# GrandmasterB42/bevyray

Measured on AMD Instinct MI355X. Metric: Mrays/s at 1920x1080, 64 spp, 8 bounces, higher is better.
Workload: dtype f32

## Files before the change

bevyray_amd/_lib.py:

```python
from __future__ import annotations

import ctypes as C
import os
import subprocess
import threading

_HERE = os.path.dirname(os.path.abspath(__file__))
_CSRC = os.path.join(_HERE, "csrc")
LIB_PATH = os.environ.get("BRT_LIB_PATH") or os.path.join(_HERE, "libbevyray_amd.so")

_lock = threading.Lock()
_lib = None


class BrtStats(C.Structure):
    _fields_ = [
        ("rays", C.c_uint64), ("node_pops", C.c_uint64), ("interior_visits", C.c_uint64),
        ("sphere_tests", C.c_uint64), ("hits", C.c_uint64), ("paths", C.c_uint64),
        ("kernel_ms", C.c_double), ("gather_ms", C.c_double), ("total_ms", C.c_double),
        ("lds_bytes", C.c_uint32), ("scene_in_lds", C.c_uint32), ("n_workgroups", C.c_uint32),
        ("threads_per_workgroup", C.c_uint32), ("prepass_ms", C.c_double),
        ("kernel_variant", C.c_uint32), ("measured_tile_costs", C.c_uint32),
        ("tree_rebuilt", C.c_uint32), ("tree_reach", C.c_float), ("forwarded_bytes", C.c_uint64),
        ("hot_records", C.c_uint32), ("reserved", C.c_uint32),
    ]

    def as_dict(self):
        return {name: getattr(self, name) for name, _ in self._fields_}


def _stale() -> bool:
    if not os.path.exists(LIB_PATH):
        return True
    t = os.path.getmtime(LIB_PATH)
    paths = [os.path.join(_CSRC, s) for s in os.listdir(_CSRC) if s.endswith((".cpp", ".hip", ".h")) or s == "Makefile"]
    paths.append(os.path.join(_HERE, "..", "include", "bevyray_amd.h"))
    return any(os.path.exists(p) and os.path.getmtime(p) > t for p in paths)


def build(force: bool = False) -> str:
    if os.environ.get("BRT_LIB_PATH"):
        return LIB_PATH
    with _lock:
        if force or _stale():
            cmd = ["make", "-C", _CSRC, "-j", str(min(6, os.cpu_count() or 1))] + (["-B"] if force else [])
            proc = subprocess.run(cmd, capture_output=True, text=True)
            if proc.returncode != 0:
                raise RuntimeError("building libbevyray_amd.so failed:\n" + proc.stdout + proc.stderr)
    return LIB_PATH


_VP, _U32, _I32, _F = C.c_void_p, C.c_uint32, C.c_int32, C.c_float
_PROTOTYPES = {
    "brt_abi_version": (_U32, []),
    "brt_last_error": (C.c_char_p, [_VP]),
    "brt_create": (_I32, [C.POINTER(_I32), _I32, C.POINTER(_VP)]),
    "brt_destroy": (_I32, [_VP]),
    "brt_set_policy": (_I32, [_VP, _U32]),
    "brt_set_tuning": (_I32, [_VP, C.c_char_p, _U32]),
    "brt_get_tuning": (_I32, [_VP, C.c_char_p, C.POINTER(_U32), C.POINTER(_U32)]),
    "brt_upload_scene": (_I32, [_VP, _VP, _U32, _VP, _U32, _VP, _U32]),
    "brt_render": (_I32, [_VP, _VP, _VP, _U32, _U32, _U32, _VP, _VP, _VP, _U32, C.POINTER(BrtStats)]),
    "brt_host_alloc": (_I32, [_VP, C.c_uint64, C.POINTER(_VP)]),
    "brt_host_free": (_I32, [_VP, _VP]),
    "brt_render_part_device": (_I32, [_VP, _VP, _VP, _U32, _U32, _U32, _U32, _U32, _VP, _VP, _VP, _VP, _U32,
                                      C.POINTER(BrtStats)]),
    "brt_render_device": (_I32, [_VP, _VP, _VP, _U32, _U32, _U32, _VP, _VP, _VP, _VP, _U32, C.POINTER(BrtStats)]),
    "brt_tile_rows": (_U32, [_U32, _U32]),
    "brt_set_strip_table": (_I32, [_VP, _U32, _U32, _VP]),
    "brt_plan_strips": (_I32, [_VP, _VP, _VP, _U32, _U32, _U32, _U32, _U32, _VP]),
    "brt_host_plan_strips": (_I32, [_VP, _U32, _U32, _VP]),
    "brt_deinterleave_device": (_I32, [_VP, _VP, _U32, _U32, _U32, _VP, _VP, _U32]),
    "brt_rccl_unique_id": (_I32, [_VP]),
    "brt_rccl_comm_create": (_I32, [_VP, _VP, _I32, _I32, C.POINTER(_VP)]),
    "brt_rccl_comm_destroy": (_I32, [_VP, _VP]),
    "brt_gather_rccl": (_I32, [_VP, _VP, _I32, _I32, _VP, _VP, _U32, _U32, _VP, _VP, _U32]),
    "brt_import_frame_fd": (_I32, [_VP, _I32, C.c_uint64, _U32, C.POINTER(_VP)]),
    "brt_release_frame": (_I32, [_VP, _VP]),
    "brt_debug_export_frame_fd": (_I32, [_VP, C.c_uint64, C.POINTER(_I32), C.POINTER(_VP)]),
    "brt_debug_copy_to_host": (_I32, [_VP, _VP, _VP, C.c_uint64]),
    "brt_debug_eval": (_I32, [_VP, _U32, _VP, _VP, _U32]),
    "brt_set_denoise": (_I32, [_VP, _U32, _F, _F, _F]),
    "brt_denoise_device": (_I32, [_VP, _VP, _VP, _U32, _U32, _VP, _VP, _VP, _U32, C.POINTER(BrtStats)]),
    "brt_blend_post_device": (_I32, [_VP, _VP, _VP, _U32, _U32, _VP, _VP, _VP, _VP, _U32, C.POINTER(BrtStats)]),
    "brt_debug_denoise_guides": (_I32, [_VP, _VP, _VP, _U32, _U32, _VP]),
    "brt_set_temporal": (_I32, [_VP, _U32]),
    "brt_reset_temporal": (_I32, [_VP]),
    "brt_debug_temporal_state": (_I32, [_VP, _U32, _U32, _VP]),
    "brt_query_rays_device": (_I32, [_VP, _VP, _U32, _U32, _F, _VP, _VP, _U32, C.POINTER(C.c_uint64)]),
    "brt_query_rays": (_I32, [_VP, _VP, _U32, _U32, _F, _VP, C.POINTER(C.c_uint64)]),
    "brt_query_origin_bound": (_I32, [_VP, C.POINTER(_F)]),
    "brt_host_pixel_ray": (_I32, [_VP, _VP, _U32, _U32, _U32, _U32, _VP]),
    "brt_upscale_device": (_I32, [_VP, _VP, _VP, _U32, _U32, _VP, _U32, _U32, _VP, _VP, _U32, C.POINTER(BrtStats)]),
    "brt_render_upscaled_device": (_I32, [_VP, _VP, _VP, _U32, _U32, _U32, _U32, _VP, _VP, _U32, C.POINTER(BrtStats)]),
    "brt_host_upscale_window": (_I32, [_VP, _U32, _U32, _VP]),
    "brt_upscale_blend_device": (_I32, [_VP, _VP, _VP, _U32, _U32, _U32, _VP, _U32, _U32, _VP, _VP, _VP, _VP, _U32,
                                        C.POINTER(BrtStats)]),
    "brt_render_upscaled_blend_device": (_I32, [_VP, _VP, _VP, _U32, _U32, _U32, _U32, _U32, _VP, _VP, _VP, _VP, _U32,
                                                C.POINTER(BrtStats)]),
    "brt_host_blend_covered": (_I32, [_VP, _U32, _F, _F, C.POINTER(_U32)]),
    "brt_render_pixels_device": (_I32, [_VP, _VP, _VP, _U32, _U32, _VP, _U32, _VP, _VP, _U32, C.POINTER(BrtStats)]),
    "brt_render_pixels": (_I32, [_VP, _VP, _VP, _U32, _U32, _VP, _U32, _VP, _U32, C.POINTER(BrtStats)]),
    "brt_upscale_refine_device": (_I32, [_VP, _VP, _VP, _U32, _U32, _VP, _U32, _U32, _VP, _U32, _VP, _VP, _U32, C.POINTER(BrtStats)]),
    "brt_render_upscaled_refined_device": (_I32, [_VP, _VP, _VP, _U32, _U32, _U32, _U32, _VP, _U32, _VP, _VP, _U32,
                                                  C.POINTER(BrtStats)]),
    "brt_upscale_refine_mask_device": (_I32, [_VP, _VP, _VP, _U32, _U32, _VP, _U32, _U32, _VP, _VP, _U32]),
    "brt_set_adaptive": (_I32, [_VP, _U32, _F, _U32]),
    "brt_render_adaptive_device": (_I32, [_VP, _VP, _VP, _U32, _U32, _VP, _VP, _VP, _U32, C.POINTER(BrtStats)]),
    "brt_adaptive_refine_device": (_I32, [_VP, _VP, _VP, _U32, _U32, _VP, _VP, _VP, _VP, _U32, C.POINTER(BrtStats)]),
    "brt_adaptive_mask_device": (_I32, [_VP, _VP, _VP, _U32, _U32, _VP, _VP, _VP, _U32]),
    "brt_host_adaptive_class": (_I32, [_F, _U32, _VP, _VP, _VP, _VP, _F, _U32, C.POINTER(_U32)]),
    "brt_debug_profile": (_I32, [_VP, C.POINTER(C.c_uint64)]),
    "brt_debug_tile_order": (_I32, [_VP, _VP, _VP, _U32, _U32, C.c_uint64, _U32, _U32, _U32, _VP, _VP]),
    "brt_build_bvh": (_I32, [_VP, _U32, _VP, _U32, C.POINTER(_U32)]),
    "brt_build_bvh_sah": (_I32, [_VP, _U32, _F, _VP, _U32, C.POINTER(_U32)]),
    "brt_host_srgb_thresholds": (_I32, [C.POINTER(_F)]),
    "brt_host_tree_reach": (_I32, [_VP, _U32, _VP, C.POINTER(_F), C.POINTER(_U32), C.POINTER(_F)]),
    "brt_build_bvh_device": (_I32, [_VP, _VP, _U32, _VP, _U32, C.POINTER(_U32), C.POINTER(C.c_double)]),
    "brt_build_bvh_sah_device": (_I32, [_VP, _VP, _U32, _F, _VP, _U32, C.POINTER(_U32), C.POINTER(C.c_double)]),
    "brt_validate_scene": (_I32, [_VP, _U32, _VP, _U32, _VP, _U32, C.POINTER(_U32)]),
    "brt_scene_generate": (_I32, [_U32, C.c_uint64, _VP, _VP, _U32, C.POINTER(_U32)]),
    "brt_host_camera_extract": (_I32, [C.POINTER(_F), C.POINTER(_F), C.POINTER(_F), _F, _F, _F, _F, _U32, _U32, _VP]),
    "brt_host_window_extract": (_I32, [_F, _U32, _VP]),
    "brt_host_material": (_I32, [C.POINTER(_F), _F, _F, _F, _F, _F, _VP]),
    "brt_host_tile_order": (_I32, [_VP, _VP, _U32, _U32, C.c_uint64, _U32, _U32, _U32, _U32, _U32, _VP, _VP]),
}
EXPORTS = tuple(_PROTOTYPES)


def _share_hip_runtime_with_torch() -> None:
    import importlib.util
    import sys
    if os.environ.get("BRT_NO_TORCH") == "1" or "torch" in sys.modules:
        return
    if importlib.util.find_spec("torch") is not None:
        import torch


def load() -> C.CDLL:
    global _lib
    if _lib is not None:
        return _lib
    build()
    _share_hip_runtime_with_torch()
    lib = C.CDLL(LIB_PATH)
    for name, (res, args) in _PROTOTYPES.items():
        fn = getattr(lib, name)
        fn.restype = res
        fn.argtypes = args
    if lib.brt_abi_version() != 6:
        raise RuntimeError("libbevyray_amd.so ABI version mismatch")
    _lib = lib
    return lib


def kernel_code_hash(path: str = LIB_PATH) -> str:
    import hashlib
    import struct
    with open(path, "rb") as f:
        data = f.read()
    if data[:4] != b"\x7fELF" or data[4] != 2:
        raise RuntimeError(f"{path}: not an ELF64 file")
    shoff, = struct.unpack_from("<Q", data, 0x28)
    shentsize, shnum, shstrndx = struct.unpack_from("<HHH", data, 0x3A)
    def sec(i):
        name, _type, _flags, _addr, off, size = struct.unpack_from("<IIQQQQ", data, shoff + i * shentsize)
        return name, off, size
    _, stroff, strsize = sec(shstrndx)
    strtab = data[stroff:stroff + strsize]
    for i in range(shnum):
        name, off, size = sec(i)
        if strtab[name:strtab.index(b"\0", name)] == b".hip_fatbin":
            return hashlib.sha256(data[off:off + size]).hexdigest()[:16]
    raise RuntimeError(f"{path}: no .hip_fatbin section")


class BrtError(RuntimeError):
    def __init__(self, code: int, text: str):
        super().__init__(f"bevyray_amd error {code}: {text}")
        self.code = code
        self.text = text


def check(rc: int, ctx=None) -> None:
    if rc != 0:
        msg = load().brt_last_error(ctx)
        raise BrtError(rc, msg.decode("utf-8", "replace") if msg else "")
```

bevyray_amd/csrc/brt_api.cpp:

```cpp
#include "brt_frame.h"
#include "brt_sah.h"

using namespace brt;

namespace {

uint32_t env_u32(const char* name, uint32_t dflt) {
    const char* v = std::getenv(name);
    if (!v || !*v) return dflt;
    return (uint32_t)std::strtoul(v, nullptr, 10);
}

void free_device(DeviceCtx& dc) {
    if (hipSetDevice(dc.device) != hipSuccess) return;
    for (void* p : std::initializer_list<void*>{dc.d_scene, dc.d_ctrl, dc.d_strip_table, dc.d_tile, dc.d_gather, dc.d_pack, dc.d_raster_rgba,
             dc.d_raster_depth, dc.d_bvh_scratch, dc.d_tile_cost, dc.d_tile_order, dc.d_order_meta, dc.d_order_scratch, dc.d_slice_state,
             dc.d_record_hits, dc.d_bvh_models, dc.d_denoise, dc.d_temporal, dc.d_tsph, dc.d_uplow, dc.d_qctl, dc.d_qmap, dc.d_qrays, dc.d_qhits,
             dc.d_pxbuf, dc.d_pxlist, dc.d_pxout})
        if (p) (void)hipFree(p);
    if (dc.h_stage) (void)hipHostFree(dc.h_stage);
    for (hipEvent_t e : {dc.ev_copy, dc.ev_asm, dc.ev_in, dc.ev_g0, dc.ev_g1, dc.ev_pack, dc.ev_strip, dc.ev_strip_read, dc.ev_q, dc.ev_dn,
                         dc.ev0, dc.ev1, dc.ev_last, dc.ev_p0, dc.ev_p1})
        if (e) (void)hipEventDestroy(e);
    if (dc.stream) (void)hipStreamDestroy(dc.stream);
    dc = DeviceCtx();
}

constexpr uint32_t kMaxSahModels = 1u << 16;
constexpr uint32_t kMaxGpuBuildModels = 1u << 24;

int32_t build_bvh_on_device(brt_ctx* ctx, const Model* models, uint32_t n, bool sah, float reach, std::vector<BVHNode>* out, double* build_ms) {
    out->clear();
    if (n == 0) return BRT_OK;
    if (n > (sah ? kMaxSahModels : kMaxGpuBuildModels))
        return ctx_fail(ctx, BRT_ERR_UNSUPPORTED, sah ? "GPU SAH build supports up to 65 536 spheres" : "GPU BVH build supports up to 2^24 spheres");
    DeviceCtx& dc = ctx->devs[0];
    HIP_TRY(ctx, hipSetDevice(dc.device));
    int32_t rc = ensure(ctx, &dc.d_bvh_scratch, &dc.bvh_scratch_cap,
                        sah ? sah_scratch_bytes(n) : ploc_scratch_bytes(n, nullptr, ctx->knobs[K_PLOC_ONE_BLOCK_MAX]));
    if (rc != BRT_OK) return rc;
    rc = ensure(ctx, &dc.d_bvh_models, &dc.bvh_models_cap, (size_t)n * sizeof(Model));
    if (rc != BRT_OK) return rc;
    HIP_TRY(ctx, hipMemcpyAsync(dc.d_bvh_models, models, (size_t)n * sizeof(Model), hipMemcpyHostToDevice, dc.stream));
    BVHNode* d_out = nullptr;
    uint32_t* d_info = nullptr;
    HIP_TRY(ctx, hipEventRecord(dc.ev0, dc.stream));
    if (sah) HIP_TRY(ctx, launch_build_sah(reinterpret_cast<const Model*>(dc.d_bvh_models), n, reach, dc.d_bvh_scratch, &d_out, &d_info, dc.stream));
    else HIP_TRY(ctx, launch_build_ploc(reinterpret_cast<const Model*>(dc.d_bvh_models), n, dc.d_bvh_scratch, &d_out, &d_info, ctx->knobs[K_PLOC_ONE_BLOCK_MAX], dc.stream));
    HIP_TRY(ctx, hipEventRecord(dc.ev1, dc.stream));
    out->resize(2 * (size_t)n - 1);
    HIP_TRY(ctx, hipMemcpyAsync(out->data(), d_out, out->size() * sizeof(BVHNode), hipMemcpyDeviceToHost, dc.stream));
    uint32_t info[2] = {0u, 0u};
    HIP_TRY(ctx, hipMemcpyAsync(info, d_info, sizeof info, hipMemcpyDeviceToHost, dc.stream));
    HIP_TRY(ctx, hipStreamSynchronize(dc.stream));
    if (info[0] != 2u * n - 1u) {
        out->clear();
        return ctx_fail(ctx, BRT_ERR_HIP, "GPU BVH build made no progress after " + std::to_string(info[1]) + " rounds");
    }
    if (sah) sah_giant_leaves_first(out->data(), (uint32_t)out->size(), models, n);
    float kernel_ms = 0.0f;
    HIP_TRY(ctx, hipEventElapsedTime(&kernel_ms, dc.ev0, dc.ev1));
    if (build_ms) *build_ms = kernel_ms;
    return BRT_OK;
}

}

namespace brt {

int32_t upload_scene(brt_ctx* ctx, const void* models, uint32_t n_models, const void* materials, uint32_t n_materials,
                     const void* bvh_nodes, uint32_t n_nodes, uint32_t level, bool rebuild) {
    if (const uint32_t k = ctx->knobs[K_TEST_THROW]) { ctx->knobs.v[K_TEST_THROW] = 0u; throw_for_test(k); }
    const size_t mb = (size_t)n_models * sizeof(Model), tb = (size_t)n_materials * sizeof(Material),
                 bb = (bvh_nodes ? (size_t)n_nodes : 0) * sizeof(BVHNode);
    auto same = [](const std::vector<char>& v, const void* p, size_t n) {
        return v.size() == n && (n == 0 || (p && std::memcmp(v.data(), p, n) == 0));
    };
    if (!rebuild && ctx->has_scene && ctx->knobs[K_NO_DIRTY_TRACKING] == 0 && same(ctx->last_models, models, mb) &&
        same(ctx->last_materials, materials, tb) && same(ctx->last_bvh, bvh_nodes, bb))
        return BRT_OK;
    for (auto& dc : ctx->devs) {
        HIP_TRY(ctx, hipSetDevice(dc.device));
        for (hipEvent_t e : {dc.ev_last, dc.ev_copy, dc.ev_asm, dc.ev_q}) HIP_TRY(ctx, hipEventSynchronize(e));
    }
    ctx->has_scene = false;
    float reach = 0.0f;
    if (!rebuild) {
        ctx->tree_scene = tree_scene_of(static_cast<const Model*>(models), models ? n_models : 0u);
        ctx->tree_callee_sah = false;
        ctx->tree_level = 0;
        ctx->tree_reach = 0.0f;
        ctx->query_level = 0;
    } else {
        reach = tree_reach_of(ctx->tree_scene.scale, level);
    }
    std::vector<BVHNode> built;
    const BVHNode* nodes = static_cast<const BVHNode*>(bvh_nodes);
    if (n_models > 0 && models && (!bvh_nodes || n_nodes == 0)) {
        const bool sah = ctx->knobs[K_BVH_QUALITY] != 0u && n_models <= kMaxSahModels;
        const bool on_gpu = ctx->knobs[K_CPU_BVH] == 0u && n_models <= kMaxGpuBuildModels;
        int32_t rc;
        if (on_gpu) rc = build_bvh_on_device(ctx, static_cast<const Model*>(models), n_models, sah, reach, &built, nullptr);
        else rc = sah ? build_bvh_sah(static_cast<const Model*>(models), n_models, reach, &built)
                      : build_bvh_ploc(static_cast<const Model*>(models), n_models, &built);
        if (rc != BRT_OK) return rc;
        ctx->tree_callee_sah = sah;
        ctx->tree_level = level;
        ctx->tree_reach = reach;
        nodes = built.data();
        n_nodes = (uint32_t)built.size();
    }
    std::string err;
    int32_t rc = validate_and_encode(static_cast<const Model*>(models), n_models, static_cast<const Material*>(materials),
                                     n_materials, nodes, n_nodes, &ctx->enc, &err);
    if (rc != BRT_OK) return ctx_fail(ctx, rc, err);
    const EncodedScene& e = ctx->enc;

    struct Sec { const void* src; size_t bytes; size_t off; };
    Sec secs[6] = {
        {e.pairs.data(), e.pairs.size() * 4, 0}, {e.spheres.data(), e.spheres.size() * 4, 0},
        {e.sphere_material.data(), e.sphere_material.size() * 4, 0}, {e.materials.data(), e.materials.size() * 4, 0},
        {e.leaf_table.data(), e.leaf_table.size() * 4, 0}, {e.sphere_mats.data(), e.sphere_mats.size() * 4, 0}};
    size_t total = 0;
    for (auto& s : secs) { s.off = total; total += align256(s.bytes ? s.bytes : 16); }

    const uint64_t shape = (ctx->knobs[K_HOT_RECORDS] != 0u && !rebuild && e.desc16 && e.simple_tree && e.n_pairs > 64u) ? tree_shape_hash(e) : 0ull;
    ctx->tree_epoch++;
    for (auto& dc : ctx->devs) {
        HIP_TRY(ctx, hipSetDevice(dc.device));
        int32_t r2 = ensure(ctx, &dc.d_scene, &dc.scene_cap, total);
        if (r2 != BRT_OK) return r2;
        const bool reuse = shape != 0ull && dc.hot_shape == shape && dc.hot_records != 0u && dc.h_total_rank.size() == e.n_pairs &&
                           dc.h_total_srank.size() == e.n_models;
        uint32_t root = e.root_desc;
        Sec mine[6];
        for (int q = 0; q < 6; q++) mine[q] = secs[q];
        if (reuse) {
            permute_scene(e.pairs, e.spheres, e.sphere_material, e.sphere_mats, e.root_desc, dc.h_total_rank, dc.h_total_srank, &dc.h_pairs_cur,
                          &dc.h_spheres_cur, &dc.h_sphmat_cur, &dc.h_sphmats_cur, &root);
            mine[0].src = dc.h_pairs_cur.data(); mine[1].src = dc.h_spheres_cur.data(); mine[2].src = dc.h_sphmat_cur.data(); mine[5].src = dc.h_sphmats_cur.data();
        }
        for (auto& s : mine)
            if (s.bytes) HIP_TRY(ctx, hipMemcpyAsync(dc.d_scene + s.off, s.src, s.bytes, hipMemcpyHostToDevice, dc.stream));
        const uint32_t kept_hot = reuse ? dc.hot_records : 0u;
        DeviceSceneView v{};
        v.pairs = reinterpret_cast<const float*>(dc.d_scene + secs[0].off);
        v.spheres = reinterpret_cast<const float*>(dc.d_scene + secs[1].off);
        v.sphere_material = reinterpret_cast<const uint32_t*>(dc.d_scene + secs[2].off);
        v.materials = reinterpret_cast<const float*>(dc.d_scene + secs[3].off);
        v.leaf_table = reinterpret_cast<const uint32_t*>(dc.d_scene + secs[4].off);
        v.sphere_mats = reinterpret_cast<const float*>(dc.d_scene + secs[5].off);
        v.n_pairs = e.n_pairs;
        v.n_models = e.n_models;
        v.n_materials = e.n_materials;
        v.n_leaf_table = (uint32_t)(e.leaf_table.size() / 2);
        v.root_desc = root;
        v.stack_entries = e.stack_entries;
        v.desc16 = e.desc16 ? 1u : 0u;
        v.simple_tree = e.simple_tree ? 1u : 0u;
        v.boxes_ordered = e.boxes_ordered ? 1u : 0u;
        dc.view = v;
        dc.hot_records = kept_hot;
        if (reuse) dc.hot_tree = ctx->tree_epoch;
        dc.frames_since_upload = 0u;
    }
    for (auto& dc : ctx->devs) {
        HIP_TRY(ctx, hipSetDevice(dc.device));
        HIP_TRY(ctx, hipStreamSynchronize(dc.stream));
    }
// ... 284 lines not shown
```

bevyray_amd/csrc/brt_api_launch.cpp:

```cpp
#include "brt_frame.h"

namespace brt {

int32_t make_frame_params(brt_ctx* ctx, const void* camera80, const void* window16, uint32_t level, uint32_t width,
                          uint32_t height, uint32_t part, uint32_t n_parts, FrameParams* out) {
    if (const uint32_t k = ctx->knobs[K_TEST_THROW]) { ctx->knobs.v[K_TEST_THROW] = 0u; throw_for_test(k); }
    if (!camera80 || !window16) return ctx_fail(ctx, BRT_ERR_INVALID_ARGUMENT, "camera/window is null");
    if (width == 0 || height == 0 || width > 32768u || height > 32768u)
        return ctx_fail(ctx, BRT_ERR_INVALID_ARGUMENT, "width/height must be in [1, 32768]");
    if (n_parts == 0 || part >= n_parts) return ctx_fail(ctx, BRT_ERR_INVALID_ARGUMENT, "part >= n_parts");
    Camera cam;
    Window win;
    std::memcpy(&cam, camera80, sizeof cam);
    std::memcpy(&win, window16, sizeof win);
    if (cam.projection_type != 0)
        return ctx_fail(ctx, BRT_ERR_UNSUPPORTED, "only perspective projection (0) is supported (extract.rs:148)");
    if (cam.bounce_count >= 0x7fffffffu) return ctx_fail(ctx, BRT_ERR_INVALID_ARGUMENT, "bounce_count too large");
    FrameParams fp;
    std::memset(&fp, 0, sizeof fp);
    fp.width = width;
    fp.height = height;
    fp.level = level;
    fp.sample_count = cam.sample_count;
    fp.bounce_count = cam.bounce_count;
    fp.seed_scaled = win.random_seed * 10000.0f;
    const float heightf = (float)win.height;
    const float widthf = (float)win.height * cam.aspect;
    fp.inv_width = 1.0f / widthf;
    fp.inv_height = 1.0f / heightf;
    fp.aspect = cam.aspect;
    fp.tan_half_fov = tan_half_fov(cam.fov);
    for (int k = 0; k < 3; k++) {
        fp.cam_pos[k] = cam.position[k];
        fp.cam_dir[k] = cam.direction[k];
        fp.cam_up[k] = cam.up[k];
    }
    const float* a = cam.direction;
    const float* b = cam.up;
    fp.cam_right[0] = a[1] * b[2] - a[2] * b[1];
    fp.cam_right[1] = a[2] * b[0] - a[0] * b[2];
    fp.cam_right[2] = a[0] * b[1] - a[1] * b[0];
    fp.near_ = cam.near_;
    fp.far_ = cam.far_;
    fp.fallback_far = (level == 1u) ? cam.far_ + 10.0f : cam.far_ - 1.0f;
    fp.spp_f = (float)cam.sample_count;
    fp.part = part;
    fp.n_parts = n_parts;
    fp.tiles_x = (width + 7u) / 8u;
    const uint32_t strips = (height + BRT_STRIP_ROWS - 1u) / BRT_STRIP_ROWS;
    fp.local_strips = (strips + n_parts - 1u) / n_parts;
    fp.queue_size = fp.local_strips * fp.tiles_x * 64u;
    fp.queue_lane = 0u;
    fp.bottom_up = ctx->knobs[K_BOTTOM_UP];
    fp.refill_min = std::clamp(ctx->knobs[K_REFILL_MIN], 1u, 64u);
    fp.walk_exit_lanes = std::min(ctx->knobs[K_WALK_EXIT], 63u);
    fp.leaf_vote = std::min(ctx->knobs[K_LEAF_VOTE], 64u);
    fp.drain_donate = std::min(ctx->knobs[K_DRAIN_DONATE], 56u);
    fp.pool_cap = 0;
    fp.pool_adopt = std::min(ctx->knobs[K_POOL_ADOPT], 63u);
    fp.crit_begin = fp.crit_end = 0;
    fp.split_nonsky = fp.split_tiles = 0;
    fp.slice_state = nullptr;
    fp.slice_serial = 0;
    fp.wgq_batch = std::min(ctx->knobs[K_WGQ_BATCH] & ~63u, 512u);
    fp.policy_flags = ctx->policy_flags & kPolicyMask;
    fp.tunable = (fp.policy_flags != 0u || fp.bottom_up != 0u || fp.refill_min != kRefillMin || fp.walk_exit_lanes != kWalkExitLanes ||
                  fp.leaf_vote != kLeafVote || fp.drain_donate != kDrainDonate || fp.pool_adopt != kPoolAdopt ||
                  fp.wgq_batch != 0u || ctx->knobs[K_LPT_LANE_PERMILLE] != 0u || ctx->knobs[K_TUNABLE] != 0u)
                     ? 1u : 0u;
    *out = fp;
    return BRT_OK;
}

LaunchPlan plan_launch(const Knobs& kn, const DeviceCtx& dc, const FrameParams& fp) {
    LaunchPlan lp{};
    const uint32_t hist = fp.record_hits ? dc.view.n_pairs : 0u;
    const bool force_global = kn[K_FORCE_GLOBAL_SCENE] != 0;
    const uint32_t force_top = kn[K_FORCE_LDS_TOP];
    const uint32_t block_env = kn[K_BLOCK_THREADS];
    const uint32_t wg_env = kn[K_WG_PER_CU];
    const uint32_t max_waves_cu = 32;
    lp.scene_mode = SCENE_GLOBAL;
    const uint64_t n_tiles = fp.queue_size / 64u, wave_slots = (uint64_t)dc.num_cus * (BRT_BLOCK / 64u);
    const uint32_t pool_max = (2u * n_tiles <= 5u * wave_slots && kn[K_POOL_FORCE] == 0u) ? 0u : kn[K_POOL_CAP];
    auto pool_of = [&](uint32_t block) {
        const uint32_t want = fp.drain_donate * (block / 64u - 1u);
        return want < pool_max ? want : pool_max;
    };
    if (!force_global && !force_top && dc.view.desc16) {
        struct Cand { uint32_t block, per_cu; };
        const Cand cands[] = {{1024, 1}, {512, 2}, {512, 3}, {1024, 2}, {512, 1}, {256, 1}};
        for (int opt = 0; opt < 4 && lp.scene_mode != SCENE_LDS; opt++) {
            const int with_pool = opt < 2 ? 1 : 0, with_rows = (opt & 1) == 0 ? 1 : 0;
            for (const Cand& c : cands) {
                if (block_env && c.block != block_env) continue;
                if (wg_env && c.per_cu != wg_env) continue;
                const uint32_t pool = with_pool ? pool_of(c.block) : 0u;
                const size_t need = trace_lds_bytes(dc.view, SCENE_LDS, c.block, pool, 0, with_rows != 0);
                if (need * c.per_cu <= dc.max_lds && c.per_cu * (c.block / 64) <= max_waves_cu) {
                    lp.scene_mode = SCENE_LDS;
                    lp.block = c.block;
                    lp.wg_per_cu = c.per_cu;
                    lp.lds_bytes = need;
                    lp.pool_cap = pool;
                    lp.rows = (uint32_t)with_rows;
                    break;
                }
            }
        }
    }
    if (lp.scene_mode != SCENE_LDS && !force_global && dc.view.desc16) {
        DeviceSceneView v = dc.view;
        v.lds_pairs = 0;
        const uint32_t block = block_env ? block_env : BRT_BLOCK;
        const uint32_t per_cu = wg_env ? wg_env : 1u;
        const size_t share = dc.max_lds / per_cu;
        const uint32_t pool = pool_of(block) < 192u / per_cu ? pool_of(block) : 192u / per_cu;
        const size_t fixed = trace_lds_bytes(v, SCENE_LDS_TOP, block, pool, hist);
        if (fixed + 64 * PAIR_BYTES <= share && per_cu * (block / 64u) <= max_waves_cu) {
            uint32_t k = (uint32_t)((share - fixed) / PAIR_BYTES);
            if (k > v.n_pairs) k = v.n_pairs;
            if (force_top && force_top < k) k = force_top;
            v.lds_pairs = k;
            lp.scene_mode = SCENE_LDS_TOP;
            lp.lds_pairs = k;
            lp.block = block;
            lp.wg_per_cu = per_cu;
            lp.pool_cap = pool;
            lp.lds_bytes = trace_lds_bytes(v, SCENE_LDS_TOP, block, pool, hist);
        }
    }
    if (lp.scene_mode == SCENE_GLOBAL) {
        lp.block = block_env ? block_env : 256u;
        lp.pool_cap = pool_of(lp.block);
        lp.lds_bytes = trace_lds_bytes(dc.view, SCENE_GLOBAL, lp.block, lp.pool_cap);
        uint32_t per_cu = (uint32_t)(dc.max_lds / (lp.lds_bytes ? lp.lds_bytes : 1));
        const uint32_t by_waves = max_waves_cu / (lp.block / 64u);
        if (per_cu > by_waves) per_cu = by_waves;
        if (per_cu < 1) per_cu = 1;
        if (wg_env) per_cu = wg_env;
        lp.wg_per_cu = per_cu;
    }
    lp.grid = (uint32_t)dc.num_cus * lp.wg_per_cu;
    const uint32_t useful = (fp.queue_size + lp.block - 1u) / lp.block;
    if (lp.grid > useful) lp.grid = useful;
    if (lp.grid < 1) lp.grid = 1;
    return lp;
}

int32_t launch_part(brt_ctx* ctx, DeviceCtx& dc, const FrameParams& fp, const float* d_raster_rgba,
                    const float* d_raster_depth, float* d_out_tile, hipStream_t stream, uint32_t flags, bool timed,
                    LaunchPlan* plan_out) {
    HIP_TRY(ctx, hipStreamWaitEvent(stream, dc.ev_last, 0));
    HIP_TRY(ctx, hipMemsetAsync(dc.d_ctrl, 0, 512, stream));
    if (timed) HIP_TRY(ctx, hipEventRecord(dc.ev0, stream));
    LaunchPlan lp{};
    if (fp.level == 0u) {
        HIP_TRY(ctx, launch_passthrough(fp, d_out_tile, d_raster_rgba, stream));
    } else {
        TraceLaunch tl{};
        tl.scene = dc.view;
        tl.frame = fp;
        tl.queue_counter = reinterpret_cast<uint32_t*>(dc.d_ctrl + 256);
        tl.out_tile = d_out_tile;
        tl.raster_rgba = d_raster_rgba;
        tl.raster_depth = d_raster_depth;
        tl.counters = reinterpret_cast<unsigned long long*>(dc.d_ctrl);
        tl.counters_on = (flags & BRT_FLAG_COUNTERS) != 0;
        tl.stream = stream;
        if (flags & BRT_FLAG_KERNEL_SIMPLE) {
            if (fp.policy_flags != 0u) return ctx_fail(ctx, BRT_ERR_UNSUPPORTED, "the bring-up kernel implements the default policy only (brt_set_policy)");
            HIP_TRY(ctx, launch_trace_simple(tl));
            lp.block = 256;
            lp.grid = (fp.queue_size + 255u) / 256u;
        } else {
            lp = plan_launch(ctx->knobs, dc, fp);
            {
                uint32_t key[8];
                view_key_of(ctx, fp, key);
                const bool known = dc.view_rays != 0 && std::memcmp(key, dc.view_key, sizeof key) == 0;
                const uint64_t per_lane = known ? dc.view_rays / ((uint64_t)dc.num_cus * BRT_BLOCK) : 0;
                const uint64_t longest_bound = (uint64_t)fp.sample_count * ((uint64_t)fp.bounce_count + 1u);
                const bool lean1 = !tl.frame.tunable && fp.level == 3u && !tl.counters_on && ctx->knobs[K_NO_LEAN] == 0u &&
                                   (fp.tile_cost == nullptr || ctx->knobs[K_LEAN_MEASURE] != 0u);
                tl.lean = !lean1 ? 0 : ((known && longest_bound < per_lane / 2) ? 2 : 1);
                lp.variant = (uint32_t)tl.lean | (tl.frame.tunable ? 16u : 0u);
                lp.measured = fp.tile_cost != nullptr ? 1u : 0u;
            }
            tl.scene_mode = lp.scene_mode;
            tl.scene.lds_pairs = lp.lds_pairs;
            tl.grid = lp.grid;
            tl.block = lp.block;
            tl.lds_bytes = lp.lds_bytes;
            tl.frame.pool_cap = lp.pool_cap;
            tl.frame.rows_on = lp.scene_mode == SCENE_LDS ? lp.rows : 0u;
            if (tl.frame.wgq_batch == 0u) {
                uint32_t b = (fp.queue_size / (lp.grid * 8u)) & ~63u;
                const uint32_t cap = (lp.block / 2u) & ~63u;
                if (b > cap) b = cap;
                if (b > 512u) b = 512u;
                if (b < 64u) b = 64u;
                tl.frame.wgq_batch = b;
            }
            HIP_TRY(ctx, launch_trace_persistent(tl));
        }
    }
    if (timed) HIP_TRY(ctx, hipEventRecord(dc.ev1, stream));
    HIP_TRY(ctx, hipEventRecord(dc.ev_last, stream));
    if (plan_out) *plan_out = lp;
    return BRT_OK;
}

uint64_t part_pixels(const FrameParams& fp) { return PartStrips(fp.height, fp.part, fp.n_parts).total_rows() * fp.width; }

void launch_stats(const brt_ctx* ctx, const DeviceCtx& dc, const LaunchPlan& lp, brt_stats* stats) {
    stats->lds_bytes = (uint32_t)lp.lds_bytes;
    stats->scene_in_lds = lp.scene_mode == SCENE_LDS ? 1u : (lp.scene_mode == SCENE_LDS_TOP ? 2u : 0u);
    stats->n_workgroups = lp.grid;
    stats->threads_per_workgroup = lp.block;
    stats->kernel_variant = lp.variant;
    stats->measured_tile_costs = lp.measured;
    stats->hot_records = dc.hot_tree == ctx->tree_epoch ? dc.hot_records : 0u;
}

int32_t collect_part(brt_ctx* ctx, DeviceCtx& dc, const FrameParams& fp, hipStream_t stream, bool prepass_ran, brt_stats* st) {
    int32_t rc = update_tile_order(ctx, dc, fp, stream);
    if (rc != BRT_OK) return rc;
    unsigned long long c[5];
    HIP_TRY(ctx, hipMemcpyAsync(c, dc.d_ctrl, sizeof c, hipMemcpyDeviceToHost, stream));
    HIP_TRY(ctx, hipStreamSynchronize(stream));
    st->rays += c[0];
    st->node_pops += c[1];
    st->interior_visits += c[2];
    st->sphere_tests += c[3];
    st->hits += c[4];
    dc.view_rays = c[0];
    view_key_of(ctx, fp, dc.view_key);
    float ms = 0.0f;
    HIP_TRY(ctx, hipEventElapsedTime(&ms, dc.ev0, dc.ev1));
    if (ms > st->kernel_ms) st->kernel_ms = ms;
    if (prepass_ran) {
        HIP_TRY(ctx, hipEventElapsedTime(&ms, dc.ev_p0, dc.ev_p1));
        if (ms > st->prepass_ms) st->prepass_ms = ms;
    }
    return BRT_OK;
}

}
```

bevyray_amd/csrc/brt_api_order.cpp:

```cpp
#include "brt_frame.h"

using namespace brt;

namespace {

bool lpt_enabled(const brt_ctx* ctx) { return ctx->knobs[K_LPT] != 0; }
uint64_t camera_hash(const FrameParams& fp) {
    uint64_t h = 1469598103934665603ull;
    auto mix = [&](const float* f, int n) {
        for (int i = 0; i < n; i++) { uint32_t u; std::memcpy(&u, f + i, 4); h = (h ^ u) * 1099511628211ull; }
    };
    mix(fp.cam_pos, 3); mix(fp.cam_dir, 3); mix(fp.cam_up, 3); mix(&fp.tan_half_fov, 1); mix(&fp.aspect, 1);
    return h | 1ull;
}

void order_key_of(const brt_ctx* ctx, const FrameParams& fp, uint32_t key[6]) {
    key[0] = fp.width; key[1] = fp.height; key[2] = fp.part; key[3] = fp.n_parts;
    key[4] = fp.strip_of ? ctx->strip_epoch : 0u;
    key[5] = fp.local_strips * fp.tiles_x;
}

constexpr uint32_t kMaxDilate = 8;
double camera_motion_px(const brt_ctx* ctx, const float* pos0, const float* dir0, const FrameParams& fp) {
    const float* a = dir0;
// ... 17 lines not shown
    const double px = camera_motion_px(ctx, dc.cost_cam_pos, dc.cost_cam_dir, fp);
    if (!(px < 8.0 * kMaxDilate)) return kMaxDilate + 1u;
    return (uint32_t)std::ceil(px / 8.0) + 1u;
}
bool camera_jumped(const brt_ctx* ctx, const DeviceCtx& dc, const FrameParams& fp) {
    return dc.costs_valid && camera_hash(fp) != dc.order_cam && dilation_tiles(ctx, dc, fp) > kMaxDilate;
}

uint32_t split_tail_of(const brt_ctx* ctx, const DeviceCtx& dc, uint32_t n_tiles) {
    const uint64_t wave_slots = (uint64_t)dc.num_cus * (BRT_BLOCK / 64u);
    if (ctx->knobs[K_SPLIT_FORCE] != 0u) return ctx->knobs[K_SPLIT_FORCE] < n_tiles ? ctx->knobs[K_SPLIT_FORCE] : n_tiles;
    if ((uint64_t)n_tiles < 6u * wave_slots) return 0u;
    uint64_t r = (uint64_t)ctx->knobs[K_SPLIT_TAIL] * wave_slots / 4u;
    if (r != 0u && r < n_tiles / 2u) r = n_tiles / 2u;
    return (uint32_t)(r < n_tiles ? r : n_tiles);
}

int32_t build_order_on_device(brt_ctx* ctx, DeviceCtx& dc, uint32_t n_tiles, uint32_t tiles_x, uint32_t spp, uint32_t rx, uint32_t ry,
                              hipStream_t stream) {
    if (!dc.d_order_meta) HIP_TRY(ctx, hipMalloc(reinterpret_cast<void**>(&dc.d_order_meta), 256));
    int32_t rc = ensure(ctx, &dc.d_order_scratch, &dc.order_scratch_cap, order_scratch_bytes(n_tiles));
    if (rc != BRT_OK) return rc;
    const uint32_t split_tail = split_tail_of(ctx, dc, n_tiles);
    rc = ensure(ctx, &dc.d_tile_order, &dc.tile_order_cap, ((size_t)n_tiles + split_tail) * 4);
    if (rc != BRT_OK) return rc;
    const uint64_t sky_cost = (uint64_t)64 * spp * (1000 + ctx->knobs[K_LPT_SKY_SLACK]) / 1000;
    HIP_TRY(ctx, launch_build_order(dc.d_tile_cost, dc.d_tile_cost + n_tiles, n_tiles, sky_cost, (uint64_t)dc.num_cus * BRT_BLOCK, tiles_x, rx,
                                    ry, split_tail, dc.d_tile_order, dc.d_order_meta, dc.d_order_scratch, stream));
    HIP_TRY(ctx, hipEventRecord(dc.ev_last, stream));
    return BRT_OK;
}

int32_t apply_hot_order(brt_ctx* ctx, DeviceCtx& dc, hipStream_t stream) {
    const uint32_t n = dc.view.n_pairs, m = dc.view.n_models;
    const EncodedScene& e = ctx->enc;
    if (n == 0u || e.pairs.size() != (size_t)n * PAIR_WORDS || e.spheres.size() != (size_t)m * 4u || e.sphere_material.size() != m || e.sphere_mats.size() != (size_t)m * 8u) return BRT_OK;
    if (dc.hot_tree != ctx->tree_epoch) { dc.h_pairs_cur = e.pairs; dc.h_spheres_cur = e.spheres; dc.h_sphmat_cur = e.sphere_material; dc.h_sphmats_cur = e.sphere_mats; }
    const std::vector<float>& cur = dc.h_pairs_cur;
    const uint32_t cur_root = dc.hot_tree != ctx->tree_epoch ? e.root_desc : dc.view.root_desc;
    dc.h_hits.resize(n);
    HIP_TRY(ctx, hipMemcpyAsync(dc.h_hits.data(), dc.d_record_hits, (size_t)n * 4, hipMemcpyDeviceToHost, stream));
    HIP_TRY(ctx, hipStreamSynchronize(stream));
    std::vector<uint32_t>& rank = dc.h_rank;
    std::vector<uint32_t> order(n);
    for (uint32_t i = 0; i < n; i++) order[i] = i;
    std::stable_sort(order.begin(), order.end(), [&](uint32_t a, uint32_t b) { return dc.h_hits[a] > dc.h_hits[b]; });
    rank.resize(n);
    uint32_t visited = 0;
    for (uint32_t i = 0; i < n; i++) { rank[order[i]] = i; visited += dc.h_hits[order[i]] != 0u ? 1u : 0u; }
    using D = Desc<true>;
    constexpr uint32_t kDescWord = PAIR_DESC / 4u;
    std::vector<uint32_t> score(m, 0u), sorder(m), srank(m);
    auto leaf_sphere = [&](uint32_t d, uint32_t* id) {
        if ((int32_t)d < -1 && (d & D::LEAF1)) { *id = d & D::INDEX_MASK; return *id < m; }
        return false;
    };
    for (uint32_t r = 0; r < n; r++)
        for (uint32_t k = 0; k < 2u; k++) {
            uint32_t d, id;
            std::memcpy(&d, cur.data() + (size_t)r * PAIR_WORDS + kDescWord + k, 4);
            if (leaf_sphere(d, &id) && dc.h_hits[r] > score[id]) score[id] = dc.h_hits[r];
        }
    for (uint32_t i = 0; i < m; i++) sorder[i] = i;
    std::stable_sort(sorder.begin(), sorder.end(), [&](uint32_t a, uint32_t b) { return score[a] > score[b]; });
    for (uint32_t i = 0; i < m; i++) srank[sorder[i]] = i;
    std::vector<float> sph, mats;
    std::vector<uint32_t> mat;
    uint32_t new_root = 0;
    permute_scene(cur, dc.h_spheres_cur, dc.h_sphmat_cur, dc.h_sphmats_cur, cur_root, rank, srank, &dc.h_pairs_hot, &sph, &mat, &mats, &new_root);
    HIP_TRY(ctx, hipEventSynchronize(dc.ev_q));
    dc.hot_serial++;
    HIP_TRY(ctx, hipMemcpyAsync(const_cast<float*>(dc.view.pairs), dc.h_pairs_hot.data(), dc.h_pairs_hot.size() * 4, hipMemcpyHostToDevice, stream));
    HIP_TRY(ctx, hipMemcpyAsync(const_cast<float*>(dc.view.spheres), sph.data(), sph.size() * 4, hipMemcpyHostToDevice, stream));
    HIP_TRY(ctx, hipMemcpyAsync(const_cast<uint32_t*>(dc.view.sphere_material), mat.data(), mat.size() * 4, hipMemcpyHostToDevice, stream));
    HIP_TRY(ctx, hipMemcpyAsync(const_cast<float*>(dc.view.sphere_mats), mats.data(), mats.size() * 4, hipMemcpyHostToDevice, stream));
    HIP_TRY(ctx, hipStreamSynchronize(stream));
    if (dc.hot_tree == ctx->tree_epoch && dc.h_total_rank.size() == n && dc.h_total_srank.size() == m) {
        for (uint32_t i = 0; i < n; i++) dc.h_total_rank[i] = rank[dc.h_total_rank[i]];
        for (uint32_t i = 0; i < m; i++) dc.h_total_srank[i] = srank[dc.h_total_srank[i]];
    } else {
        dc.h_total_rank = rank;
        dc.h_total_srank = srank;
    }
    dc.hot_shape = tree_shape_hash(e);
    dc.h_pairs_cur.swap(dc.h_pairs_hot);
    dc.h_spheres_cur.swap(sph);
    dc.h_sphmat_cur.swap(mat);
    dc.h_sphmats_cur.swap(mats);
    dc.view.root_desc = new_root;
    dc.hot_tree = ctx->tree_epoch;
    dc.hot_records = visited;
    return BRT_OK;
}

}

namespace brt {

void view_key_of(const brt_ctx* ctx, const FrameParams& fp, uint32_t key[8]) {
    order_key_of(ctx, fp, key);
    key[6] = fp.sample_count; key[7] = fp.bounce_count;
}

int32_t attach_tile_order(brt_ctx* ctx, DeviceCtx& dc, FrameParams& fp, hipStream_t stream, bool may_measure, uint32_t flags) {
    fp.tile_order = nullptr;
    fp.tile_cost = nullptr;
    if (!lpt_enabled(ctx) || fp.level == 0u || (flags & BRT_FLAG_KERNEL_SIMPLE)) return BRT_OK;
    const uint32_t n_tiles = fp.local_strips * fp.tiles_x;
    uint32_t key[6];
    order_key_of(ctx, fp, key);
    const bool match = dc.order_valid && std::memcmp(key, dc.order_key, sizeof key) == 0;
    if (match && dc.costs_valid && dc.order_on_device && camera_hash(fp) != dc.order_cam && ctx->knobs[K_LPT_DILATE] != 0u) {
        uint32_t r = dilation_tiles(ctx, dc, fp);
        if (r <= kMaxDilate && ctx->knobs[K_LPT_DILATE] >= 2u && r < ctx->knobs[K_LPT_DILATE] - 1u &&
            (uint64_t)n_tiles >= 6u * (uint64_t)dc.num_cus * (BRT_BLOCK / 64u))
            r = ctx->knobs[K_LPT_DILATE] - 1u;
        if (r <= kMaxDilate) {
            HIP_TRY(ctx, hipStreamWaitEvent(stream, dc.ev_last, 0));
            const int32_t rc = build_order_on_device(ctx, dc, n_tiles, fp.tiles_x, dc.cost_spp, r, (r + fp.n_parts - 1u) / fp.n_parts, stream);
            if (rc != BRT_OK) return rc;
        }
    }
    if (match) {
        fp.tile_order = dc.d_tile_order;
        fp.queue_lane = dc.order_lane * 64u;
        fp.crit_begin = 0u;
        fp.crit_end = dc.order_crit * 64u;
        fp.order_meta = dc.order_on_device ? dc.d_order_meta : nullptr;
        if (split_tail_of(ctx, dc, n_tiles) != 0u) {
            const size_t bytes = (size_t)fp.queue_size * 36u;
            const bool fresh = bytes > dc.slice_state_cap;
            int32_t rc = ensure(ctx, &dc.d_slice_state, &dc.slice_state_cap, bytes);
            if (rc != BRT_OK) return rc;
            if (fresh || dc.slice_serial >= 0x3fffffffu) {
                HIP_TRY(ctx, hipMemsetAsync(dc.d_slice_state, 0, dc.slice_state_cap, stream));
                dc.slice_serial = 0u;
            }
            fp.slice_state = dc.d_slice_state;
            fp.slice_serial = ++dc.slice_serial;
            if (!dc.order_on_device) { fp.split_nonsky = dc.order_nonsky; fp.split_tiles = dc.order_split; }
        }
    }
    bool due = !match || camera_hash(fp) != dc.order_cam || ctx->knobs[K_LPT_REFRESH_EVERY] == 1u;
    if (may_measure && match && dc.remeasure_in != 0u && --dc.remeasure_in == 0u) due = true;
    if (may_measure && due) {
        int32_t rc = ensure(ctx, &dc.d_tile_cost, &dc.tile_cost_cap, (size_t)n_tiles * 8);
        if (rc != BRT_OK) return rc;
        HIP_TRY(ctx, hipMemsetAsync(dc.d_tile_cost, 0, (size_t)n_tiles * 8, stream));
        fp.tile_cost = dc.d_tile_cost;
    }
    return BRT_OK;
}

int32_t update_tile_order(brt_ctx* ctx, DeviceCtx& dc, const FrameParams& fp, hipStream_t stream) {
    if (!fp.tile_cost) return BRT_OK;
    const uint32_t n_tiles = fp.local_strips * fp.tiles_x;
    TileOrderParams tp{};
    tp.sample_count = fp.sample_count;
    tp.grid_lanes = (uint64_t)dc.num_cus * BRT_BLOCK;
    tp.sorted = ctx->knobs[K_LPT_SORT];
    tp.sky_slack_permille = ctx->knobs[K_LPT_SKY_SLACK];
    tp.lane_permille = ctx->knobs[K_LPT_LANE_PERMILLE];
    tp.critical = ctx->knobs[K_CRIT];
    tp.tiles_x = fp.tiles_x;
    tp.split_tail = split_tail_of(ctx, dc, n_tiles);
    int32_t rc = ensure(ctx, &dc.d_tile_order, &dc.tile_order_cap, ((size_t)n_tiles + tp.split_tail) * 4);
    if (rc != BRT_OK) return rc;
    const bool on_device = tp.sorted == 1u && tp.critical == 1u && tp.lane_permille == 0u && ctx->knobs[K_ORDER_ON_HOST] == 0u;
    dc.costs_valid = false;
    if (on_device) {
        const uint64_t wave_slots = (uint64_t)dc.num_cus * (BRT_BLOCK / 64u);
        const uint32_t r0 = (ctx->knobs[K_LPT_DILATE] >= 2u && (uint64_t)n_tiles >= 6u * wave_slots) ? ctx->knobs[K_LPT_DILATE] - 1u : 0u;
        tp.dilate_x = r0;
        tp.dilate_y = r0 ? (r0 + fp.n_parts - 1u) / fp.n_parts : 0u;
        rc = build_order_on_device(ctx, dc, n_tiles, fp.tiles_x, tp.sample_count, tp.dilate_x, tp.dilate_y, stream);
        if (rc != BRT_OK) return rc;
        dc.order_lane = 0;
        dc.order_crit = 0;
        dc.order_on_device = true;
        dc.costs_valid = true;
        dc.cost_spp = tp.sample_count;
        for (int k = 0; k < 3; k++) { dc.cost_cam_pos[k] = fp.cam_pos[k]; dc.cost_cam_dir[k] = fp.cam_dir[k]; }
    } else {
        dc.h_cost.resize(2 * (size_t)n_tiles);
        HIP_TRY(ctx, hipMemcpyAsync(dc.h_cost.data(), dc.d_tile_cost, (size_t)n_tiles * 8, hipMemcpyDeviceToHost, stream));
        HIP_TRY(ctx, hipStreamSynchronize(stream));
        TileOrder to;
        build_tile_order(dc.h_cost.data(), dc.h_cost.data() + n_tiles, n_tiles, tp, &to);
        dc.h_order.swap(to.order);
        dc.order_lane = to.n_lane;
        dc.order_crit = to.n_critical;
        dc.order_on_device = false;
        dc.order_nonsky = to.n_nonsky;
        dc.order_split = to.n_split;
        HIP_TRY(ctx, hipMemcpyAsync(dc.d_tile_order, dc.h_order.data(), dc.h_order.size() * 4, hipMemcpyHostToDevice, stream));
        HIP_TRY(ctx, hipStreamSynchronize(stream));
    }
    order_key_of(ctx, fp, dc.order_key);
    dc.order_valid = true;
    dc.remeasure_in = 0;
    dc.order_cam = camera_hash(fp);
    return BRT_OK;
}

uint64_t tree_shape_hash(const EncodedScene& e) {
    uint64_t h = 1469598103934665603ull ^ ((uint64_t)e.n_pairs << 32) ^ e.n_models;
    constexpr uint32_t kDescWord = PAIR_DESC / 4u;
    for (uint32_t r = 0; r < e.n_pairs; r++)
        for (uint32_t k = 0; k < 2u; k++) {
            uint32_t d;
            std::memcpy(&d, e.pairs.data() + (size_t)r * PAIR_WORDS + kDescWord + k, 4);
            h = (h ^ d) * 1099511628211ull;
        }
    return h | 1ull;
}

void permute_scene(const std::vector<float>& pairs, const std::vector<float>& spheres, const std::vector<uint32_t>& sphmat,
                   const std::vector<float>& sphmats, uint32_t root, const std::vector<uint32_t>& rank, const std::vector<uint32_t>& srank,
                   std::vector<float>* out_pairs, std::vector<float>* out_spheres, std::vector<uint32_t>* out_sphmat,
                   std::vector<float>* out_sphmats, uint32_t* out_root) {
    using D = Desc<true>;
    constexpr uint32_t kDescWord = PAIR_DESC / 4u;
    const uint32_t n = (uint32_t)rank.size(), m = (uint32_t)srank.size();
    auto remap = [&](uint32_t d) {
        if ((int32_t)d >= 0 && d < n) return rank[d];
        if ((int32_t)d < -1 && (d & D::LEAF1) && (d & D::INDEX_MASK) < m) return (d & ~D::INDEX_MASK) | srank[d & D::INDEX_MASK];
        return d;
    };
    out_pairs->resize(pairs.size());
    for (uint32_t i = 0; i < n; i++) {
        const float* src = pairs.data() + (size_t)i * PAIR_WORDS;
        float* dst = out_pairs->data() + (size_t)rank[i] * PAIR_WORDS;
        std::memcpy(dst, src, PAIR_BYTES);
        for (uint32_t k = 0; k < 2u; k++) {
            uint32_t d;
            std::memcpy(&d, src + kDescWord + k, 4);
            d = remap(d);
            std::memcpy(dst + kDescWord + k, &d, 4);
        }
    }
    out_spheres->resize(spheres.size());
    out_sphmats->resize(sphmats.size());
    out_sphmat->resize(m);
    for (uint32_t i = 0; i < m; i++) {
        std::memcpy(out_spheres->data() + (size_t)srank[i] * 4, spheres.data() + (size_t)i * 4, 16);
        std::memcpy(out_sphmats->data() + (size_t)srank[i] * 8, sphmats.data() + (size_t)i * 8, 32);
        (*out_sphmat)[srank[i]] = sphmat[i];
    }
    *out_root = remap(root);
}

int32_t prepass_order(brt_ctx* ctx, DeviceCtx& dc, const FrameParams& fp, const float* d_raster_rgba,
                      const float* d_raster_depth, float* d_out_tile, hipStream_t stream, uint32_t flags, bool* ran) {
    *ran = false;
    const uint32_t knob = ctx->knobs[K_PREPASS_SPP];
    const uint32_t k = knob < fp.sample_count / 16u ? knob : fp.sample_count / 16u;
    if (k == 0u || (k == 1u && knob != 1u) || !lpt_enabled(ctx) || fp.level == 0u || (flags & BRT_FLAG_KERNEL_SIMPLE)) return BRT_OK;
    uint32_t key[6];
    order_key_of(ctx, fp, key);
    bool hot_stale = ctx->knobs[K_HOT_RECORDS] != 0u && dc.hot_tree == ctx->tree_epoch && dc.hot_records != 0u &&
                     camera_motion_px(ctx, dc.hot_cam_pos, dc.hot_cam_dir, fp) > std::max(64.0, 0.25 * (double)fp.height);
    if (dc.frames_since_upload < 1000u) dc.frames_since_upload++;
    if (!hot_stale && ctx->knobs[K_HOT_RECORDS] != 0u && dc.hot_tree != ctx->tree_epoch && dc.frames_since_upload == 2u && dc.view.desc16 &&
        dc.view.simple_tree && dc.view.n_pairs > 64u && plan_launch(ctx->knobs, dc, fp).scene_mode == SCENE_LDS_TOP)
        hot_stale = true;
    if (dc.order_valid && std::memcmp(key, dc.order_key, sizeof key) == 0 && !(ctx->knobs[K_LPT_DILATE] != 0u && camera_jumped(ctx, dc, fp)) && !hot_stale)
        return BRT_OK;
    FrameParams pp = fp;
    pp.sample_count = k;
    pp.spp_f = (float)k;
    pp.tile_order = nullptr;
    pp.order_meta = nullptr;
    pp.slice_state = nullptr;
    pp.split_nonsky = pp.split_tiles = 0u;
    pp.tunable = 1u;
    pp.queue_lane = 0u;
    pp.crit_begin = pp.crit_end = 0u;
    const uint32_t n_tiles = pp.local_strips * pp.tiles_x;
    int32_t rc = ensure(ctx, &dc.d_tile_cost, &dc.tile_cost_cap, (size_t)n_tiles * 8);
    if (rc != BRT_OK) return rc;
    HIP_TRY(ctx, hipMemsetAsync(dc.d_tile_cost, 0, (size_t)n_tiles * 8, stream));
    pp.tile_cost = dc.d_tile_cost;
    bool count_hits = false;
    if (ctx->knobs[K_HOT_RECORDS] != 0u && dc.view.desc16 && dc.view.simple_tree && dc.view.n_pairs > 64u &&
        plan_launch(ctx->knobs, dc, pp).scene_mode == SCENE_LDS_TOP) {
        rc = ensure(ctx, &dc.d_record_hits, &dc.record_hits_cap, (size_t)dc.view.n_pairs * 4);
        if (rc != BRT_OK) return rc;
        HIP_TRY(ctx, hipMemsetAsync(dc.d_record_hits, 0, (size_t)dc.view.n_pairs * 4, stream));
        pp.record_hits = dc.d_record_hits;
        count_hits = plan_launch(ctx->knobs, dc, pp).scene_mode == SCENE_LDS_TOP;
        if (!count_hits) pp.record_hits = nullptr;
    }
    HIP_TRY(ctx, hipEventRecord(dc.ev_p0, stream));
    rc = launch_part(ctx, dc, pp, d_raster_rgba, d_raster_depth, d_out_tile, stream, flags & ~(uint32_t)BRT_FLAG_COUNTERS, false, nullptr);
    if (rc != BRT_OK) return rc;
    HIP_TRY(ctx, hipEventRecord(dc.ev_p1, stream));
    rc = update_tile_order(ctx, dc, pp, stream);
    if (rc != BRT_OK) return rc;
    if (count_hits) {
        rc = apply_hot_order(ctx, dc, stream);
        if (rc != BRT_OK) return rc;
        for (int q = 0; q < 3; q++) { dc.hot_cam_pos[q] = fp.cam_pos[q]; dc.hot_cam_dir[q] = fp.cam_dir[q]; }
    }
    dc.remeasure_in = 1u;
    *ran = true;
    return BRT_OK;
}

bool strip_table_valid(const uint32_t* t, uint32_t n_strips, uint32_t n_parts) {
    if (n_parts == 0u || n_parts > 64u) return false;
    for (uint32_t g = 0; g * n_parts < n_strips; g++) {
        uint64_t seen = 0;
        for (uint32_t s = g * n_parts; s < n_strips && s < (g + 1u) * n_parts; s++) {
            if (t[s] >= n_parts || (seen >> t[s]) & 1ull) return false;
            seen |= 1ull << t[s];
        }
    }
    return true;
}
int32_t strip_table_attach(brt_ctx* ctx, DeviceCtx& dc, FrameParams* fp, const uint32_t** part_of_strip, hipStream_t stream) {
    if (part_of_strip) *part_of_strip = nullptr;
    const uint32_t strips = (fp->height + BRT_STRIP_ROWS - 1u) / BRT_STRIP_ROWS, n_parts = fp->n_parts;
    if (ctx->strip_part.empty() || ctx->strip_n_parts != n_parts || ctx->strip_part.size() != strips || n_parts < 2u) return BRT_OK;
    const uint32_t local = (strips + n_parts - 1u) / n_parts;
    if (dc.strip_epoch != ctx->strip_epoch || !dc.d_strip_table) {
        const size_t words = (size_t)strips + (size_t)n_parts * local;
        HIP_TRY(ctx, hipEventSynchronize(dc.ev_strip));
        if (dc.strip_table_cap < words * 4u)
            for (hipEvent_t e : {dc.ev_last, dc.ev_strip_read}) HIP_TRY(ctx, hipEventSynchronize(e));
        int32_t rc = ensure(ctx, &dc.d_strip_table, &dc.strip_table_cap, words * 4u);
        if (rc != BRT_OK) return rc;
        std::vector<uint32_t>& h = dc.h_strip_table;
        h.assign(words, 0xffffffu);
        std::copy(ctx->strip_part.begin(), ctx->strip_part.end(), h.begin());
        for (uint32_t s = 0; s < strips; s++) h[(size_t)strips + (size_t)ctx->strip_part[s] * local + s / n_parts] = s;
        HIP_TRY(ctx, hipStreamWaitEvent(stream, dc.ev_last, 0));
        HIP_TRY(ctx, hipStreamWaitEvent(stream, dc.ev_strip_read, 0));
        HIP_TRY(ctx, hipMemcpyAsync(dc.d_strip_table, h.data(), words * 4u, hipMemcpyHostToDevice, stream));
        HIP_TRY(ctx, hipEventRecord(dc.ev_strip, stream));
        dc.strip_epoch = ctx->strip_epoch;
    } else {
        HIP_TRY(ctx, hipStreamWaitEvent(stream, dc.ev_strip, 0));
    }
    const uint32_t* d = reinterpret_cast<const uint32_t*>(dc.d_strip_table);
    if (part_of_strip) *part_of_strip = d;
    fp->strip_of = d + strips + (size_t)fp->part * local;
    return BRT_OK;
}
int32_t strip_table_read(brt_ctx* ctx, DeviceCtx& dc, const uint32_t* part_of_strip, hipStream_t stream) {
    if (!part_of_strip) return BRT_OK;
    HIP_TRY(ctx, hipStreamWaitEvent(stream, dc.ev_strip_read, 0));
    HIP_TRY(ctx, hipEventRecord(dc.ev_strip_read, stream));
    return BRT_OK;
}
uint64_t part_pixels_table(const brt_ctx* ctx, const FrameParams& fp) {
    uint64_t rows = 0;
    for (uint32_t s = 0; s < (uint32_t)ctx->strip_part.size(); s++)
        if (ctx->strip_part[s] == fp.part) {
            const uint32_t r0 = s * BRT_STRIP_ROWS;
            rows += (r0 + BRT_STRIP_ROWS <= fp.height) ? BRT_STRIP_ROWS : (fp.height - r0);
        }
    return rows * fp.width;
}

}

extern "C" {

uint32_t brt_tile_rows(uint32_t height, uint32_t n_parts) {
    if (n_parts == 0) return 0;
    const uint32_t strips = (height + BRT_STRIP_ROWS - 1u) / BRT_STRIP_ROWS;
    return ((strips + n_parts - 1u) / n_parts) * BRT_STRIP_ROWS;
}

int32_t brt_set_strip_table(brt_ctx* ctx, uint32_t n_parts, uint32_t n_strips, const uint32_t* part_of_strip) {
    return guard(ctx ? &ctx->last_error : nullptr, [&]() -> int32_t {
    if (!ctx) return fail(BRT_ERR_INVALID_ARGUMENT, "ctx is null");
    if (!part_of_strip) { ctx->strip_epoch++; ctx->strip_part.clear(); ctx->strip_n_parts = 0u; return BRT_OK; }
    if (n_parts < 1u || n_strips < 1u || n_strips > 4096u) return ctx_fail(ctx, BRT_ERR_INVALID_ARGUMENT, "n_parts / n_strips out of range");
    if (!strip_table_valid(part_of_strip, n_strips, n_parts))
        return ctx_fail(ctx, BRT_ERR_INVALID_ARGUMENT, "strip table: every group of n_parts consecutive strips must hold each part at most once");
    ctx->strip_epoch++;
    ctx->strip_part.assign(part_of_strip, part_of_strip + n_strips);
    ctx->strip_n_parts = n_parts;
    return BRT_OK;
    });
}

int32_t brt_plan_strips(brt_ctx* ctx, const void* camera80, const void* window16, uint32_t level, uint32_t width, uint32_t height,
                        uint32_t n_parts, uint32_t probe_spp, uint32_t* out_part_of_strip) {
    return guard(ctx ? &ctx->last_error : nullptr, [&]() -> int32_t {
    if (!ctx) return fail(BRT_ERR_INVALID_ARGUMENT, "ctx is null");
    if (!ctx->has_scene) return ctx_fail(ctx, BRT_ERR_NO_SCENE, "no scene uploaded");
    if (n_parts < 1u || n_parts > 64u || probe_spp < 1u) return ctx_fail(ctx, BRT_ERR_INVALID_ARGUMENT, "n_parts must be 1..64, probe_spp >= 1");
    FrameParams fp;
    int32_t rc = make_frame_params(ctx, camera80, window16, level == 0u ? 3u : level, width, height, 0u, 1u, &fp);
    if (rc != BRT_OK) return rc;
    fp.sample_count = probe_spp;
    fp.spp_f = (float)probe_spp;
    DeviceCtx& dc = ctx->devs[0];
    HIP_TRY(ctx, hipSetDevice(dc.device));
    const uint32_t n_tiles = fp.local_strips * fp.tiles_x, strips = fp.local_strips;
    rc = ensure(ctx, &dc.d_tile, &dc.tile_cap, (size_t)strips * BRT_STRIP_ROWS * width * 16u);
    if (rc != BRT_OK) return rc;
    rc = ensure(ctx, &dc.d_tile_cost, &dc.tile_cost_cap, (size_t)n_tiles * 8u);
    if (rc != BRT_OK) return rc;
    HIP_TRY(ctx, hipStreamWaitEvent(dc.stream, dc.ev_last, 0));
    HIP_TRY(ctx, hipMemsetAsync(dc.d_tile_cost, 0, (size_t)n_tiles * 8u, dc.stream));
    fp.tile_cost = dc.d_tile_cost;
    rc = launch_part(ctx, dc, fp, nullptr, nullptr, dc.d_tile, dc.stream, 0u, false, nullptr);
    if (rc != BRT_OK) return rc;
    std::vector<uint32_t> cost(n_tiles);
    HIP_TRY(ctx, hipMemcpyAsync(cost.data(), dc.d_tile_cost, (size_t)n_tiles * 4u, hipMemcpyDeviceToHost, dc.stream));
    HIP_TRY(ctx, hipStreamSynchronize(dc.stream));
    dc.costs_valid = false;
    std::vector<uint64_t> strip_cost(strips, 0);
    for (uint32_t t = 0; t < n_tiles; t++) strip_cost[t / fp.tiles_x] += cost[t];
    std::vector<uint32_t> table(strips, 0u);
    plan_strip_table(strip_cost.data(), strips, n_parts, table.data());
    if (out_part_of_strip) std::memcpy(out_part_of_strip, table.data(), (size_t)strips * 4u);
    ctx->strip_epoch++;
    ctx->strip_part = table;
    ctx->strip_n_parts = n_parts;
    return BRT_OK;
    });
}

int32_t brt_debug_tile_order(brt_ctx* ctx, const uint32_t* ray_sum, const uint32_t* longest_pixel, uint32_t n_tiles,
                             uint32_t sample_count, uint64_t grid_lanes, uint32_t tiles_x, uint32_t dilate, uint32_t split_tail,
                             uint32_t* out_order, uint32_t* out_info4) {
    return guard(ctx ? &ctx->last_error : nullptr, [&]() -> int32_t {
    if (!ctx) return fail(BRT_ERR_INVALID_ARGUMENT, "ctx is null");
    if (!ray_sum || !longest_pixel || !out_order || !out_info4 || n_tiles == 0) return ctx_fail(ctx, BRT_ERR_INVALID_ARGUMENT, "null buffer / no tiles");
    if (dilate != 0u && (tiles_x == 0u || n_tiles % tiles_x != 0u)) return ctx_fail(ctx, BRT_ERR_INVALID_ARGUMENT, "dilate needs a tiles_x that divides n_tiles");
    DeviceCtx& dc = ctx->devs[0];
    HIP_TRY(ctx, hipSetDevice(dc.device));
    uint32_t* d_cost = nullptr;
    uint32_t* d_order = nullptr;
    uint32_t* d_meta = nullptr;
    char* d_scratch = nullptr;
    auto body = [&]() -> int32_t {
        HIP_TRY(ctx, hipMalloc(reinterpret_cast<void**>(&d_cost), (size_t)n_tiles * 8));
        HIP_TRY(ctx, hipMalloc(reinterpret_cast<void**>(&d_order), ((size_t)n_tiles + split_tail) * 4));
        HIP_TRY(ctx, hipMalloc(reinterpret_cast<void**>(&d_meta), 256));
        HIP_TRY(ctx, hipMalloc(reinterpret_cast<void**>(&d_scratch), order_scratch_bytes(n_tiles)));
        HIP_TRY(ctx, hipMemcpyAsync(d_cost, ray_sum, (size_t)n_tiles * 4, hipMemcpyHostToDevice, dc.stream));
        HIP_TRY(ctx, hipMemcpyAsync(d_cost + n_tiles, longest_pixel, (size_t)n_tiles * 4, hipMemcpyHostToDevice, dc.stream));
        const uint64_t sky_cost = (uint64_t)64 * sample_count * (1000 + 20) / 1000;
        HIP_TRY(ctx, launch_build_order(d_cost, d_cost + n_tiles, n_tiles, sky_cost, grid_lanes, tiles_x, dilate, dilate, split_tail, d_order, d_meta, d_scratch, dc.stream));
        HIP_TRY(ctx, hipMemcpyAsync(out_info4, d_meta, 16, hipMemcpyDeviceToHost, dc.stream));
        HIP_TRY(ctx, hipStreamSynchronize(dc.stream));
        HIP_TRY(ctx, hipMemcpy(out_order, d_order, ((size_t)n_tiles + out_info4[3]) * 4, hipMemcpyDeviceToHost));
        return BRT_OK;
    };
    const int32_t rc = body();
    if (d_cost) (void)hipFree(d_cost);
    if (d_order) (void)hipFree(d_order);
    if (d_meta) (void)hipFree(d_meta);
    if (d_scratch) (void)hipFree(d_scratch);
    return rc;
    });
}

}
```

bevyray_amd/csrc/brt_ctx.h:

```cpp
#pragma once
#include <hip/hip_runtime.h>

#include <cstdint>
#include <cstring>
#include <string>
#include <vector>

#include "brt_adaptive.h"
#include "brt_denoise.h"
#include "brt_temporal.h"
#include "brt_host.h"
#include "brt_kernels.h"
#include "brt_pixels.h"
#include "brt_query.h"
#include "brt_upscale.h"

namespace brt {

struct DeviceCtx {
    int device = 0;
    hipStream_t stream = nullptr;
    hipEvent_t ev0 = nullptr, ev1 = nullptr;
    hipEvent_t ev_last = nullptr;
    hipEvent_t ev_p0 = nullptr, ev_p1 = nullptr;
    int num_cus = 0;
    size_t max_lds = 0;
    char* d_scene = nullptr;
    size_t scene_cap = 0;
    DeviceSceneView view{};
    char* d_ctrl = nullptr;
    float* d_tile = nullptr;
    size_t tile_cap = 0;
    float* d_raster_rgba = nullptr;
    size_t raster_rgba_cap = 0;
    float* d_raster_depth = nullptr;
    size_t raster_depth_cap = 0;
    float* d_gather = nullptr;
    size_t gather_cap = 0;
    float* d_pack = nullptr;
    size_t pack_cap = 0;
    hipEvent_t ev_pack = nullptr;
    hipEvent_t ev_copy = nullptr;
    hipEvent_t ev_asm = nullptr;
    hipEvent_t ev_in = nullptr;
    hipEvent_t ev_g0 = nullptr, ev_g1 = nullptr;
    float* h_stage = nullptr;
    size_t stage_cap = 0;
    uint32_t* d_tile_cost = nullptr;
    size_t tile_cost_cap = 0;
    uint32_t* d_tile_order = nullptr;
    uint32_t order_nonsky = 0, order_split = 0;
    uint32_t* d_slice_state = nullptr;
    size_t slice_state_cap = 0;
    uint32_t slice_serial = 0;
    uint32_t order_lane = 0;
    uint32_t order_crit = 0;
    size_t tile_order_cap = 0;
    uint32_t* d_order_meta = nullptr;
    char* d_strip_table = nullptr;
    size_t strip_table_cap = 0;
    uint32_t strip_epoch = 0;
    std::vector<uint32_t> h_strip_table;
    hipEvent_t ev_strip = nullptr;
    hipEvent_t ev_strip_read = nullptr;
    char* d_order_scratch = nullptr;
    size_t order_scratch_cap = 0;
    bool order_on_device = false;
    uint64_t view_rays = 0;
    uint32_t view_key[8] = {0, 0, 0, 0, 0, 0, 0, 0};
    uint64_t base_view_rays = 0;
    uint32_t base_view_key[8] = {0, 0, 0, 0, 0, 0, 0, 0};
    bool order_valid = false;
    uint32_t remeasure_in = 0;
    uint64_t order_cam = 0;
    bool costs_valid = false;
    float cost_cam_pos[3] = {0, 0, 0}, cost_cam_dir[3] = {0, 0, 0};
    uint32_t cost_spp = 0;
    uint32_t order_key[6] = {0, 0, 0, 0, 0, 0};
    std::vector<uint32_t> h_cost;
    std::vector<uint32_t> h_order;
    uint32_t* d_record_hits = nullptr;
    size_t record_hits_cap = 0;
    uint32_t hot_tree = 0;
    uint32_t hot_records = 0;
    float hot_cam_pos[3] = {0, 0, 0}, hot_cam_dir[3] = {0, 0, 1};
    uint32_t frames_since_upload = 0;
    std::vector<uint32_t> h_hits, h_rank;
    std::vector<uint32_t> h_total_rank, h_total_srank;
    uint64_t hot_shape = 0;
    std::vector<float> h_spheres_cur, h_sphmats_cur;
    std::vector<uint32_t> h_sphmat_cur;
    std::vector<float> h_pairs_hot, h_pairs_cur;
    char* d_denoise = nullptr;
    size_t denoise_cap = 0;
    hipEvent_t ev_dn = nullptr;
    char* d_temporal = nullptr;
    size_t temporal_cap = 0;
    char* d_tsph = nullptr;
    size_t tsph_cap = 0;
    float* d_uplow = nullptr;
    size_t uplow_cap = 0;
    hipEvent_t ev_q = nullptr;
    uint32_t* d_qctl = nullptr;
    uint32_t* d_qmap = nullptr;
    size_t qmap_cap = 0;
    uint32_t qmap_tree = 0, qmap_serial = 0;
    uint32_t hot_serial = 0;
    char* d_qrays = nullptr;
    size_t qrays_cap = 0;
    char* d_qhits = nullptr;
    size_t qhits_cap = 0;
    uint32_t* d_pxbuf = nullptr;
    size_t pxbuf_cap = 0;
    char* d_pxlist = nullptr;
    size_t pxlist_cap = 0;
    char* d_pxout = nullptr;
    size_t pxout_cap = 0;
    char* d_bvh_scratch = nullptr;
    size_t bvh_scratch_cap = 0;
    char* d_bvh_models = nullptr;
    size_t bvh_models_cap = 0;
};


enum Knob : int {
    K_BOTTOM_UP, K_REFILL_MIN, K_WALK_EXIT, K_LEAF_VOTE, K_DRAIN_DONATE, K_POOL_ADOPT, K_WGQ_BATCH, K_LPT_LANE_PERMILLE, K_TUNABLE,
    K_FORCE_GLOBAL_SCENE, K_FORCE_LDS_TOP, K_BLOCK_THREADS, K_WG_PER_CU, K_POOL_CAP, K_LPT, K_LPT_SORT, K_LPT_SKY_SLACK, K_CRIT,
    K_ORDER_ON_HOST, K_NO_LEAN, K_PREPASS_SPP, K_NO_DIRTY_TRACKING, K_CPU_BVH, K_PLOC_ONE_BLOCK_MAX, K_BVH_QUALITY, K_POOL_FORCE, K_LPT_REFRESH_EVERY, K_LEAN_MEASURE, K_LPT_DILATE, K_SPLIT_TAIL, K_SPLIT_FORCE, K_HOT_RECORDS, K_TEST_THROW, K_QUERY_FORM, K_QUERY_STREAM_MIN, K_PIXELS_FORM, K_COUNT
};
struct KnobDef { const char* name; uint32_t dflt; };
constexpr KnobDef kKnobs[K_COUNT] = {
    {"BRT_BOTTOM_UP", 0}, {"BRT_REFILL_MIN", kRefillMin}, {"BRT_WALK_EXIT", kWalkExitLanes}, {"BRT_LEAF_VOTE", kLeafVote},
    {"BRT_DRAIN_DONATE", kDrainDonate}, {"BRT_POOL_ADOPT", kPoolAdopt}, {"BRT_WGQ_BATCH", 0}, {"BRT_LPT_LANE_PERMILLE", 0},
    {"BRT_TUNABLE", 0}, {"BRT_FORCE_GLOBAL_SCENE", 0}, {"BRT_FORCE_LDS_TOP", 0}, {"BRT_BLOCK_THREADS", 0}, {"BRT_WG_PER_CU", 0},
    {"BRT_POOL_CAP", 384}, {"BRT_LPT", 1}, {"BRT_LPT_SORT", 1}, {"BRT_LPT_SKY_SLACK", 20}, {"BRT_CRIT", 1}, {"BRT_ORDER_ON_HOST", 0},
    {"BRT_NO_LEAN", 0}, {"BRT_PREPASS_SPP", 4}, {"BRT_NO_DIRTY_TRACKING", 0}, {"BRT_CPU_BVH", 0},
    {"BRT_PLOC_ONE_BLOCK_MAX", kPlocOneBlockMax}, {"BRT_BVH_QUALITY", 1}, {"BRT_POOL_FORCE", 0}, {"BRT_LPT_REFRESH_EVERY", 0}, {"BRT_LEAN_MEASURE", 1}, {"BRT_LPT_DILATE", 3}, {"BRT_SPLIT_TAIL", 16}, {"BRT_SPLIT_FORCE", 0}, {"BRT_HOT_RECORDS", 1}, {"BRT_TEST_THROW", 0},
    {"BRT_QUERY_FORM", 0}, {"BRT_QUERY_STREAM_MIN", 0},
    {"BRT_PIXELS_FORM", 0}};
struct Knobs {
    uint32_t v[K_COUNT];
    Knobs() { for (int i = 0; i < K_COUNT; i++) v[i] = kKnobs[i].dflt; }
    uint32_t operator[](Knob k) const { return v[k]; }
};

}

namespace brt {
struct ExternalFrame {
    void* ptr = nullptr;
    size_t bytes = 0, mapped = 0;
    uint32_t type = 0;
    hipExternalMemory_t ext = nullptr;
    hipMemGenericAllocationHandle_t vmm{};
};
}

struct brt_ctx {
    std::vector<brt::ExternalFrame> external;
    std::vector<brt::DeviceCtx> devs;
    brt::EncodedScene enc;
    bool has_scene = false;
    uint32_t scene_epoch = 0;
    std::vector<uint32_t> strip_part;
    uint32_t strip_n_parts = 0, strip_epoch = 0;
    uint32_t tree_epoch = 0;
    uint32_t last_n_models = 0;
    std::vector<std::pair<char*, size_t>> pinned;
    std::vector<char> last_models, last_materials, last_bvh;
    float scene_centre[3] = {0, 0, 0};
    bool tree_callee_sah = false;
    brt::TreeScene tree_scene;
    uint32_t tree_level = 0;
    float tree_reach = 0.0f;
    uint32_t tree_rebuilds = 0;
    uint32_t query_level = 0;
    brt::Knobs knobs;
    uint32_t policy_flags = 0;
    brt::DenoiseSettings denoise;
    struct Adaptive {
        uint32_t base_spp = 8;
        float threshold = brt::kAdaptDefaultThreshold;
        uint32_t min_taps = 6;
    } adaptive;
    struct Temporal {
        uint32_t max_history = 32;
        bool valid = false;
        uint32_t width = 0, height = 0, set = 0;
        brt::FrameParams prev{};
        uint32_t prev_models = 0;
        int64_t prev_epoch = -1;
        uint32_t slot_models = 0;
        int64_t slot_epoch[2] = {-1, -1};
        std::vector<uint32_t> h_rmap;
    } temporal;
    std::string last_error;
};

namespace brt {

inline int32_t ctx_fail(brt_ctx* ctx, int32_t code, const std::string& msg) {
    if (ctx) ctx->last_error = msg;
    g_last_error = msg;
    return code;
}

#define HIP_TRY(ctx, expr)                                                                              \
    do {                                                                                                \
        hipError_t _e = (expr);                                                                         \
        if (_e != hipSuccess)                                                                           \
            return ctx_fail(ctx, BRT_ERR_HIP, std::string(#expr) + ": " + hipGetErrorString(_e));       \
    } while (0)

template <typename T>
int32_t ensure(brt_ctx* ctx, T** ptr, size_t* cap, size_t bytes) {
    if (*cap >= bytes && *ptr) return BRT_OK;
    if (*ptr) HIP_TRY(ctx, hipFree(*ptr));
    *ptr = nullptr;
    *cap = 0;
    HIP_TRY(ctx, hipMalloc(reinterpret_cast<void**>(ptr), bytes));
    *cap = bytes;
    return BRT_OK;
}

inline size_t align256(size_t x) { return (x + 255) & ~(size_t)255; }

void release_external_frames(brt_ctx* ctx);

}

namespace brt {
bool strip_table_valid(const uint32_t* part_of_strip, uint32_t n_strips, uint32_t n_parts);
int32_t strip_table_attach(brt_ctx* ctx, DeviceCtx& dc, FrameParams* fp, const uint32_t** part_of_strip, hipStream_t stream);
int32_t strip_table_read(brt_ctx* ctx, DeviceCtx& dc, const uint32_t* part_of_strip, hipStream_t stream);
uint64_t part_pixels_table(const brt_ctx* ctx, const FrameParams& fp);
}
```

bevyray_amd/csrc/brt_frame.h:

```cpp
#pragma once
#include <hip/hip_runtime.h>

#include <algorithm>
#include <chrono>
#include <cmath>
#include <cstdlib>
#include <cstring>
#include <limits>
#include <string>
#include <vector>

#include "brt_ctx.h"

namespace brt {

constexpr uint32_t kPolicyMask = BRT_POLICY_OR_SHORT_CIRCUIT | BRT_POLICY_MINMAX_SELECT | BRT_POLICY_POW_EXP2_LOG2;
constexpr uint32_t kLptAfterUpload = 4;

inline double ms_since(std::chrono::steady_clock::time_point t0) {
    return std::chrono::duration<double, std::milli>(std::chrono::steady_clock::now() - t0).count();
}

struct StreamChoice { bool own; hipStream_t stream; };
inline StreamChoice stream_of(const DeviceCtx& dc, void* hip_stream, uint32_t flags) {
    const bool own = (hip_stream == nullptr) && !(flags & BRT_FLAG_CALLER_STREAM);
    return {own, own ? dc.stream : static_cast<hipStream_t>(hip_stream)};
}

struct PartStrips {
    uint32_t part, n_parts;
    uint32_t n_full;
    uint32_t tail_rows;
    PartStrips(uint32_t height, uint32_t part_, uint32_t n_parts_) : part(part_), n_parts(n_parts_) {
        const uint32_t full = height / BRT_STRIP_ROWS;
        n_full = full > part ? (full - part + n_parts - 1u) / n_parts : 0u;
        tail_rows = full % n_parts == part ? height - full * BRT_STRIP_ROWS : 0u;
    }
    uint32_t count() const { return n_full + (tail_rows ? 1u : 0u); }
    uint32_t frame_row(uint32_t k) const { return (part + k * n_parts) * BRT_STRIP_ROWS; }
    uint32_t rows(uint32_t k) const { return k < n_full ? BRT_STRIP_ROWS : tail_rows; }
    uint64_t total_rows() const { return (uint64_t)n_full * BRT_STRIP_ROWS + tail_rows; }
};

int32_t upload_scene(brt_ctx* ctx, const void* models, uint32_t n_models, const void* materials, uint32_t n_materials,
                     const void* bvh_nodes, uint32_t n_nodes, uint32_t level, bool rebuild);
int32_t ensure_tree_reach(brt_ctx* ctx, const void* camera80, uint32_t* rebuilt);
void tree_stats(const brt_ctx* ctx, uint32_t rebuilt, brt_stats* stats);

struct LaunchPlan {
    int scene_mode;
    uint32_t lds_pairs;
    uint32_t block, grid, wg_per_cu;
    uint32_t pool_cap;
    uint32_t rows;
    size_t lds_bytes;
    uint32_t variant;
    uint32_t measured;
};
int32_t make_frame_params(brt_ctx* ctx, const void* camera80, const void* window16, uint32_t level, uint32_t width,
                          uint32_t height, uint32_t part, uint32_t n_parts, FrameParams* out);
LaunchPlan plan_launch(const Knobs& kn, const DeviceCtx& dc, const FrameParams& fp);
int32_t launch_part(brt_ctx* ctx, DeviceCtx& dc, const FrameParams& fp, const float* d_raster_rgba,
                    const float* d_raster_depth, float* d_out_tile, hipStream_t stream, uint32_t flags, bool timed,
                    LaunchPlan* plan_out);
uint64_t part_pixels(const FrameParams& fp);
void launch_stats(const brt_ctx* ctx, const DeviceCtx& dc, const LaunchPlan& lp, brt_stats* stats);
int32_t collect_part(brt_ctx* ctx, DeviceCtx& dc, const FrameParams& fp, hipStream_t stream, bool prepass_ran, brt_stats* st);

void view_key_of(const brt_ctx* ctx, const FrameParams& fp, uint32_t key[8]);
int32_t attach_tile_order(brt_ctx* ctx, DeviceCtx& dc, FrameParams& fp, hipStream_t stream, bool may_measure, uint32_t flags);
int32_t update_tile_order(brt_ctx* ctx, DeviceCtx& dc, const FrameParams& fp, hipStream_t stream);
int32_t prepass_order(brt_ctx* ctx, DeviceCtx& dc, const FrameParams& fp, const float* d_raster_rgba,
                      const float* d_raster_depth, float* d_out_tile, hipStream_t stream, uint32_t flags, bool* ran);
uint64_t tree_shape_hash(const EncodedScene& e);
void permute_scene(const std::vector<float>& pairs, const std::vector<float>& spheres, const std::vector<uint32_t>& sphmat,
                   const std::vector<float>& sphmats, uint32_t root, const std::vector<uint32_t>& rank, const std::vector<uint32_t>& srank,
                   std::vector<float>* out_pairs, std::vector<float>* out_spheres, std::vector<uint32_t>* out_sphmat,
                   std::vector<float>* out_sphmats, uint32_t* out_root);

void drain_all_streams(brt_ctx* ctx);
template <class Body>
int32_t with_tree_reach(brt_ctx* ctx, const void* camera80, uint32_t level, brt_stats* stats, Body&& body) {
    uint32_t rebuilt = 0u;
    int32_t rc = level != 0u ? ensure_tree_reach(ctx, camera80, &rebuilt) : BRT_OK;
    if (rc == BRT_OK) rc = body();
    if (rc != BRT_OK) drain_all_streams(ctx);
    else tree_stats(ctx, rebuilt, stats);
    return rc;
}
int32_t render_frame_device(brt_ctx* ctx, const void* camera80, const void* window16, uint32_t level, uint32_t width, uint32_t height,
                            const float* d_raster_rgba, const float* d_raster_depth, void* d_frame, void* hip_stream, uint32_t flags,
                            brt_stats* stats);

struct StreamPlan {
    DeviceSceneView scene;
    int scene_mode;
    uint32_t grid, block;
    size_t lds_bytes;
};
StreamPlan plan_stream(const brt_ctx* ctx, const DeviceCtx& dc, uint32_t n_items, uint32_t waves_by_hand, uint32_t waves_other);

struct PixelsTarget {
    void* d_out;
    bool scatter;
    uint32_t out_format;
};
int32_t pixels_enqueue(brt_ctx* ctx, DeviceCtx& dc, const void* camera80, const void* window16, uint32_t width, uint32_t height,
                       const uint32_t* d_pixels, uint32_t n_pixels, const uint32_t* d_count, const PixelsTarget& target, uint32_t* d_ctl,
                       hipStream_t stream, bool force_plain, PixelsLaunch* pl);

bool overlaps(const void* a, size_t a_bytes, const void* b, size_t b_bytes);
size_t out_bytes(uint32_t width, uint32_t height, uint32_t fmt);
int32_t refine_list(brt_ctx* ctx, DeviceCtx& dc, uint32_t width, uint32_t height, hipStream_t stream);

int32_t denoise_begin(brt_ctx* ctx, DeviceCtx& dc, const void* camera80, const void* window16, uint32_t width, uint32_t height,
                      hipStream_t stream, FrameParams* fp, DenoiseScratch* ds);
int32_t run_denoise(brt_ctx* ctx, DeviceCtx& dc, const FrameParams& fp, const DenoiseScratch& ds, const float* d_in, void* d_out,
                    uint32_t out_format, hipStream_t stream, uint32_t flags, const BlendPost& bp);
bool blend_post_on(uint32_t level, uint32_t flags);
int32_t post_flags_check(brt_ctx* ctx, uint32_t level, uint32_t flags);

}
```

bevyray_amd/csrc/brt_host.cpp:

```cpp
#include "brt_host.h"
#include "brt_ploc.h"
#include "brt_sah.h"
#include "brt_srgb_table.h"

#include <algorithm>
#include <cmath>
#include <cstring>
#include <limits>

namespace brt {

thread_local std::string g_last_error;

int32_t fail(int32_t code, const std::string& msg) {
    g_last_error = msg;
    return code;
}

int32_t guard_fail(std::string* ctx_error, int32_t code, const char* what) noexcept {
    auto put = [&](std::string& dst) noexcept {
        try {
            dst.assign(what ? what : "?");
        } catch (...) {
            try { dst.assign(code == BRT_ERR_OUT_OF_MEMORY ? "out of memory" : "internal error"); } catch (...) {}
        }
    };
    put(g_last_error);
    if (ctx_error) put(*ctx_error);
    return code;
}

void throw_for_test(uint32_t kind) {
    if (kind == 1u) throw std::bad_alloc();
    if (kind == 2u) throw std::logic_error("BRT_TEST_THROW: logic_error");
    throw 42;
}


int32_t validate_and_encode(const Model* models, uint32_t n_models, const Material* materials, uint32_t n_materials,
                            const BVHNode* nodes, uint32_t n_nodes, EncodedScene* out, std::string* err) {
    if (n_models == 0) { *err = "scene has no spheres (the reference skips the pass)"; return BRT_ERR_EMPTY_SCENE; }
    if (!models || !materials || n_materials == 0) { *err = "null models/materials"; return BRT_ERR_INVALID_ARGUMENT; }
    if (!nodes || n_nodes == 0) { *err = "null/empty BVH"; return BRT_ERR_INVALID_BVH; }
    if (n_models > DESC32_MAX_INDEX || n_nodes > DESC32_MAX_INDEX) { *err = "scene too large for 30-bit descriptors"; return BRT_ERR_UNSUPPORTED; }
    for (uint32_t i = 0; i < n_models; i++) {
        if (models[i].material_id >= n_materials) {
            *err = "model " + std::to_string(i) + ": material_id " + std::to_string(models[i].material_id) +
                   " >= n_materials " + std::to_string(n_materials);
            return BRT_ERR_INVALID_SCENE;
        }
    }

    std::vector<uint32_t> pair_id(n_nodes, 0xffffffffu);
    std::vector<uint8_t> seen(n_nodes, 0);
    std::vector<uint32_t> depth(n_nodes, 0);
    std::vector<uint32_t> order;
    order.reserve(n_nodes / 2 + 1);
    uint32_t max_leaf_depth = 0;
    uint32_t n_general_leaves = 0;

    auto leaf_check = [&](uint32_t n) -> bool {
        uint64_t end = (uint64_t)nodes[n].index + (uint64_t)nodes[n].model_count;
        return end <= (uint64_t)n_models;
    };

    std::vector<uint32_t> frontier{0};
    seen[0] = 1;
    size_t head = 0;
    while (head < frontier.size()) {
        uint32_t n = frontier[head++];
        const BVHNode& nd = nodes[n];
        if (nd.model_count > 0) {
            if (!leaf_check(n)) {
                *err = "BVH leaf " + std::to_string(n) + ": models [" + std::to_string(nd.index) + ", +" +
                       std::to_string(nd.model_count) + ") exceed n_models " + std::to_string(n_models);
                return BRT_ERR_INVALID_BVH;
            }
            max_leaf_depth = std::max(max_leaf_depth, depth[n]);
            if (nd.model_count > 1) n_general_leaves++;
            continue;
        }
        uint64_t c0 = nd.index, c1 = (uint64_t)nd.index + 1;
        if (c1 >= n_nodes) {
            *err = "BVH node " + std::to_string(n) + ": child index " + std::to_string(c1) + " >= n_nodes " + std::to_string(n_nodes);
            return BRT_ERR_INVALID_BVH;
        }
        if (seen[c0] || seen[c1]) {
            *err = "BVH node " + std::to_string(n) + ": child " + std::to_string(seen[c0] ? c0 : c1) +
                   " is reachable twice (cycle or shared subtree)";
            return BRT_ERR_INVALID_BVH;
        }
        seen[c0] = seen[c1] = 1;
        depth[c0] = depth[c1] = depth[n] + 1;
        pair_id[n] = (uint32_t)order.size();
        order.push_back(n);
        frontier.push_back((uint32_t)c0);
        frontier.push_back((uint32_t)c1);
    }

    EncodedScene& e = *out;
    e = EncodedScene();
    e.n_pairs = (uint32_t)order.size();
    if ((uint64_t)e.n_pairs * PAIR_UNITS > 0x7FFFFFFFull) { *err = "scene too large for 31-bit record offsets"; return BRT_ERR_UNSUPPORTED; }
    e.pairs.assign(pair_array_bytes(e.n_pairs) / 4, 0.0f);

    e.desc16 = (n_models <= DESC16_MAX_INDEX) && (e.n_pairs <= DESC16_MAX_INDEX) && (n_general_leaves <= DESC16_MAX_INDEX);
    const uint32_t LEAF = e.desc16 ? Desc<true>::LEAF : Desc<false>::LEAF;
    const uint32_t LEAF1 = e.desc16 ? Desc<true>::LEAF1 : Desc<false>::LEAF1;
    auto desc_of = [&](uint32_t n) -> uint32_t {
        const BVHNode& nd = nodes[n];
        if (nd.model_count == 0) return e.desc16 ? Desc<true>::interior(pair_id[n]) : Desc<false>::interior(pair_id[n]);
        if (nd.model_count == 1) return LEAF | LEAF1 | nd.index;
        uint32_t id = (uint32_t)(e.leaf_table.size() / 2);
        e.leaf_table.push_back(nd.index);
        e.leaf_table.push_back(nd.model_count);
        return LEAF | id;
    };

    e.root_desc = desc_of(0);
    e.boxes_ordered = true;
    for (uint32_t i = 0; i < e.n_pairs; i++) {
        const BVHNode& nd = nodes[order[i]];
        const BVHNode& L = nodes[nd.index];
        const BVHNode& R = nodes[nd.index + 1];
        float* rec = &e.pairs[(size_t)PAIR_WORDS * i];
        const uint32_t block[3] = {PAIR_X / 4, PAIR_Y / 4, PAIR_Z / 4};
        for (int k = 0; k < 3; k++) {
            float* g = rec + block[k];
            g[0] = L.bounds_min[k]; g[1] = R.bounds_min[k]; g[2] = L.bounds_max[k]; g[3] = R.bounds_max[k];
            g[4] = L.bounds_max[k]; g[5] = R.bounds_max[k]; g[6] = L.bounds_min[k]; g[7] = R.bounds_min[k];
            for (const BVHNode* c : {&L, &R})
                if (!(std::isfinite(c->bounds_min[k]) && std::isfinite(c->bounds_max[k]) && c->bounds_min[k] <= c->bounds_max[k]))
                    e.boxes_ordered = false;
        }
        const uint32_t dd[2] = {desc_of(nd.index), desc_of(nd.index + 1)};
        std::memcpy(rec + PAIR_DESC / 4, dd, sizeof dd);
    }

    e.n_models = n_models;
    e.spheres.resize(4 * (size_t)n_models);
    e.sphere_material.resize(n_models);
    for (uint32_t i = 0; i < n_models; i++) {
        e.spheres[4 * (size_t)i + 0] = models[i].position[0];
        e.spheres[4 * (size_t)i + 1] = models[i].position[1];
        e.spheres[4 * (size_t)i + 2] = models[i].position[2];
        e.spheres[4 * (size_t)i + 3] = models[i].radius * models[i].radius;
        e.sphere_material[i] = models[i].material_id;
    }
    e.n_materials = n_materials;
    e.materials.resize(8 * (size_t)n_materials);
    std::memcpy(e.materials.data(), materials, 32 * (size_t)n_materials);
    e.sphere_mats.resize(8 * (size_t)n_models);
    for (uint32_t i = 0; i < n_models; i++) std::memcpy(e.sphere_mats.data() + 8 * (size_t)i, &materials[models[i].material_id], 32);
    e.max_leaf_depth = max_leaf_depth;
    e.stack_entries = std::min<uint32_t>(32u, max_leaf_depth + 1u);
// ... 498 lines not shown
    return guard(nullptr, [&]() -> int32_t {
    if (!out_n_nodes) return fail(BRT_ERR_INVALID_ARGUMENT, "out_n_nodes is null");
    *out_n_nodes = 0;
    if (n_models == 0) return BRT_OK;
    if (!models) return fail(BRT_ERR_INVALID_ARGUMENT, "models is null");
    std::vector<BVHNode> nodes;
    int32_t rc = build_bvh_sah((const Model*)models, n_models, reach, &nodes);
    if (rc != BRT_OK) return rc;
    *out_n_nodes = (uint32_t)nodes.size();
    if (nodes.size() > capacity || !out_nodes)
        return fail(BRT_ERR_CAPACITY, "BVH needs " + std::to_string(nodes.size()) + " nodes, capacity " + std::to_string(capacity));
    std::memcpy(out_nodes, nodes.data(), nodes.size() * sizeof(BVHNode));
    return BRT_OK;
    });
}

int32_t brt_host_srgb_thresholds(float* out255) {
    return guard(nullptr, [&]() -> int32_t {
    if (!out255) return fail(BRT_ERR_INVALID_ARGUMENT, "null pointer");
    std::memcpy(out255, kSrgbThreshold, sizeof kSrgbThreshold);
    return BRT_OK;
    });
}

int32_t brt_host_tree_reach(const void* models, uint32_t n_models, const void* camera80, float* out_scene_scale, uint32_t* out_level,
                            float* out_reach) {
    return guard(nullptr, [&]() -> int32_t {
    if ((!models && n_models != 0u) || !camera80) return fail(BRT_ERR_INVALID_ARGUMENT, "null pointer");
    const TreeScene t = tree_scene_of((const Model*)models, n_models);
    Camera cam;
    std::memcpy(&cam, camera80, sizeof cam);
    uint32_t level = tree_level_for(t.scale, t.big, cam.position);
    if (tree_pads_equal(t, 0.0f, tree_reach_of(t.scale, level))) level = 0u;
    if (out_scene_scale) *out_scene_scale = t.scale;
    if (out_level) *out_level = level;
    if (out_reach) *out_reach = tree_reach_of(t.scale, level);
    return BRT_OK;
    });
}

int32_t brt_validate_scene(const void* models, uint32_t n_models, const void* materials, uint32_t n_materials,
                           const void* bvh_nodes, uint32_t n_nodes, uint32_t* out_max_depth) {
    return guard(nullptr, [&]() -> int32_t {
    EncodedScene e;
    std::string err;
    int32_t rc = validate_and_encode((const Model*)models, n_models, (const Material*)materials, n_materials,
                                     (const BVHNode*)bvh_nodes, n_nodes, &e, &err);
    if (rc != BRT_OK) return fail(rc, err);
    if (out_max_depth) *out_max_depth = e.max_leaf_depth;
    return BRT_OK;
    });
}

int32_t brt_scene_generate(uint32_t kind, uint64_t seed, void* out_models, void* out_materials, uint32_t capacity,
                           uint32_t* out_n_models) {
    return guard(nullptr, [&]() -> int32_t {
    if (!out_n_models) return fail(BRT_ERR_INVALID_ARGUMENT, "out_n_models is null");
    std::vector<Model> models;
    std::vector<Material> materials;
    int32_t rc = scene_generate(kind, seed, &models, &materials);
    if (rc != BRT_OK) return rc;
    *out_n_models = (uint32_t)models.size();
    if (models.size() > capacity || !out_models || !out_materials)
        return fail(BRT_ERR_CAPACITY, "scene has " + std::to_string(models.size()) + " spheres, capacity " + std::to_string(capacity));
    std::memcpy(out_models, models.data(), models.size() * sizeof(Model));
    std::memcpy(out_materials, materials.data(), materials.size() * sizeof(Material));
    return BRT_OK;
    });
}

int32_t brt_host_camera_extract(const float* t, const float* target, const float* up, float fov, float aspect_ratio,
                                float near_, float far_, uint32_t sample_count, uint32_t bounces, void* out_camera80) {
    return guard(nullptr, [&]() -> int32_t {
    if (!t || !target || !up || !out_camera80) return fail(BRT_ERR_INVALID_ARGUMENT, "null pointer");
    auto norm = [](float* v) { float l = std::sqrt(v[0] * v[0] + v[1] * v[1] + v[2] * v[2]); v[0] /= l; v[1] /= l; v[2] /= l; };
    float back[3] = {t[0] - target[0], t[1] - target[1], t[2] - target[2]};
    norm(back);
    float right[3] = {up[1] * back[2] - up[2] * back[1], up[2] * back[0] - up[0] * back[2], up[0] * back[1] - up[1] * back[0]};
    norm(right);
    float up2[3] = {back[1] * right[2] - back[2] * right[1], back[2] * right[0] - back[0] * right[2], back[0] * right[1] - back[1] * right[0]};
    Camera c;
    std::memset(&c, 0, sizeof c);
    c.sample_count = sample_count;
    c.bounce_count = bounces;
    c.projection_type = 0;
    c.near_ = near_; c.far_ = far_; c.fov = fov; c.aspect = aspect_ratio;
    for (int k = 0; k < 3; k++) { c.position[k] = t[k]; c.direction[k] = -back[k]; c.up[k] = up2[k]; }
    std::memcpy(out_camera80, &c, sizeof c);
    return BRT_OK;
    });
}

int32_t brt_host_window_extract(float random_seed, uint32_t physical_height, void* out_window16) {
    return guard(nullptr, [&]() -> int32_t {
    if (!out_window16) return fail(BRT_ERR_INVALID_ARGUMENT, "null pointer");
    Window w;
    std::memset(&w, 0, sizeof w);
    w.random_seed = random_seed;
    w.height = physical_height;
    std::memcpy(out_window16, &w, sizeof w);
    return BRT_OK;
    });
}

int32_t brt_host_material(const float* base_color_srgb3, float metallic, float perceptual_roughness, float reflectance,
                          float ior, float specular_transmission, void* out_material32) {
    return guard(nullptr, [&]() -> int32_t {
    if (!base_color_srgb3 || !out_material32) return fail(BRT_ERR_INVALID_ARGUMENT, "null pointer");
    StdMat m;
    for (int k = 0; k < 3; k++) m.base[k] = base_color_srgb3[k];
    m.metallic = metallic; m.perceptual_roughness = perceptual_roughness; m.reflectance = reflectance;
    m.ior = ior; m.specular_transmission = specular_transmission;
    Material r = prepare_asset(m);
    std::memcpy(out_material32, &r, sizeof r);
    return BRT_OK;
    });
}

int32_t brt_host_pixel_ray(const void* camera80, const void* window16, uint32_t width, uint32_t height, uint32_t px, uint32_t py,
                           void* out_ray32) {
    return guard(nullptr, [&]() -> int32_t {
    if (!camera80 || !window16 || !out_ray32) return fail(BRT_ERR_INVALID_ARGUMENT, "null pointer");
    if (width == 0 || height == 0 || width > 32768u || height > 32768u) return fail(BRT_ERR_INVALID_ARGUMENT, "width/height must be in [1, 32768]");
    if (px >= width || py >= height) return fail(BRT_ERR_INVALID_ARGUMENT, "pixel outside the frame");
    Camera cam;
    Window win;
    std::memcpy(&cam, camera80, sizeof cam);
    std::memcpy(&win, window16, sizeof win);
    const float heightf = (float)win.height;
    const float widthf = (float)win.height * cam.aspect;
    const float inv_width = 1.0f / widthf, inv_height = 1.0f / heightf;
    const float tan_half = tan_half_fov(cam.fov);
    const float* a = cam.direction;
    const float* b = cam.up;
    const float right[3] = {a[1] * b[2] - a[2] * b[1], a[2] * b[0] - a[0] * b[2], a[0] * b[1] - a[1] * b[0]};
    const float uvx = ((float)px + 0.5f) / (float)width;
    const float uvy = ((float)py + 0.5f) / (float)height;
    const float ndc_x = (uvx * 2.0f - 1.0f) + inv_width * 0.0f;
    const float ndc_y = (1.0f - uvy * 2.0f) + inv_height * 0.0f;
    const float sx = (ndc_x * cam.aspect) * tan_half;
    const float sy = ndc_y * tan_half;
    float v[3];
    for (int k = 0; k < 3; k++) v[k] = (a[k] + sx * right[k]) + sy * b[k];
    const float len = std::sqrt((v[0] * v[0] + v[1] * v[1]) + v[2] * v[2]);
    float ray[8] = {cam.position[0], cam.position[1], cam.position[2], std::numeric_limits<float>::infinity(),
                    v[0] / len, v[1] / len, v[2] / len, 0.0f};
    const uint32_t user = py * width + px;
    std::memcpy(&ray[7], &user, 4);
    std::memcpy(out_ray32, ray, sizeof ray);
    return BRT_OK;
    });
}

int32_t brt_host_tile_order(const uint32_t* ray_sum, const uint32_t* longest_pixel, uint32_t n_tiles, uint32_t sample_count,
                            uint64_t grid_lanes, uint32_t sorted, uint32_t lane_permille, uint32_t tiles_x, uint32_t dilate,
                            uint32_t split_tail, uint32_t* out_order, uint32_t* out_info5) {
    return guard(nullptr, [&]() -> int32_t {
    if (!ray_sum || !longest_pixel || !out_order || !out_info5) return fail(BRT_ERR_INVALID_ARGUMENT, "null pointer");
    if (dilate != 0u && (tiles_x == 0u || n_tiles % tiles_x != 0u)) return fail(BRT_ERR_INVALID_ARGUMENT, "dilate needs a tiles_x that divides n_tiles");
    TileOrderParams tp{};
    tp.sample_count = sample_count; tp.grid_lanes = grid_lanes; tp.sorted = sorted; tp.sky_slack_permille = 20;
    tp.lane_permille = lane_permille; tp.critical = 1; tp.tiles_x = tiles_x; tp.dilate_x = tp.dilate_y = dilate;
    tp.split_tail = split_tail;
    TileOrder to;
    build_tile_order(ray_sum, longest_pixel, n_tiles, tp, &to);
    std::memcpy(out_order, to.order.data(), to.order.size() * 4);
    out_info5[0] = to.n_lane; out_info5[1] = to.n_critical; out_info5[2] = to.longest_pixel;
    out_info5[3] = to.n_nonsky; out_info5[4] = to.n_split;
    return BRT_OK;
    });
}

}
```

bevyray_amd/csrc/brt_kernels.h:

```cpp
#pragma once
#include <hip/hip_runtime.h>

#include <cstddef>
#include <cstdint>

#include "brt_layout.h"

#define BRT_BLOCK 1024

#include "../../include/bevyray_amd.h"

namespace brt {

struct TraceLaunch {
    DeviceSceneView scene;
    FrameParams frame;
    uint32_t* queue_counter;
    float* out_tile;
    const float* raster_rgba;
    const float* raster_depth;
    unsigned long long* counters;
    int scene_mode;
    bool counters_on;
    int lean;
    uint32_t grid, block;
    size_t lds_bytes;
    hipStream_t stream;
};

size_t trace_lds_bytes(const DeviceSceneView& sv, int scene_mode, uint32_t block, uint32_t pool_cap, uint32_t hist_words = 0, bool rows = false);
constexpr uint32_t POOL_RECORD_BYTES = 96;
constexpr uint32_t WGQ_BYTES = 64;
hipError_t launch_trace_persistent(const TraceLaunch& tl);
hipError_t launch_trace_simple(const TraceLaunch& tl);
hipError_t launch_passthrough(const FrameParams& fp, float* out_tile, const float* raster_rgba, hipStream_t stream);
hipError_t launch_deinterleave(const float* tiles, void* frame, uint32_t width, uint32_t height, uint32_t n_parts,
                               uint32_t tile_rows, uint32_t out_format, hipStream_t stream, const uint32_t* part_of_strip = nullptr);
hipError_t launch_pack_strips(const float* frame, float* packed, uint32_t width, uint32_t height, uint32_t n_parts, uint32_t tile_rows,
                              uint32_t floats_per_pixel, hipStream_t stream);
hipError_t launch_debug_eval(uint32_t op, const float* in, float* out, uint32_t n, hipStream_t stream);

size_t order_scratch_bytes(uint32_t n_tiles);
hipError_t launch_build_order(const uint32_t* d_ray_sum, const uint32_t* d_longest, uint32_t n_tiles, uint64_t sky_cost,
                              uint64_t grid_lanes, uint32_t tiles_x, uint32_t dilate_x, uint32_t dilate_y, uint32_t split_tail,
                              uint32_t* d_order, uint32_t* d_meta, char* d_scratch, hipStream_t stream);

constexpr uint32_t kPlocOneBlockMax = 6000;
size_t ploc_scratch_bytes(uint32_t n, uint32_t* n_pow2_out, uint32_t one_block_max);
hipError_t launch_build_ploc(const Model* d_models, uint32_t n, char* d_scratch, BVHNode** d_out, uint32_t** d_info,
                             uint32_t one_block_max, hipStream_t stream);

size_t sah_scratch_bytes(uint32_t n);
hipError_t launch_build_sah(const Model* d_models, uint32_t n, float reach, char* d_scratch, BVHNode** d_out, uint32_t** d_info, hipStream_t stream);

}
```

bevyray_amd/csrc/brt_trace.h:

```cpp
#pragma once
#include <hip/hip_runtime.h>

#include <cstdlib>
#include <type_traits>

#include "brt_device.h"
#include "brt_kernels.h"

#ifndef BRT_PHASE_PRIO_AT
#define BRT_PHASE_PRIO_AT 2
#endif

namespace brt {

struct PixelCoord {
    uint32_t px, py;
    uint32_t local_row;
    uint32_t tile;
    uint32_t t;
    bool inside;
};
BRT_DEV uint32_t slot_tile(const FrameParams& fp, uint32_t slot_tile_index) {
    return fp.tile_order ? fp.tile_order[slot_tile_index] : slot_tile_index;
}
// ... 173 lines not shown
    return ended;
}

template <bool COUNTERS, int LEAN, bool TUNABLE>
BRT_DEV void shade_landed(const ScenePtrs& sc, const FrameParams& fp, bool landed, float t, uint32_t idx, PixelState& ps,
                          f3& o, f3& d, f3& tput, uint32_t& bounce, float& first_depth, bool& active, bool& need_cam,
                          uint32_t& n_rays, HitCounters& hc, float* out_tile, const float* raster_rgba,
                          const float* raster_depth) {
    const bool osc = TUNABLE && (fp.policy_flags & 1u);
    const bool sel = TUNABLE && (fp.policy_flags & 2u);
    const bool pw5 = TUNABLE && (fp.policy_flags & 4u);
    const bool hit = landed && t != kInf, sky = landed && t == kInf;
    prof_section<COUNTERS>(hc, SEC_SCATTER, hit);
    prof_section<COUNTERS>(hc, SEC_SKY, sky);
    auto end_sample = [&](f3 c) {
        ps.sum = ps.sum + sqrt3(c);
        if (!LEAN) ps.dsum = ps.dsum + (first_depth == kInf ? fp.fallback_far : first_depth);
        ps.sample++;
        bounce = 0;
        need_cam = true;
        if (ps.sample == ps.sample_end) {
            const uint32_t at_end = ps.tile >> kSliceShift, tile = ps.tile & kTileMask;
            if (at_end == kSliceFirst) {
                ps.tile |= kSliceDone << kSliceShift;
            } else {
                const uint32_t rays = n_rays - ps.rays_begin;
                pixel_finish<LEAN != 0>(fp, ps, out_tile, raster_rgba, raster_depth);
                if (fp.tile_cost) {
                    atomicAdd(&fp.tile_cost[tile], rays);
                    atomicMax(&fp.tile_cost[fp.local_strips * fp.tiles_x + tile], rays);
                }
            }
            active = false;
        }
    };
    if (!landed) return;
    n_rays++;
    if (bounce == 0) first_depth = t;
    f3 v1 = d;
    if (hit) {
        hc.hits++;
        const float4 s = sc.spheres[idx];
        o = mk3(o.x + t * d.x, o.y + t * d.y, o.z + t * d.z);
        v1 = mk3(o.x - s.x, o.y - s.y, o.z - s.z);
    }
    const f3 n1 = normalize3(v1);
    bool metal = false, glass = false, diffuse = false, absorbed = false;
    f3 att, acc;
    float ior, draw;
    if (hit) {
#if BRT_MAT_BY_SPHERE
        const float4 m0 = sc.sphere_mats[2 * idx];
        const float4 m1 = sc.sphere_mats[2 * idx + 1];
#else
        const uint32_t mid = sc.sphere_material[idx];
        const float4 m0 = sc.materials[2 * mid];
        const float4 m1 = sc.materials[2 * mid + 1];
#endif
        metal = rng_float(ps.rng) < m0.w;
        glass = !metal && (rng_float(ps.rng) < m1.w);
        diffuse = !metal && !glass;
        if (glass && !osc) draw = rng_float(ps.rng);
        ior = m1.z;
        att = glass ? mk3(1.0f, 1.0f, 1.0f) : mk3(m0.x, m0.y, m0.z);
        uint32_t need = metal ? 1u : (diffuse ? 2u : 0u);
        acc = diffuse ? n1 : mk3(-0.0f, -0.0f, -0.0f);
        float scale = diffuse ? 1.0f : m1.x;
        unsigned long long t_ball = 0;
        if (COUNTERS) t_ball = wall_clock64();
        if (BRT_BALL_ASM && !COUNTERS) {
            ball_loop_asm(ps.rng, acc, m1.x, __builtin_amdgcn_ballot_w64(diffuse), __builtin_amdgcn_ballot_w64(metal), &hc.asm_counts);
            need = 0u;
        }
        while (need != 0u) {
            if (COUNTERS) prof_section<COUNTERS>(hc, SEC_BALL, true);
            const float px = rng_ball_coord(ps.rng);
            const float py = rng_ball_coord(ps.rng);
            const float pz = rng_ball_coord(ps.rng);
            const f3 p = mk3(px, py, pz);
            const bool ok = dot3(p, p) <= 1.0f;
            const f3 cand = acc + scale * p;
            acc = mk3(ok ? cand.x : acc.x, ok ? cand.y : acc.y, ok ? cand.z : acc.z);
            scale = ok ? m1.x : scale;
            need -= ok ? 1u : 0u;
        }
        if (COUNTERS) {
            const uint64_t m = __ballot(true);
            if (mbcnt64(m) == 0u) hc.ticks_ball += wall_clock64() - t_ball;
        }
        if (diffuse) {
            const float eps = 1e-8f;
            if (__builtin_fabsf(acc.x) < eps && __builtin_fabsf(acc.y) < eps && __builtin_fabsf(acc.z) < eps) acc = n1;
            absorbed = dot3(acc, n1) < 0.0f;
        }
    }
    const bool limit = hit && bounce >= fp.bounce_count;
    const bool early = sky || (diffuse && (absorbed || limit)) || (glass && limit && !osc);
    bool cam = false;
    f3 cdir;
    if (early) {
        f3 c;
        if (sky) {
            const float a = 0.5f * (n1.y + 1.0f);
            const float b = 1.0f - a;
            c = tput * mk3(b * 1.0f + a * 0.5f, b * 1.0f + a * 0.7f, b * 1.0f + a * 1.0f);
        } else if (absorbed) {
            c = tput * mk3(0.0f, 0.0f, 0.0f);
        } else {
            c = mk3(0.0f, 0.0f, 0.0f);
        }
        end_sample(c);
        cam = active;
        if (cam) {
            prof_section<COUNTERS>(hc, SEC_CAMERA, true);
            cdir = camera_dir_raw(fp, ps.ndc0x, ps.ndc0y, ps.rng);
        }
    }
    const bool second = (metal || glass) && !early;
    if (second || cam) {
        const float dn = dot3(d, n1);
        f3 v2 = metal ? d - (2.0f * dn) * n1 : d;
        if (cam) v2 = cdir;
        const f3 u = normalize3(v2);
        if (cam) {
            d = u;
            need_cam = false;
        } else if (metal) {
            d = u + acc;
            absorbed = dot3(d, n1) < 0.0f;
        } else {
            const float ri = dn < 0.0f ? (1.0f / ior) : ior;
            const float cos_theta = sel ? min_sel(dot3(neg3(u), n1), 1.0f) : min_f(dot3(neg3(u), n1), 1.0f);
            const float sin_theta = __builtin_sqrtf(1.0f - cos_theta * cos_theta);
            const bool cannot_refract = ri * sin_theta > 1.0f;
            const float refl = schlick(cos_theta, ri, pw5);
            bool reflects = cannot_refract;
            if (osc) {
                if (!cannot_refract) reflects = refl > rng_float(ps.rng);
            } else {
                reflects = reflects || (refl > draw);
            }
            d = reflects ? reflect3(u, n1) : refract3(u, n1, ri, sel);
        }
    }
    if (hit && !early) {
        if (diffuse) d = acc;
        if (absorbed || limit) {
            f3 c = mk3(0.0f, 0.0f, 0.0f);
            if (absorbed) c = tput * c;
            end_sample(c);
        } else {
            tput = tput * att;
            bounce++;
        }
    }
}

BRT_DEV void pool_lock(uint32_t* ctl, uint32_t lane) {
    if (lane == 0)
        while (atomicCAS(&ctl[0], 0u, 1u) != 0u) __builtin_amdgcn_s_sleep(1);
    __builtin_amdgcn_fence(__ATOMIC_ACQUIRE, "workgroup");
}
BRT_DEV void pool_unlock(uint32_t* ctl, uint32_t lane) {
    __builtin_amdgcn_fence(__ATOMIC_RELEASE, "workgroup");
    if (lane == 0) atomicExch(&ctl[0], 0u);
}
BRT_DEV uint32_t pool_peek(const uint32_t* ctl, int i) { return __atomic_load_n(&ctl[i], __ATOMIC_RELAXED); }


#ifndef BRT_PRIO_TOP
#define BRT_PRIO_TOP 1
#endif
template <int MODE, bool D16, bool SIMPLE, bool COUNTERS, bool TUNABLE, int LEAN>
__global__ __launch_bounds__(BRT_BLOCK) void k_trace_persistent(DeviceSceneView sv, FrameParams fp,
                                                                uint32_t* __restrict__ queue_counter,
                                                                float* __restrict__ out_tile,
                                                                const float* __restrict__ raster_rgba,
                                                                const float* __restrict__ raster_depth,
                                                                unsigned long long* __restrict__ counters) {
    static_assert(MODE == SCENE_GLOBAL || D16, "a scene staged in LDS always uses 16-bit descriptors");
    static_assert(!LEAN || (!COUNTERS && !TUNABLE), "LEAN is a specialisation of the production timing kernel");
    using StackT = typename std::conditional<D16, int16_t, int32_t>::type;
    extern __shared__ uint4 smem[];
    ScenePtrs sc;
    StackT* stacks;
    sc.materials = reinterpret_cast<const float4*>(sv.materials);
    sc.sphere_mats = reinterpret_cast<const float4*>(sv.sphere_mats);
    sc.boxes_ordered = sv.boxes_ordered != 0u;
    sc.pairs_far = reinterpret_cast<const char*>(sv.pairs);
    sc.near_bytes = 0u;
    sc.near_base = 0u;
    sc.sph_base = 0u;
    sc.rows_scratch = 0u;
    sc.hits = nullptr;
    sc.minmax_select = TUNABLE && (fp.policy_flags & 2u) != 0u;
    if (MODE == SCENE_LDS) {
        const uint32_t pair_granules = (uint32_t)(pair_array_bytes(sv.n_pairs) / 16);
        float4* p = reinterpret_cast<float4*>(smem);
        float4* l_pairs = p; p += pair_granules;
        float4* l_sp = p; p += sv.n_models;
        uint2* p2 = reinterpret_cast<uint2*>(p);
        uint2* l_lt = p2; p2 += sv.n_leaf_table;
        uint32_t* p1 = reinterpret_cast<uint32_t*>(p2);
        uint32_t* l_sm = p1; p1 += BRT_MAT_BY_SPHERE ? 0u : sv.n_models;
        stacks = reinterpret_cast<StackT*>(p1);
        const float4* g_pairs = reinterpret_cast<const float4*>(sv.pairs);
        const float4* g_sp = reinterpret_cast<const float4*>(sv.spheres);
        const uint2* g_lt = reinterpret_cast<const uint2*>(sv.leaf_table);
        for (uint32_t i = threadIdx.x; i < pair_granules; i += blockDim.x) l_pairs[i] = g_pairs[i];
        for (uint32_t i = threadIdx.x; i < sv.n_models; i += blockDim.x) { l_sp[i] = g_sp[i]; if (!BRT_MAT_BY_SPHERE) l_sm[i] = sv.sphere_material[i]; }
        for (uint32_t i = threadIdx.x; i < sv.n_leaf_table; i += blockDim.x) l_lt[i] = g_lt[i];
        sc.pairs = reinterpret_cast<const char*>(l_pairs);
        sc.near_base = (uint32_t)(uintptr_t)(__attribute__((address_space(3))) char*)reinterpret_cast<char*>(l_pairs);
        sc.sph_base = (uint32_t)(uintptr_t)(__attribute__((address_space(3))) char*)reinterpret_cast<char*>(l_sp);
        sc.spheres = l_sp; sc.sphere_material = BRT_MAT_BY_SPHERE ? sv.sphere_material : l_sm; sc.leaf_table = l_lt;
    } else {
        sc.spheres = reinterpret_cast<const float4*>(sv.spheres);
        sc.sphere_material = sv.sphere_material;
        sc.leaf_table = reinterpret_cast<const uint2*>(sv.leaf_table);
        if (MODE == SCENE_LDS_TOP) {
            const uint32_t pair_granules = sv.lds_pairs * PAIR_UNITS;
            float4* l_pairs = reinterpret_cast<float4*>(smem);
            const float4* g_pairs = reinterpret_cast<const float4*>(sv.pairs);
            for (uint32_t i = threadIdx.x; i < pair_granules; i += blockDim.x) l_pairs[i] = g_pairs[i];
            sc.pairs = reinterpret_cast<const char*>(l_pairs);
            sc.near_bytes = sv.lds_pairs * PAIR_BYTES;
            sc.near_base = (uint32_t)(uintptr_t)(__attribute__((address_space(3))) char*)reinterpret_cast<char*>(l_pairs);
            stacks = reinterpret_cast<StackT*>(l_pairs + pair_granules);
        } else {
            sc.pairs = reinterpret_cast<const char*>(sv.pairs);
            stacks = reinterpret_cast<StackT*>(smem);
        }
    }
    const uint32_t lane = lane_id();
    const uint32_t wave = threadIdx.x >> 6;
    const uint32_t n_waves = blockDim.x >> 6;
    const uint32_t stack_col = D16 ? ((lane & 31u) * 2u + (lane >> 5)) : lane;
    StackT* stk = stacks + wave * ((sv.stack_entries + 2u) * 64u) + stack_col;
    char* const lds = reinterpret_cast<char*>(smem);
    uint32_t off = (uint32_t)(reinterpret_cast<char*>(stacks + n_waves * ((sv.stack_entries + 2u) * 64u)) - lds);
    off = (off + 15u) & ~15u;
    uint32_t* const wgq = reinterpret_cast<uint32_t*>(lds + off);
    off += WGQ_BYTES;
    if (MODE == SCENE_LDS && BRT_WALK_ROWS && fp.rows_on != 0u) {
        sc.rows_scratch = (uint32_t)(uintptr_t)(__attribute__((address_space(3))) char*)(lds + off) + wave * ROWS_SCRATCH_BYTES;
        off += n_waves * ROWS_SCRATCH_BYTES;
    }
    uint32_t* pool_ctl = nullptr;
    float4* pool = nullptr;
    if (fp.pool_cap != 0u) {
        pool_ctl = reinterpret_cast<uint32_t*>(lds + off);
        pool = reinterpret_cast<float4*>(lds + off + 16u);
        if (threadIdx.x == 0) { pool_ctl[0] = 0u; pool_ctl[1] = 0u; pool_ctl[2] = n_waves; pool_ctl[3] = 0u; }
    }
    constexpr bool kHits = TUNABLE && MODE == SCENE_LDS_TOP;
    uint32_t* hist = nullptr;
    if (kHits && fp.record_hits != nullptr) {
        if (fp.pool_cap != 0u) off += 16u + fp.pool_cap * POOL_RECORD_BYTES;
        hist = reinterpret_cast<uint32_t*>(lds + off);
        for (uint32_t i = threadIdx.x; i < sv.n_pairs; i += blockDim.x) hist[i] = 0u;
        sc.hits = hist;
    }
    if (threadIdx.x < WGQ_BYTES / 4u) wgq[threadIdx.x] = 0u;
    __syncthreads();
    const uint32_t wgq_batch = fp.wgq_batch >= 64u ? fp.wgq_batch : 64u;
    const uint32_t queue_lane = TUNABLE ? fp.queue_lane : 0u;
    const uint32_t refill_min = TUNABLE ? fp.refill_min : kRefillMin;
    const uint32_t walk_exit_lanes = TUNABLE ? fp.walk_exit_lanes : kWalkExitLanes;
    const uint32_t leaf_vote = TUNABLE ? fp.leaf_vote : kLeafVote;
    const uint32_t drain_donate = TUNABLE ? fp.drain_donate : kDrainDonate;
    const uint32_t pool_adopt = TUNABLE ? fp.pool_adopt : kPoolAdopt;
    const uint32_t crit_end = LEAN == 2 ? 0u : (fp.order_meta ? fp.order_meta[0] * 64u : fp.crit_end);
    constexpr bool kSlices = !COUNTERS;
    const uint32_t split_tiles = fp.slice_state ? (fp.order_meta ? fp.order_meta[3] : fp.split_tiles) : 0u;
    const uint32_t split_mid = (fp.order_meta ? fp.order_meta[2] : fp.split_nonsky) * 64u;
    const uint32_t split_lo = split_mid - split_tiles * 64u, split_hi = split_mid + split_tiles * 64u;
    const bool slices = kSlices && fp.sample_count >= 16u;
    const bool slice_b = LEAN == 0 || fp.tile_cost != nullptr;
    const uint32_t queue_size = fp.queue_size + split_tiles * 64u;

    PixelState ps;
    ps.sample = 0; ps.rng = 0; ps.out_index = 0; ps.frame_index = 0; ps.tile = 0; ps.rays_begin = 0;
    ps.ndc0x = ps.ndc0y = 0.0f; ps.sum = mk3(0.0f, 0.0f, 0.0f); ps.dsum = 0.0f; ps.sample_end = fp.sample_count;
    f3 o = mk3(0.0f, 0.0f, 0.0f), d = mk3(0.0f, 0.0f, 1.0f), tput = mk3(1.0f, 1.0f, 1.0f);
    uint32_t bounce = 0;
    float first_depth = kInf;
    bool active = false;
    bool exhausted = !TUNABLE;
    bool in_flight = false;
    bool need_cam = false;
    bool crit = false;
    bool wave_crit = false;
    WalkState<StackT> walk;
    walk.a = 0.0f; walk.inv = mk3(0.0f, 0.0f, 0.0f); walk.closest = kInf; walk.closest_idx = 0xffffffffu;
    walk.cur = Desc<D16>::DONE; walk.sp = stk; walk.n = 0;
    walk.ox = walk.oy = walk.oz = 0u;
    uint32_t n_rays = 0;
    HitCounters hc = {};
    unsigned long long t_start = 0, t_empty = 0, drain_lane_rounds = 0;
    unsigned long long t_mark = 0, ticks_refill = 0, ticks_walk = 0, ticks_shade = 0, ticks_pre = 0;
#ifdef BRT_LIFE_HIST
    unsigned long long lh_start = wall_clock64();
#endif
    if (COUNTERS) t_start = t_mark = wall_clock64();

    bool tiles_done = false;
    bool again_mark = false;
    auto slice_settle = [&]() {
        const bool done = kSlices && !active && (ps.tile >> kSliceShift) == kSliceDone;
        if (__ballot(done) == 0ull) return;
        if (done) {
            ps.tile &= ~kSliceFlagsMask;
            if (slice_store(fp, ps, n_rays - ps.rays_begin, slice_b)) {
                ps.sample_end = fp.sample_count;
                active = true;
            }
        }
    };
    auto begin_pixel = [&](uint32_t q, uint32_t tile) {
        const PixelCoord c = slot_to_pixel<TUNABLE>(fp, q, tile);
        const bool first_half = q >= split_lo && q < split_mid, second_half = q >= split_mid && q < split_hi;
        if (c.inside && !(second_half && !slices)) {
            pixel_begin(fp, c, ps);
            crit = q >= fp.crit_begin && q < crit_end;
            ps.rays_begin = n_rays;
            ps.sample_end = fp.sample_count;
            bool taken = true;
            if (slices && first_half) {
                ps.sample_end = slice_point(fp);
                ps.tile |= kSliceFirst << kSliceShift;
            } else if (slices && second_half) {
                uint32_t rays_before = 0u;
                taken = slice_load(fp, ps, &rays_before, slice_b);
                ps.rays_begin = n_rays - rays_before;
                const uint64_t tm = __ballot(taken), lm = __ballot(!taken);
                if (mbcnt64(tm | lm) == 0u) {
                    if (tm) atomicAdd(&counters[62], (unsigned long long)__popcll(tm));
                    if (lm) atomicAdd(&counters[63], (unsigned long long)__popcll(lm));
                }
            }
            if (fp.sample_count == 0) {
                asm volatile("" : "+v"(ps.sum.x), "+v"(ps.sum.y), "+v"(ps.sum.z), "+v"(ps.dsum));
                pixel_finish<LEAN != 0>(fp, ps, out_tile, raster_rgba, raster_depth);
            } else if (taken) { active = true; bounce = 0; need_cam = true; }
        }
    };

    for (;;) {
        if (split_tiles != 0u) slice_settle();
        if (crit_end != 0u) {
            const bool wc = __ballot(active && crit) != 0ull;
            if (wc != wave_crit) {
                wave_crit = wc;
                if (wc) __builtin_amdgcn_s_setprio(3); else __builtin_amdgcn_s_setprio(0);
            }
        }
        if (COUNTERS) { const unsigned long long now = wall_clock64(); ticks_shade += now - t_mark; t_mark = now; }
        while (TUNABLE) {
            const bool need = !active && !exhausted && !wave_crit;
            const uint64_t m = __ballot(need);
            if (m == 0) break;
            if ((uint32_t)__popcll(m) < refill_min && __ballot(active) != 0ull) break;
            const uint32_t n_need = (uint32_t)__popcll(m);
            const uint32_t rank = mbcnt64(m);
            uint32_t q = 0xffffffffu, tile = 0;
            bool none_left;
            {
                pool_lock(wgq, lane);
                uint32_t lo = pool_peek(wgq, 1), hi = pool_peek(wgq, 2), bbase = pool_peek(wgq, 3);
                bool done = pool_peek(wgq, 4) != 0u;
                if (lo == hi && !done) {
                    const uint32_t left = queue_lane > bbase ? queue_lane - bbase : 0u;
                    uint32_t batch = (left / (gridDim.x * 4u)) & ~63u;
                    batch = batch > wgq_batch ? wgq_batch : (batch < 64u ? 64u : batch);
                    if (bbase < crit_end) batch = 64u;
                    uint32_t b = 0;
                    if (lane == 0) b = atomicAdd(queue_counter, batch);
                    b = (uint32_t)__shfl((int)b, 0, 64);
                    bbase = b;
                    lo = b < queue_lane ? b : queue_lane;
                    hi = b + batch < queue_lane ? b + batch : queue_lane;
                    if (hi < lo) hi = lo;
                    done = lo == hi;
                    const uint32_t ti = (b >> 6) + lane;
                    if (lane < (batch >> 6) && ti < (queue_lane >> 6)) wgq[8u + lane] = slot_tile(fp, ti);
                    if (lane == 0) { wgq[2] = hi; wgq[3] = bbase; wgq[4] = done ? 1u : 0u; }
                }
                const uint32_t avail = hi - lo;
                const uint32_t take = n_need < avail ? n_need : avail;
                if (need && rank < take) {
                    q = lo + rank;
                    tile = wgq[8u + ((q - bbase) >> 6)];
                }
                if (lane == 0) wgq[1] = lo + take;
                none_left = done && take == 0u;
                pool_unlock(wgq, lane);
            }
            if (need) {
                if (none_left) {
                    exhausted = true;
                    if (COUNTERS && t_empty == 0) t_empty = wall_clock64();
                } else if (q != 0xffffffffu) {
                    begin_pixel(q, tile);
                }
            }
        }
        if (queue_lane != queue_size && !tiles_done && !wave_crit && __ballot(active) == 0ull &&
            __ballot(!exhausted) == 0ull) {
            uint32_t b = 0;
            if (lane == 0) b = atomicAdd(queue_counter + 1, 64u);
            b = queue_lane + (uint32_t)__shfl((int)b, 0, 64);
            if (b < queue_size) begin_pixel(b + lane, slot_tile(fp, b >> 6));
            else {
                tiles_done = true;
                if (COUNTERS && t_empty == 0) t_empty = wall_clock64();
            }
        }
        if (COUNTERS) { const unsigned long long now = wall_clock64(); ticks_refill += now - t_mark; t_mark = now; }
        bool finish_walks = false;
        if (fp.pool_cap != 0u && __ballot(exhausted) != 0ull && !wave_crit) {
            const uint64_t am = __ballot(active);
            uint32_t live = (uint32_t)__popcll(am);
            asm volatile("" : "+s"(live));
            const bool quiet = __ballot(in_flight) == 0ull;
            const bool thin = live != 0u && live <= drain_donate && !tiles_done;
            bool leave = false;
            if (live == 0u || (thin && quiet && pool_peek(pool_ctl, 2) > 1u) || (live <= pool_adopt && pool_peek(pool_ctl, 1) != 0u)) {
                pool_lock(pool_ctl, lane);
                const uint32_t count = pool_peek(pool_ctl, 1), alive = pool_peek(pool_ctl, 2);
                if (thin && quiet && alive > 1u && count + live <= fp.pool_cap) {
                    if (active) {
                        float4* rec = pool + 6u * (count + mbcnt64(am));
                        rec[0] = make_float4(ps.ndc0x, ps.ndc0y, ps.sum.x, ps.sum.y);
                        rec[1] = make_float4(ps.sum.z, ps.dsum, __uint_as_float(ps.rng), __uint_as_float(ps.sample));
                        rec[2] = make_float4(__uint_as_float(ps.out_index), __uint_as_float(ps.frame_index),
                                             __uint_as_float(ps.tile), __uint_as_float(n_rays - ps.rays_begin));
                        rec[3] = make_float4(o.x, o.y, o.z, d.x);
                        rec[4] = make_float4(d.y, d.z, tput.x, tput.y);
                        rec[5] = make_float4(tput.z, __uint_as_float(bounce), first_depth, __uint_as_float((crit ? 1u : 0u) | (need_cam ? 2u : 0u)));
                        active = false;
                    }
                    const bool stay = queue_lane != queue_size && !tiles_done;
                    if (lane == 0) { pool_ctl[1] = count + live; if (!stay) pool_ctl[2] = alive - 1u; }
                    leave = !stay;
                } else if (count != 0u && live < 64u) {
                    const uint64_t im = ~am;
                    const uint32_t idle = 64u - live;
                    const uint32_t k = idle < count ? idle : count;
                    const uint32_t r = mbcnt64(im);
                    if (!active && r < k) {
                        const float4* rec = pool + 6u * (count - k + r);
                        const float4 r0 = rec[0], r1 = rec[1], r2 = rec[2], r3 = rec[3], r4 = rec[4], r5 = rec[5];
                        ps.ndc0x = r0.x; ps.ndc0y = r0.y; ps.sum = mk3(r0.z, r0.w, r1.x); ps.dsum = r1.y;
                        ps.rng = __float_as_uint(r1.z); ps.sample = __float_as_uint(r1.w);
                        ps.out_index = __float_as_uint(r2.x); ps.frame_index = __float_as_uint(r2.y);
                        ps.tile = __float_as_uint(r2.z); ps.rays_begin = n_rays - __float_as_uint(r2.w);
                        ps.sample_end = (ps.tile >> kSliceShift) == kSliceFirst ? slice_point(fp) : fp.sample_count;
                        o = mk3(r3.x, r3.y, r3.z); d = mk3(r3.w, r4.x, r4.y); tput = mk3(r4.z, r4.w, r5.x);
                        bounce = __float_as_uint(r5.y); first_depth = r5.z;
                        crit = (__float_as_uint(r5.w) & 1u) != 0u; need_cam = (__float_as_uint(r5.w) & 2u) != 0u;
                        active = true; in_flight = false; exhausted = true;
                    }
                    if (lane == 0) pool_ctl[1] = count - k;
                } else if (live == 0u && count == 0u && (queue_lane == queue_size || tiles_done)) {
                    if (lane == 0) pool_ctl[2] = alive - 1u;
                    leave = true;
                }
                pool_unlock(pool_ctl, lane);
            }
            if (leave) break;
            finish_walks = wave_count(active) <= drain_donate && !tiles_done;
        } else if (__ballot(active) == 0 && (queue_lane == queue_size || tiles_done || __ballot(!exhausted) != 0ull)) {
            break;
        }
        if (__ballot(active) == 0) continue;

        bool again;
        do {
        if (COUNTERS && again_mark) { const unsigned long long now = wall_clock64(); ticks_shade += now - t_mark; t_mark = now; }
        prof_section<COUNTERS>(hc, SEC_ROUND, active);
        if (COUNTERS && __ballot(exhausted) != 0ull) drain_lane_rounds += (unsigned long long)__popcll(__ballot(active)) | (1ull << 32);
        const bool fresh = active && !in_flight;
        constexpr int kPhasePrio = (MODE == SCENE_LDS || BRT_PRIO_TOP) ? BRT_PHASE_PRIO_AT : 0;
        if (kPhasePrio == 2 && !wave_crit) __builtin_amdgcn_s_setprio(1);
        prof_section<COUNTERS>(hc, SEC_CAMERA_TOP, fresh && need_cam);
        if (fresh && bounce == 0) {
            o = mk3(fp.cam_pos[0], fp.cam_pos[1], fp.cam_pos[2]);
            tput = mk3(1.0f, 1.0f, 1.0f);
            first_depth = kInf;
            if (need_cam) {
                d = camera_ray_dir(fp, ps.ndc0x, ps.ndc0y, ps.rng);
                need_cam = false;
            }
        }
        if (fresh) walk_begin<D16>(walk, sc, sv.root_desc, stk, d);
        if (COUNTERS) { const unsigned long long now = wall_clock64(); ticks_pre += now - t_mark; t_mark = now; }
        if (kPhasePrio == 1 && !wave_crit) __builtin_amdgcn_s_setprio(1);
        if (active) walk_run<64, COUNTERS, D16, SIMPLE, MODE, StackT, kHits, TUNABLE, LEAN != 2>(sc, walk, stk, o, d, finish_walks ? 0u : walk_exit_lanes, leaf_vote, hc);
        in_flight = active && walk_pending<D16, SIMPLE>(walk);
        if (COUNTERS) { const unsigned long long now = wall_clock64(); ticks_walk += now - t_mark; t_mark = now; }
        const bool landed = active && !in_flight;
        const float t = walk.closest;
        const uint32_t idx = walk.closest_idx;
        if (kPhasePrio != 0 && !wave_crit) __builtin_amdgcn_s_setprio(0);
        shade_landed<COUNTERS, LEAN, TUNABLE>(sc, fp, landed, t, idx, ps, o, d, tput, bounce, first_depth, active, need_cam, n_rays, hc,
                                              out_tile, raster_rgba, raster_depth);
        again_mark = true;
        {
            const uint32_t live_now = wave_count(active);
            bool mgmt = live_now == 0u || (crit_end != 0u && (__ballot(active && crit) != 0ull) != wave_crit) ||
                        (TUNABLE && __ballot(!active && !exhausted) != 0ull);
            const bool pooled = fp.pool_cap != 0u && !wave_crit && (!TUNABLE || __ballot(exhausted) != 0ull);
            if (!mgmt && pooled && live_now <= pool_adopt)
                mgmt = (live_now <= drain_donate && !tiles_done && __ballot(in_flight) == 0ull && pool_peek(pool_ctl, 2) > 1u) ||
                       pool_peek(pool_ctl, 1) != 0u;
            finish_walks = pooled && live_now <= drain_donate && !tiles_done;
            again = __builtin_amdgcn_readfirstlane(mgmt ? 0 : 1) != 0;
        }
        } while (again);
        again_mark = false;
    }

    if (kHits && hist != nullptr) {
        __syncthreads();
        for (uint32_t i = threadIdx.x; i < sv.n_pairs; i += blockDim.x) {
            const uint32_t c = hist[i];
            if (c != 0u) atomicAdd(&fp.record_hits[i], c);
        }
    }
    const uint32_t r = wave_sum(n_rays);
    if (lane == 0) atomicAdd(&counters[0], (unsigned long long)r);
#if BRT_ASM_COUNT
    if (!COUNTERS) {
        const AsmCounts& c = hc.asm_counts;
        const uint32_t v[12] = {wave_sum(c.int_exec), wave_sum(c.int_lanes), wave_sum(c.leaf_exec), wave_sum(c.leaf_lanes), wave_sum(c.ball_exec), wave_sum(c.ball_lanes),
                                wave_sum(c.fix_int_lanes), wave_sum(c.fix_leaf_lanes), wave_sum(c.rows_int_exec), wave_sum(c.rows_calls), wave_sum(c.rows_cycles), wave_sum(c.wide_cycles)};
        if (lane == 0) {
            for (int k = 0; k < 6; k++) atomicAdd(&counters[33 + k], (unsigned long long)v[k]);
            atomicAdd(&counters[39], (unsigned long long)v[6]);
            atomicAdd(&counters[43], (unsigned long long)v[7]);
            atomicAdd(&counters[44], (unsigned long long)v[8]);
            atomicAdd(&counters[5], (unsigned long long)v[9]);
            atomicAdd(&counters[6], (unsigned long long)v[10]);
            atomicAdd(&counters[7], (unsigned long long)v[11]);
        }
    }
#endif
    if (COUNTERS) {
        const uint32_t a = wave_sum(hc.node_pops), b = wave_sum(hc.interior), c = wave_sum(hc.sphere_tests);
        if (lane == 0) {
            atomicAdd(&counters[1], (unsigned long long)a);
            atomicAdd(&counters[2], (unsigned long long)b);
            atomicAdd(&counters[3], (unsigned long long)c);
        }
    }
#ifdef BRT_LIFE_HIST
    if (!COUNTERS && lane == 0) {
        const unsigned long long lh_end = wall_clock64();
        atomicMax(&counters[24], ~lh_start);
        atomicMax(&counters[27], lh_end);
        atomicAdd(&counters[29], 1ull);
        atomicAdd(&counters[45], lh_end - lh_start);
        const unsigned long long bin = (lh_end - lh_start) >> 13;
        if (bin >= 88ull && bin < 152ull) atomicAdd(&counters[46 + ((bin - 88ull) >> 2)], 1ull << (16 * ((bin - 88ull) & 3ull)));
    }
#endif
    if (COUNTERS) {
        const unsigned long long t_end = wall_clock64();
        unsigned long long te = 0;
        for (int l = 0; l < 64; l++) {
            const unsigned long long v = __shfl(t_empty, l, 64);
            if (v != 0 && (te == 0 || v < te)) te = v;
        }
        if (lane == 0) {
            atomicMax(&counters[24], ~t_start);
            if (te) { atomicMax(&counters[25], ~te); atomicMax(&counters[26], te); atomicAdd(&counters[28], t_end - te); }
            atomicMax(&counters[27], t_end);
            atomicAdd(&counters[29], 1ull);
            atomicAdd(&counters[45], t_end - t_start);
            {
                const unsigned long long bin = (t_end - t_start) >> 15;
                if (bin < 64ull) atomicAdd(&counters[46 + (bin >> 2)], 1ull << (16 * (bin & 3ull)));
            }
            atomicAdd(&counters[30], drain_lane_rounds & 0xffffffffull);
            atomicAdd(&counters[31], drain_lane_rounds >> 32);
            atomicAdd(&counters[5], ticks_refill);
            atomicAdd(&counters[6], ticks_walk);
            atomicAdd(&counters[7], ticks_shade + (t_end - t_mark));
            atomicAdd(&counters[43], ticks_pre);
        }
    }
    if (COUNTERS) {
        unsigned long long tb = hc.ticks_ball;
        for (int off = 32; off > 0; off >>= 1) tb += __shfl_down(tb, off, 64);
        if (lane == 0) atomicAdd(&counters[44], tb);
    }
    if (COUNTERS) {
        const uint32_t h = wave_sum(hc.hits);
        if (lane == 0) atomicAdd(&counters[4], (unsigned long long)h);
        for (int k = 0; k < 8; k++) {
            const uint32_t e = wave_sum(hc.sec_exec[k]), l = wave_sum(hc.sec_lanes[k]);
            if (lane == 0) {
                atomicAdd(&counters[8 + 2 * k], (unsigned long long)e);
                atomicAdd(&counters[9 + 2 * k], (unsigned long long)l);
            }
        }
    }
}


template <int MODE, bool D, bool S, bool C, bool T, int LEAN = 0>
static hipError_t launch_persistent_t(const TraceLaunch& tl) {
    auto kern = k_trace_persistent<MODE, D, S, C, T, LEAN>;
    if (MODE == SCENE_LDS || MODE == SCENE_LDS_TOP) {
        static const size_t static_lds = [&] {
            hipFuncAttributes at{};
            return hipFuncGetAttributes(&at, reinterpret_cast<const void*>(kern)) == hipSuccess ? at.sharedSizeBytes : (size_t)1;
        }();
        if (static_lds != 0) return hipErrorInvalidConfiguration;
    }
    hipError_t e = hipFuncSetAttribute(reinterpret_cast<const void*>(kern), hipFuncAttributeMaxDynamicSharedMemorySize,
                                       (int)tl.lds_bytes);
    if (e != hipSuccess) return e;
    hipLaunchKernelGGL(kern, dim3(tl.grid), dim3(tl.block), tl.lds_bytes, tl.stream, tl.scene, tl.frame, tl.queue_counter,
                       tl.out_tile, tl.raster_rgba, tl.raster_depth, tl.counters);
    return hipGetLastError();
}

template <int MODE, bool D, bool T>
static hipError_t launch_persistent_md(const TraceLaunch& tl) {
    if constexpr (!T && MODE != SCENE_GLOBAL) {
        if (tl.lean && tl.scene.simple_tree && !tl.counters_on)
            return tl.lean == 2 ? launch_persistent_t<MODE, D, true, false, false, 2>(tl) : launch_persistent_t<MODE, D, true, false, false, 1>(tl);
    }
    if (tl.scene.simple_tree)
        return tl.counters_on ? launch_persistent_t<MODE, D, true, true, T>(tl) : launch_persistent_t<MODE, D, true, false, T>(tl);
    return tl.counters_on ? launch_persistent_t<MODE, D, false, true, T>(tl) : launch_persistent_t<MODE, D, false, false, T>(tl);
}

template <bool T>
static hipError_t launch_persistent_all(const TraceLaunch& tl) {
    switch (tl.scene_mode) {
        case SCENE_LDS:
            if (!tl.scene.desc16) return hipErrorInvalidValue;
            return launch_persistent_md<SCENE_LDS, true, T>(tl);
        case SCENE_LDS_TOP:
            if (!tl.scene.desc16) return hipErrorInvalidValue;
            return launch_persistent_md<SCENE_LDS_TOP, true, T>(tl);
        default:
            return tl.scene.desc16 ? launch_persistent_md<SCENE_GLOBAL, true, T>(tl) : launch_persistent_md<SCENE_GLOBAL, false, T>(tl);
    }
}

}
```

include/bevyray_amd.h:

```cpp
#ifndef BEVYRAY_AMD_H
#define BEVYRAY_AMD_H

#include <stdint.h>

#ifdef __cplusplus
extern "C" {
#endif

#define BRT_ABI_VERSION 6u

#define BRT_STRIP_ROWS 8u

enum {
    BRT_OK = 0,
    BRT_ERR_INVALID_ARGUMENT = -1,
    BRT_ERR_NO_DEVICE = -2,
    BRT_ERR_HIP = -3,
    BRT_ERR_INVALID_BVH = -4,
    BRT_ERR_INVALID_SCENE = -5,
    BRT_ERR_EMPTY_SCENE = -6,
    BRT_ERR_NO_SCENE = -7,
    BRT_ERR_UNSUPPORTED = -8,
    BRT_ERR_CAPACITY = -9,
    BRT_ERR_RCCL = -10,
// ... 55 lines not shown
int32_t brt_create(const int32_t* device_ids, int32_t n_devices, brt_ctx** out_ctx);
int32_t brt_destroy(brt_ctx* ctx);

enum { BRT_POLICY_OR_SHORT_CIRCUIT = 1u, BRT_POLICY_MINMAX_SELECT = 2u, BRT_POLICY_POW_EXP2_LOG2 = 4u };
int32_t brt_set_policy(brt_ctx* ctx, uint32_t flags);

int32_t brt_set_tuning(brt_ctx* ctx, const char* name, uint32_t value);
int32_t brt_get_tuning(const brt_ctx* ctx, const char* name, uint32_t* out_value, uint32_t* out_default);

int32_t brt_upload_scene(brt_ctx* ctx,
                         const void* models, uint32_t n_models,
                         const void* materials, uint32_t n_materials,
                         const void* bvh_nodes, uint32_t n_nodes);

int32_t brt_render(brt_ctx* ctx, const void* camera80, const void* window16, uint32_t level,
                   uint32_t width, uint32_t height,
                   const float* raster_rgba, const float* raster_depth,
                   float* out_rgba, uint32_t flags, brt_stats* stats_or_null);

int32_t brt_host_alloc(brt_ctx* ctx, uint64_t bytes, void** out_ptr);
int32_t brt_host_free(brt_ctx* ctx, void* ptr);

int32_t brt_render_part_device(brt_ctx* ctx, const void* camera80, const void* window16, uint32_t level,
                               uint32_t width, uint32_t height, uint32_t part, uint32_t n_parts,
                               const float* d_raster_rgba, const float* d_raster_depth,
                               float* d_out_tile, void* hip_stream, uint32_t flags,
                               brt_stats* stats_or_null);

int32_t brt_render_device(brt_ctx* ctx, const void* camera80, const void* window16, uint32_t level,
                          uint32_t width, uint32_t height,
                          const float* d_raster_rgba, const float* d_raster_depth,
                          void* d_frame, void* hip_stream, uint32_t flags, brt_stats* stats_or_null);

uint32_t brt_tile_rows(uint32_t height, uint32_t n_parts);

int32_t brt_deinterleave_device(brt_ctx* ctx, const float* d_tiles, uint32_t n_parts,
                                uint32_t width, uint32_t height, void* d_frame, void* hip_stream, uint32_t flags);

int32_t brt_set_strip_table(brt_ctx* ctx, uint32_t n_parts, uint32_t n_strips, const uint32_t* part_of_strip);
int32_t brt_plan_strips(brt_ctx* ctx, const void* camera80, const void* window16, uint32_t level, uint32_t width, uint32_t height,
                        uint32_t n_parts, uint32_t probe_spp, uint32_t* out_part_of_strip);
int32_t brt_host_plan_strips(const uint64_t* strip_cost, uint32_t n_strips, uint32_t n_parts, uint32_t* out_part_of_strip);

int32_t brt_rccl_unique_id(void* out_id128);
int32_t brt_rccl_comm_create(brt_ctx* ctx, const void* id128, int32_t rank, int32_t world, void** out_comm);
int32_t brt_rccl_comm_destroy(brt_ctx* ctx, void* comm);
int32_t brt_gather_rccl(brt_ctx* ctx, void* nccl_comm, int32_t rank, int32_t world, const float* d_tile, float* d_tiles_on_root,
                        uint32_t width, uint32_t height, void* d_frame_on_root, void* hip_stream, uint32_t flags);

enum { BRT_EXTMEM_OPAQUE_FD = 1, BRT_EXTMEM_DMABUF_FD = 2 };
int32_t brt_import_frame_fd(brt_ctx* ctx, int32_t fd, uint64_t bytes, uint32_t handle_type, void** out_d_frame);
int32_t brt_release_frame(brt_ctx* ctx, void* d_frame);
int32_t brt_debug_export_frame_fd(brt_ctx* ctx, uint64_t bytes, int32_t* out_fd, void** out_d_ptr);
int32_t brt_debug_copy_to_host(brt_ctx* ctx, const void* d_src, void* h_dst, uint64_t bytes);

enum {
    BRT_DBG_MINMAX = 0,
    BRT_DBG_SQRT_DIV = 1,
    BRT_DBG_RNG = 2,
    BRT_DBG_SLAB = 3,
    BRT_DBG_SPHERE = 4,
    BRT_DBG_SEED = 5,
    BRT_DBG_DIV = 6,
    BRT_DBG_DIV_SWEEP = 7,
    BRT_DBG_SQRT_SWEEP = 8,
    BRT_DBG_ENCODE = 9
};
int32_t brt_debug_eval(brt_ctx* ctx, uint32_t op, const float* in16, float* out8, uint32_t n);

int32_t brt_set_denoise(brt_ctx* ctx, uint32_t iterations, float sigma_luminance, float sigma_normal, float sigma_depth);
int32_t brt_denoise_device(brt_ctx* ctx, const void* camera80, const void* window16, uint32_t width, uint32_t height,
                           const float* d_frame_rgba, void* d_out, void* hip_stream, uint32_t flags, brt_stats* stats_or_null);
int32_t brt_debug_denoise_guides(brt_ctx* ctx, const void* camera80, const void* window16, uint32_t width, uint32_t height, float* out8);

int32_t brt_blend_post_device(brt_ctx* ctx, const void* camera80, const void* window16, uint32_t width, uint32_t height,
                              const float* d_coverage_rgba, const float* d_raster_rgba_or_null, void* d_out, void* hip_stream,
                              uint32_t flags, brt_stats* stats_or_null);

int32_t brt_set_temporal(brt_ctx* ctx, uint32_t max_history);
int32_t brt_reset_temporal(brt_ctx* ctx);
int32_t brt_debug_temporal_state(brt_ctx* ctx, uint32_t width, uint32_t height, float* out8);

#define BRT_QUERY_CLOSEST 0u
#define BRT_QUERY_ANY 1u
#define BRT_QUERY_STATUS_MISS 0u
#define BRT_QUERY_STATUS_HIT 1u
#define BRT_QUERY_STATUS_FRONT_FACE 2u
#define BRT_QUERY_STATUS_INVALID 4u
#define BRT_QUERY_STATUS_OUT_OF_REACH 8u
#define BRT_QUERY_NONE 4294967295u
int32_t brt_query_rays_device(brt_ctx* ctx, const void* d_rays, uint32_t n_rays, uint32_t mode, float origin_bound, void* d_hits,
                              void* hip_stream, uint32_t flags, uint64_t* out_stats8_or_null);
int32_t brt_query_rays(brt_ctx* ctx, const void* rays, uint32_t n_rays, uint32_t mode, float origin_bound, void* hits,
                       uint64_t* out_stats8_or_null);
int32_t brt_query_origin_bound(brt_ctx* ctx, float* out_bound);
int32_t brt_host_pixel_ray(const void* camera80, const void* window16, uint32_t width, uint32_t height, uint32_t px, uint32_t py,
                           void* out_ray32);

int32_t brt_upscale_device(brt_ctx* ctx, const void* camera80, const void* window16, uint32_t low_width, uint32_t low_height,
                           const float* d_low_rgba, uint32_t width, uint32_t height, void* d_out, void* hip_stream, uint32_t flags,
                           brt_stats* stats_or_null);
int32_t brt_render_upscaled_device(brt_ctx* ctx, const void* camera80, const void* window16, uint32_t low_width, uint32_t low_height,
                                   uint32_t width, uint32_t height, void* d_frame, void* hip_stream, uint32_t flags,
                                   brt_stats* stats_or_null);
int32_t brt_host_upscale_window(const void* window16, uint32_t height, uint32_t low_height, void* out_window16);

int32_t brt_upscale_blend_device(brt_ctx* ctx, const void* camera80, const void* window16, uint32_t level, uint32_t low_width,
                                 uint32_t low_height, const float* d_low_rgba, uint32_t width, uint32_t height,
                                 const float* d_raster_rgba_or_null, const float* d_raster_depth_or_null, void* d_out, void* hip_stream,
                                 uint32_t flags, brt_stats* stats_or_null);
int32_t brt_render_upscaled_blend_device(brt_ctx* ctx, const void* camera80, const void* window16, uint32_t level, uint32_t low_width,
                                         uint32_t low_height, uint32_t width, uint32_t height, const float* d_raster_rgba_or_null,
                                         const float* d_raster_depth_or_null, void* d_frame, void* hip_stream, uint32_t flags,
                                         brt_stats* stats_or_null);
int32_t brt_host_blend_covered(const void* camera80, uint32_t level, float t, float raster_depth, uint32_t* out_covered);

int32_t brt_render_pixels_device(brt_ctx* ctx, const void* camera80, const void* window16, uint32_t width, uint32_t height,
                                 const uint32_t* d_pixels, uint32_t n_pixels, float* d_out_rgba32f, void* hip_stream, uint32_t flags,
                                 brt_stats* stats_or_null);
int32_t brt_render_pixels(brt_ctx* ctx, const void* camera80, const void* window16, uint32_t width, uint32_t height, const uint32_t* pixels,
                          uint32_t n_pixels, float* out_rgba32f, uint32_t flags, brt_stats* stats_or_null);

#define BRT_REFINE_EDGES 1u
#define BRT_REFINE_SPECULAR 2u
int32_t brt_upscale_refine_device(brt_ctx* ctx, const void* camera80, const void* window16, uint32_t low_width, uint32_t low_height,
                                  const float* d_low_rgba, uint32_t width, uint32_t height, void* d_out, uint32_t classes,
                                  uint32_t* d_refined_count_or_null, void* hip_stream, uint32_t flags, brt_stats* stats_or_null);
int32_t brt_render_upscaled_refined_device(brt_ctx* ctx, const void* camera80, const void* window16, uint32_t low_width,
                                           uint32_t low_height, uint32_t width, uint32_t height, void* d_frame, uint32_t classes,
                                           uint32_t* d_refined_count_or_null, void* hip_stream, uint32_t flags, brt_stats* stats_or_null);
int32_t brt_upscale_refine_mask_device(brt_ctx* ctx, const void* camera80, const void* window16, uint32_t low_width, uint32_t low_height,
                                       const float* d_low_rgba, uint32_t width, uint32_t height, void* d_mask_u8, void* hip_stream,
                                       uint32_t flags);

#define BRT_ADAPT_SPARSE 1u
#define BRT_ADAPT_NOISY 2u
int32_t brt_set_adaptive(brt_ctx* ctx, uint32_t base_spp, float threshold, uint32_t min_taps);
int32_t brt_render_adaptive_device(brt_ctx* ctx, const void* camera80, const void* window16, uint32_t width, uint32_t height, void* d_frame,
                                   uint32_t* d_selected_count_or_null, void* hip_stream, uint32_t flags, brt_stats* stats_or_null);
int32_t brt_adaptive_refine_device(brt_ctx* ctx, const void* camera80, const void* window16, uint32_t width, uint32_t height,
                                   const float* d_base_rgba, void* d_out, uint32_t* d_selected_count_or_null, void* hip_stream,
                                   uint32_t flags, brt_stats* stats_or_null);
int32_t brt_adaptive_mask_device(brt_ctx* ctx, const void* camera80, const void* window16, uint32_t width, uint32_t height,
                                 const float* d_base_rgba, void* d_mask_u8, void* hip_stream, uint32_t flags);
int32_t brt_host_adaptive_class(float t, uint32_t material_id, const float* rgb, const uint32_t* taps_inside25, const uint32_t* taps_id25,
                                const float* taps_rgb75, float threshold, uint32_t min_taps, uint32_t* out_class);

int32_t brt_debug_profile(brt_ctx* ctx, uint64_t* out64);

int32_t brt_debug_tile_order(brt_ctx* ctx, const uint32_t* ray_sum, const uint32_t* longest_pixel, uint32_t n_tiles,
                             uint32_t sample_count, uint64_t grid_lanes, uint32_t tiles_x, uint32_t dilate, uint32_t split_tail,
                             uint32_t* out_order, uint32_t* out_info4);


int32_t brt_host_tile_order(const uint32_t* ray_sum, const uint32_t* longest_pixel, uint32_t n_tiles, uint32_t sample_count,
                            uint64_t grid_lanes, uint32_t sorted, uint32_t lane_permille, uint32_t tiles_x, uint32_t dilate,
                            uint32_t split_tail, uint32_t* out_order, uint32_t* out_info5);

int32_t brt_build_bvh(const void* models, uint32_t n_models,
                      void* out_nodes, uint32_t capacity, uint32_t* out_n_nodes);

int32_t brt_build_bvh_sah(const void* models, uint32_t n_models, float reach,
                          void* out_nodes, uint32_t capacity, uint32_t* out_n_nodes);

int32_t brt_host_tree_reach(const void* models, uint32_t n_models, const void* camera80, float* out_scene_scale, uint32_t* out_level,
                            float* out_reach);

int32_t brt_build_bvh_device(brt_ctx* ctx, const void* models, uint32_t n_models,
                             void* out_nodes, uint32_t capacity, uint32_t* out_n_nodes, double* out_build_ms);

int32_t brt_build_bvh_sah_device(brt_ctx* ctx, const void* models, uint32_t n_models, float reach,
                                 void* out_nodes, uint32_t capacity, uint32_t* out_n_nodes, double* out_build_ms);

int32_t brt_host_srgb_thresholds(float* out255);

int32_t brt_validate_scene(const void* models, uint32_t n_models,
                           const void* materials, uint32_t n_materials,
                           const void* bvh_nodes, uint32_t n_nodes, uint32_t* out_max_depth);

enum {
    BRT_SCENE_COVER = 0,
    BRT_SCENE_RTIOW_FINAL = 1,
    BRT_SCENE_STRESS_GRID = 2
};
int32_t brt_scene_generate(uint32_t kind, uint64_t seed,
                           void* out_models, void* out_materials, uint32_t capacity,
                           uint32_t* out_n_models);

int32_t brt_host_camera_extract(const float* translation3, const float* target3, const float* up3,
                                float fov, float aspect_ratio, float near_, float far_,
                                uint32_t sample_count, uint32_t bounces, void* out_camera80);
int32_t brt_host_window_extract(float random_seed, uint32_t physical_height, void* out_window16);
int32_t brt_host_material(const float* base_color_srgb3, float metallic, float perceptual_roughness,
                          float reflectance, float ior, float specular_transmission,
                          void* out_material32);

#ifdef __cplusplus
}
#endif
#endif
```

integration/bevyray_amd_sys/src/lib.rs:

```rust
#![allow(non_camel_case_types)]
use std::os::raw::{c_char, c_void};

pub const BRT_ABI_VERSION: u32 = 6;
pub const BRT_STRIP_ROWS: u32 = 8;

pub const BRT_OK: i32 = 0;
pub const BRT_ERR_INVALID_ARGUMENT: i32 = -1;
pub const BRT_ERR_NO_DEVICE: i32 = -2;
pub const BRT_ERR_HIP: i32 = -3;
pub const BRT_ERR_INVALID_BVH: i32 = -4;
pub const BRT_ERR_INVALID_SCENE: i32 = -5;
pub const BRT_ERR_EMPTY_SCENE: i32 = -6;
pub const BRT_ERR_NO_SCENE: i32 = -7;
pub const BRT_ERR_UNSUPPORTED: i32 = -8;
pub const BRT_ERR_CAPACITY: i32 = -9;
pub const BRT_ERR_RCCL: i32 = -10;
pub const BRT_ERR_OUT_OF_MEMORY: i32 = -11;
pub const BRT_ERR_INTERNAL: i32 = -12;

pub const BRT_LEVEL_SKIP: u32 = 0;
pub const BRT_LEVEL_FALLBACK_RASTER: u32 = 1;
pub const BRT_LEVEL_FALLBACK_RAYTRACED: u32 = 2;
pub const BRT_LEVEL_PURE: u32 = 3;

// ... 42 lines not shown
pub const BRT_DBG_DIV: u32 = 6;
pub const BRT_DBG_DIV_SWEEP: u32 = 7;
pub const BRT_DBG_SQRT_SWEEP: u32 = 8;
pub const BRT_DBG_ENCODE: u32 = 9;

#[repr(C)]
pub struct brt_ctx { _private: [u8; 0] }

#[repr(C)]
#[derive(Default, Debug, Clone, Copy)]
pub struct brt_stats {
    pub rays: u64,
    pub node_pops: u64,
    pub interior_visits: u64,
    pub sphere_tests: u64,
    pub hits: u64,
    pub paths: u64,
    pub kernel_ms: f64,
    pub gather_ms: f64,
    pub total_ms: f64,
    pub lds_bytes: u32,
    pub scene_in_lds: u32,
    pub n_workgroups: u32,
    pub threads_per_workgroup: u32,
    pub prepass_ms: f64,
    pub kernel_variant: u32,
    pub measured_tile_costs: u32,
    pub tree_rebuilt: u32,
    pub tree_reach: f32,
    pub forwarded_bytes: u64,
    pub hot_records: u32,
    pub reserved: u32,
}

extern "C" {
    pub fn brt_abi_version() -> u32;
    pub fn brt_last_error(ctx: *const brt_ctx) -> *const c_char;
    pub fn brt_create(device_ids: *const i32, n_devices: i32, out_ctx: *mut *mut brt_ctx) -> i32;
    pub fn brt_destroy(ctx: *mut brt_ctx) -> i32;
    pub fn brt_set_policy(ctx: *mut brt_ctx, flags: u32) -> i32;
    pub fn brt_set_tuning(ctx: *mut brt_ctx, name: *const c_char, value: u32) -> i32;
    pub fn brt_get_tuning(ctx: *const brt_ctx, name: *const c_char, out_value: *mut u32, out_default: *mut u32) -> i32;
    pub fn brt_upload_scene(ctx: *mut brt_ctx, models: *const c_void, n_models: u32, materials: *const c_void,
                            n_materials: u32, bvh_nodes: *const c_void, n_nodes: u32) -> i32;
    pub fn brt_render(ctx: *mut brt_ctx, camera80: *const c_void, window16: *const c_void, level: u32, width: u32,
                      height: u32, raster_rgba: *const f32, raster_depth: *const f32, out_rgba: *mut f32,
                      flags: u32, stats_or_null: *mut brt_stats) -> i32;
    pub fn brt_host_alloc(ctx: *mut brt_ctx, bytes: u64, out_ptr: *mut *mut c_void) -> i32;
    pub fn brt_host_free(ctx: *mut brt_ctx, ptr: *mut c_void) -> i32;
    pub fn brt_render_part_device(ctx: *mut brt_ctx, camera80: *const c_void, window16: *const c_void, level: u32,
                                  width: u32, height: u32, part: u32, n_parts: u32, d_raster_rgba: *const f32,
                                  d_raster_depth: *const f32, d_out_tile: *mut f32, hip_stream: *mut c_void,
                                  flags: u32, stats_or_null: *mut brt_stats) -> i32;
    pub fn brt_render_device(ctx: *mut brt_ctx, camera80: *const c_void, window16: *const c_void, level: u32,
                             width: u32, height: u32, d_raster_rgba: *const f32, d_raster_depth: *const f32,
                             d_frame: *mut c_void, hip_stream: *mut c_void, flags: u32,
                             stats_or_null: *mut brt_stats) -> i32;
    pub fn brt_tile_rows(height: u32, n_parts: u32) -> u32;
    pub fn brt_deinterleave_device(ctx: *mut brt_ctx, d_tiles: *const f32, n_parts: u32, width: u32, height: u32,
                                   d_frame: *mut c_void, hip_stream: *mut c_void, flags: u32) -> i32;
    pub fn brt_set_strip_table(ctx: *mut brt_ctx, n_parts: u32, n_strips: u32, part_of_strip: *const u32) -> i32;
    pub fn brt_plan_strips(ctx: *mut brt_ctx, camera80: *const c_void, window16: *const c_void, level: u32,
                           width: u32, height: u32, n_parts: u32, probe_spp: u32, out_part_of_strip: *mut u32) -> i32;
    pub fn brt_host_plan_strips(strip_cost: *const u64, n_strips: u32, n_parts: u32, out_part_of_strip: *mut u32) -> i32;
    pub fn brt_rccl_unique_id(out_id128: *mut c_void) -> i32;
    pub fn brt_rccl_comm_create(ctx: *mut brt_ctx, id128: *const c_void, rank: i32, world: i32,
                                out_comm: *mut *mut c_void) -> i32;
    pub fn brt_rccl_comm_destroy(ctx: *mut brt_ctx, comm: *mut c_void) -> i32;
    pub fn brt_gather_rccl(ctx: *mut brt_ctx, nccl_comm: *mut c_void, rank: i32, world: i32, d_tile: *const f32,
                           d_tiles_on_root: *mut f32, width: u32, height: u32, d_frame_on_root: *mut c_void,
                           hip_stream: *mut c_void, flags: u32) -> i32;
    pub fn brt_import_frame_fd(ctx: *mut brt_ctx, fd: i32, bytes: u64, handle_type: u32,
                               out_d_frame: *mut *mut c_void) -> i32;
    pub fn brt_release_frame(ctx: *mut brt_ctx, d_frame: *mut c_void) -> i32;
    pub fn brt_debug_export_frame_fd(ctx: *mut brt_ctx, bytes: u64, out_fd: *mut i32, out_d_ptr: *mut *mut c_void) -> i32;
    pub fn brt_debug_copy_to_host(ctx: *mut brt_ctx, d_src: *const c_void, h_dst: *mut c_void, bytes: u64) -> i32;
    pub fn brt_debug_eval(ctx: *mut brt_ctx, op: u32, in16: *const f32, out8: *mut f32, n: u32) -> i32;
    pub fn brt_set_denoise(ctx: *mut brt_ctx, iterations: u32, sigma_luminance: f32, sigma_normal: f32,
                           sigma_depth: f32) -> i32;
    pub fn brt_denoise_device(ctx: *mut brt_ctx, camera80: *const c_void, window16: *const c_void, width: u32,
                              height: u32, d_frame_rgba: *const f32, d_out: *mut c_void, hip_stream: *mut c_void,
                              flags: u32, stats_or_null: *mut brt_stats) -> i32;
    pub fn brt_debug_denoise_guides(ctx: *mut brt_ctx, camera80: *const c_void, window16: *const c_void,
                                    width: u32, height: u32, out8: *mut f32) -> i32;
    pub fn brt_blend_post_device(ctx: *mut brt_ctx, camera80: *const c_void, window16: *const c_void, width: u32,
                                 height: u32, d_coverage_rgba: *const f32, d_raster_rgba_or_null: *const f32,
                                 d_out: *mut c_void, hip_stream: *mut c_void, flags: u32,
                                 stats_or_null: *mut brt_stats) -> i32;
    pub fn brt_set_temporal(ctx: *mut brt_ctx, max_history: u32) -> i32;
    pub fn brt_reset_temporal(ctx: *mut brt_ctx) -> i32;
    pub fn brt_debug_temporal_state(ctx: *mut brt_ctx, width: u32, height: u32, out8: *mut f32) -> i32;
    pub fn brt_query_rays_device(ctx: *mut brt_ctx, d_rays: *const c_void, n_rays: u32, mode: u32,
                                 origin_bound: f32, d_hits: *mut c_void, hip_stream: *mut c_void, flags: u32,
                                 out_stats8_or_null: *mut u64) -> i32;
    pub fn brt_query_rays(ctx: *mut brt_ctx, rays: *const c_void, n_rays: u32, mode: u32, origin_bound: f32,
                          hits: *mut c_void, out_stats8_or_null: *mut u64) -> i32;
    pub fn brt_query_origin_bound(ctx: *mut brt_ctx, out_bound: *mut f32) -> i32;
    pub fn brt_host_pixel_ray(camera80: *const c_void, window16: *const c_void, width: u32, height: u32, px: u32,
                              py: u32, out_ray32: *mut c_void) -> i32;
    pub fn brt_upscale_device(ctx: *mut brt_ctx, camera80: *const c_void, window16: *const c_void, low_width: u32,
                              low_height: u32, d_low_rgba: *const f32, width: u32, height: u32, d_out: *mut c_void,
                              hip_stream: *mut c_void, flags: u32, stats_or_null: *mut brt_stats) -> i32;
    pub fn brt_render_upscaled_device(ctx: *mut brt_ctx, camera80: *const c_void, window16: *const c_void,
                                      low_width: u32, low_height: u32, width: u32, height: u32,
                                      d_frame: *mut c_void, hip_stream: *mut c_void, flags: u32,
                                      stats_or_null: *mut brt_stats) -> i32;
    pub fn brt_host_upscale_window(window16: *const c_void, height: u32, low_height: u32, out_window16: *mut c_void) -> i32;
    pub fn brt_upscale_blend_device(ctx: *mut brt_ctx, camera80: *const c_void, window16: *const c_void,
                                    level: u32, low_width: u32, low_height: u32, d_low_rgba: *const f32,
                                    width: u32, height: u32, d_raster_rgba_or_null: *const f32,
                                    d_raster_depth_or_null: *const f32, d_out: *mut c_void,
                                    hip_stream: *mut c_void, flags: u32, stats_or_null: *mut brt_stats) -> i32;
    pub fn brt_render_upscaled_blend_device(ctx: *mut brt_ctx, camera80: *const c_void, window16: *const c_void,
                                            level: u32, low_width: u32, low_height: u32, width: u32, height: u32,
                                            d_raster_rgba_or_null: *const f32, d_raster_depth_or_null: *const f32,
                                            d_frame: *mut c_void, hip_stream: *mut c_void, flags: u32,
                                            stats_or_null: *mut brt_stats) -> i32;
    pub fn brt_host_blend_covered(camera80: *const c_void, level: u32, t: f32, raster_depth: f32,
                                  out_covered: *mut u32) -> i32;
    pub fn brt_render_pixels_device(ctx: *mut brt_ctx, camera80: *const c_void, window16: *const c_void, width: u32,
                                    height: u32, d_pixels: *const u32, n_pixels: u32, d_out_rgba32f: *mut f32,
                                    hip_stream: *mut c_void, flags: u32, stats_or_null: *mut brt_stats) -> i32;
    pub fn brt_render_pixels(ctx: *mut brt_ctx, camera80: *const c_void, window16: *const c_void, width: u32,
                             height: u32, pixels: *const u32, n_pixels: u32, out_rgba32f: *mut f32, flags: u32,
                             stats_or_null: *mut brt_stats) -> i32;
    pub fn brt_upscale_refine_device(ctx: *mut brt_ctx, camera80: *const c_void, window16: *const c_void,
                                     low_width: u32, low_height: u32, d_low_rgba: *const f32, width: u32, height: u32,
                                     d_out: *mut c_void, classes: u32, d_refined_count_or_null: *mut u32,
                                     hip_stream: *mut c_void, flags: u32, stats_or_null: *mut brt_stats) -> i32;
    pub fn brt_render_upscaled_refined_device(ctx: *mut brt_ctx, camera80: *const c_void, window16: *const c_void,
                                              low_width: u32, low_height: u32, width: u32, height: u32,
                                              d_frame: *mut c_void, classes: u32, d_refined_count_or_null: *mut u32,
                                              hip_stream: *mut c_void, flags: u32, stats_or_null: *mut brt_stats) -> i32;
    pub fn brt_upscale_refine_mask_device(ctx: *mut brt_ctx, camera80: *const c_void, window16: *const c_void,
                                          low_width: u32, low_height: u32, d_low_rgba: *const f32, width: u32,
                                          height: u32, d_mask_u8: *mut c_void, hip_stream: *mut c_void, flags: u32) -> i32;
    pub fn brt_set_adaptive(ctx: *mut brt_ctx, base_spp: u32, threshold: f32, min_taps: u32) -> i32;
    pub fn brt_render_adaptive_device(ctx: *mut brt_ctx, camera80: *const c_void, window16: *const c_void, width: u32,
                                      height: u32, d_frame: *mut c_void, d_selected_count_or_null: *mut u32,
                                      hip_stream: *mut c_void, flags: u32, stats_or_null: *mut brt_stats) -> i32;
    pub fn brt_adaptive_refine_device(ctx: *mut brt_ctx, camera80: *const c_void, window16: *const c_void, width: u32,
                                      height: u32, d_base_rgba: *const f32, d_out: *mut c_void,
                                      d_selected_count_or_null: *mut u32, hip_stream: *mut c_void, flags: u32,
                                      stats_or_null: *mut brt_stats) -> i32;
    pub fn brt_adaptive_mask_device(ctx: *mut brt_ctx, camera80: *const c_void, window16: *const c_void, width: u32,
                                    height: u32, d_base_rgba: *const f32, d_mask_u8: *mut c_void, hip_stream: *mut c_void,
                                    flags: u32) -> i32;
    pub fn brt_host_adaptive_class(t: f32, material_id: u32, rgb: *const f32, taps_inside25: *const u32, taps_id25: *const u32,
                                   taps_rgb75: *const f32, threshold: f32, min_taps: u32, out_class: *mut u32) -> i32;
    pub fn brt_debug_profile(ctx: *mut brt_ctx, out64: *mut u64) -> i32;
    pub fn brt_debug_tile_order(ctx: *mut brt_ctx, ray_sum: *const u32, longest_pixel: *const u32, n_tiles: u32,
                                sample_count: u32, grid_lanes: u64, tiles_x: u32, dilate: u32, split_tail: u32,
                                out_order: *mut u32, out_info4: *mut u32) -> i32;
    pub fn brt_host_tile_order(ray_sum: *const u32, longest_pixel: *const u32, n_tiles: u32, sample_count: u32,
                               grid_lanes: u64, sorted: u32, lane_permille: u32, tiles_x: u32, dilate: u32,
                               split_tail: u32, out_order: *mut u32, out_info5: *mut u32) -> i32;
    pub fn brt_build_bvh(models: *const c_void, n_models: u32, out_nodes: *mut c_void, capacity: u32,
                         out_n_nodes: *mut u32) -> i32;
    pub fn brt_build_bvh_sah(models: *const c_void, n_models: u32, reach: f32, out_nodes: *mut c_void,
                             capacity: u32, out_n_nodes: *mut u32) -> i32;
    pub fn brt_host_tree_reach(models: *const c_void, n_models: u32, camera80: *const c_void,
                               out_scene_scale: *mut f32, out_level: *mut u32, out_reach: *mut f32) -> i32;
    pub fn brt_build_bvh_device(ctx: *mut brt_ctx, models: *const c_void, n_models: u32, out_nodes: *mut c_void,
                                capacity: u32, out_n_nodes: *mut u32, out_build_ms: *mut f64) -> i32;
    pub fn brt_build_bvh_sah_device(ctx: *mut brt_ctx, models: *const c_void, n_models: u32, reach: f32,
                                    out_nodes: *mut c_void, capacity: u32, out_n_nodes: *mut u32,
                                    out_build_ms: *mut f64) -> i32;
    pub fn brt_host_srgb_thresholds(out255: *mut f32) -> i32;
    pub fn brt_validate_scene(models: *const c_void, n_models: u32, materials: *const c_void, n_materials: u32,
                              bvh_nodes: *const c_void, n_nodes: u32, out_max_depth: *mut u32) -> i32;
    pub fn brt_scene_generate(kind: u32, seed: u64, out_models: *mut c_void, out_materials: *mut c_void,
                              capacity: u32, out_n_models: *mut u32) -> i32;
    pub fn brt_host_camera_extract(translation3: *const f32, target3: *const f32, up3: *const f32, fov: f32,
                                   aspect_ratio: f32, near_: f32, far_: f32, sample_count: u32, bounces: u32,
                                   out_camera80: *mut c_void) -> i32;
    pub fn brt_host_window_extract(random_seed: f32, physical_height: u32, out_window16: *mut c_void) -> i32;
    pub fn brt_host_material(base_color_srgb3: *const f32, metallic: f32, perceptual_roughness: f32,
                             reflectance: f32, ior: f32, specular_transmission: f32, out_material32: *mut c_void) -> i32;
}

pub unsafe fn last_error(ctx: *const brt_ctx) -> String {
    let p = brt_last_error(ctx);
    if p.is_null() { String::new() } else { std::ffi::CStr::from_ptr(p).to_string_lossy().into_owned() }
}
```

Before: 34890.

## Precompute sky-only tiles via frustum-sphere separation and shade them without traversal

Adds a prepass kernel that builds a conservative pyramid for each 8x8 tile and tests it against every sphere. Tiles proven to see no geometry are marked in a cached bitmap, keyed on view, scene epoch and camera. In lean trace mode, marked tiles take a short path that evaluates the sky gradient per sample and skips BVH traversal, cutting wasted traversal work and queue imbalance. The cost is an extra kernel, a bitmap lookup per queue claim, and reuse of the raster_depth argument slot to carry the bitmap in lean variants, which relies on lean mode never reading raster depth.

```diff
diff --git a/bevyray_amd/_lib.py b/bevyray_amd/_lib.py
--- a/bevyray_amd/_lib.py
+++ b/bevyray_amd/_lib.py
@@ -123,6 +123,8 @@
     "brt_host_camera_extract": (_I32, [C.POINTER(_F), C.POINTER(_F), C.POINTER(_F), _F, _F, _F, _F, _U32, _U32, _VP]),
     "brt_host_window_extract": (_I32, [_F, _U32, _VP]),
     "brt_host_material": (_I32, [C.POINTER(_F), _F, _F, _F, _F, _F, _VP]),
+    "brt_debug_sky_tiles": (_I32, [_VP, _VP, _U32, _VP, C.POINTER(_U32)]),
+    "brt_host_sky_tile": (_I32, [_VP, _U32, _VP, _VP, _U32, _U32, _U32, _U32, _F, _VP, _U32]),
     "brt_host_tile_order": (_I32, [_VP, _VP, _U32, _U32, C.c_uint64, _U32, _U32, _U32, _U32, _U32, _VP, _VP]),
 }
 EXPORTS = tuple(_PROTOTYPES)
diff --git a/bevyray_amd/csrc/brt_api.cpp b/bevyray_amd/csrc/brt_api.cpp
--- a/bevyray_amd/csrc/brt_api.cpp
+++ b/bevyray_amd/csrc/brt_api.cpp
@@ -14,7 +14,7 @@
 void free_device(DeviceCtx& dc) {
     if (hipSetDevice(dc.device) != hipSuccess) return;
     for (void* p : std::initializer_list<void*>{dc.d_scene, dc.d_ctrl, dc.d_strip_table, dc.d_tile, dc.d_gather, dc.d_pack, dc.d_raster_rgba,
-             dc.d_raster_depth, dc.d_bvh_scratch, dc.d_tile_cost, dc.d_tile_order, dc.d_order_meta, dc.d_order_scratch, dc.d_slice_state,
+             dc.d_raster_depth, dc.d_bvh_scratch, dc.d_tile_cost, dc.d_tile_order, dc.d_order_meta, dc.d_sky_bits, dc.d_order_scratch, dc.d_slice_state,
              dc.d_record_hits, dc.d_bvh_models, dc.d_denoise, dc.d_temporal, dc.d_tsph, dc.d_uplow, dc.d_qctl, dc.d_qmap, dc.d_qrays, dc.d_qhits,
              dc.d_pxbuf, dc.d_pxlist, dc.d_pxout})
         if (p) (void)hipFree(p);
diff --git a/bevyray_amd/csrc/brt_api_launch.cpp b/bevyray_amd/csrc/brt_api_launch.cpp
--- a/bevyray_amd/csrc/brt_api_launch.cpp
+++ b/bevyray_amd/csrc/brt_api_launch.cpp
@@ -153,6 +153,13 @@
                     LaunchPlan* plan_out) {
     HIP_TRY(ctx, hipStreamWaitEvent(stream, dc.ev_last, 0));
     HIP_TRY(ctx, hipMemsetAsync(dc.d_ctrl, 0, 512, stream));
+    const bool lean1 = fp.level == 3u && !fp.tunable && !(flags & (BRT_FLAG_COUNTERS | BRT_FLAG_KERNEL_SIMPLE)) && ctx->knobs[K_NO_LEAN] == 0u &&
+                       (fp.tile_cost == nullptr || ctx->knobs[K_LEAN_MEASURE] != 0u);
+    const uint32_t* d_sky_bits = nullptr;
+    if (lean1) {
+        const int32_t rc = attach_sky_tiles(ctx, dc, fp, stream, &d_sky_bits);
+        if (rc != BRT_OK) return rc;
+    }
     if (timed) HIP_TRY(ctx, hipEventRecord(dc.ev0, stream));
     LaunchPlan lp{};
     if (fp.level == 0u) {
@@ -181,12 +188,11 @@
                 const bool known = dc.view_rays != 0 && std::memcmp(key, dc.view_key, sizeof key) == 0;
                 const uint64_t per_lane = known ? dc.view_rays / ((uint64_t)dc.num_cus * BRT_BLOCK) : 0;
                 const uint64_t longest_bound = (uint64_t)fp.sample_count * ((uint64_t)fp.bounce_count + 1u);
-                const bool lean1 = !tl.frame.tunable && fp.level == 3u && !tl.counters_on && ctx->knobs[K_NO_LEAN] == 0u &&
-                                   (fp.tile_cost == nullptr || ctx->knobs[K_LEAN_MEASURE] != 0u);
                 tl.lean = !lean1 ? 0 : ((known && longest_bound < per_lane / 2) ? 2 : 1);
                 lp.variant = (uint32_t)tl.lean | (tl.frame.tunable ? 16u : 0u);
                 lp.measured = fp.tile_cost != nullptr ? 1u : 0u;
             }
+            tl.sky_bits = d_sky_bits;
             tl.scene_mode = lp.scene_mode;
             tl.scene.lds_pairs = lp.lds_pairs;
             tl.grid = lp.grid;
diff --git a/bevyray_amd/csrc/brt_api_order.cpp b/bevyray_amd/csrc/brt_api_order.cpp
--- a/bevyray_amd/csrc/brt_api_order.cpp
+++ b/bevyray_amd/csrc/brt_api_order.cpp
@@ -193,6 +193,37 @@
     return BRT_OK;
 }
 
+SkyCamera sky_camera_of(const FrameParams& fp) {
+    SkyCamera c{};
+    for (int k = 0; k < 3; k++) { c.pos[k] = fp.cam_pos[k]; c.dir[k] = fp.cam_dir[k]; c.up[k] = fp.cam_up[k]; c.right[k] = fp.cam_right[k]; }
+    c.aspect = fp.aspect; c.tan_half_fov = fp.tan_half_fov; c.inv_width = fp.inv_width; c.inv_height = fp.inv_height;
+    c.width = fp.width; c.height = fp.height;
+    return c;
+}
+int32_t attach_sky_tiles(brt_ctx* ctx, DeviceCtx& dc, const FrameParams& fp, hipStream_t stream, const uint32_t** d_bits) {
+    *d_bits = nullptr;
+    if (ctx->knobs[K_SKY_TILES] == 0u) return BRT_OK;
+    const uint32_t n_tiles = fp.local_strips * fp.tiles_x;
+    uint32_t key[7];
+    order_key_of(ctx, fp, key);
+    key[6] = ctx->scene_epoch;
+    const SkyCamera cam = sky_camera_of(fp);
+    if (!dc.sky_valid || std::memcmp(key, dc.sky_key, sizeof key) != 0 || std::memcmp(&cam, &dc.sky_cam, sizeof cam) != 0) {
+        dc.sky_valid = false;
+        int32_t rc = ensure(ctx, &dc.d_sky_bits, &dc.sky_bits_cap, (size_t)sky_bitmap_words(n_tiles) * 4u);
+        if (rc != BRT_OK) return rc;
+        SkyFrame sf{};
+        sf.cam = cam;
+        sf.tiles_x = fp.tiles_x; sf.n_tiles = n_tiles; sf.part = fp.part; sf.n_parts = fp.n_parts; sf.strip_of = fp.strip_of;
+        HIP_TRY(ctx, launch_sky_tiles(sf, dc.view.spheres, dc.view.n_models, dc.d_sky_bits, stream));
+        std::memcpy(dc.sky_key, key, sizeof key);
+        dc.sky_cam = cam;
+        dc.sky_valid = true;
+    }
+    *d_bits = dc.d_sky_bits;
+    return BRT_OK;
+}
+
 int32_t update_tile_order(brt_ctx* ctx, DeviceCtx& dc, const FrameParams& fp, hipStream_t stream) {
     if (!fp.tile_cost) return BRT_OK;
     const uint32_t n_tiles = fp.local_strips * fp.tiles_x;
@@ -463,6 +494,28 @@
     ctx->strip_epoch++;
     ctx->strip_part = table;
     ctx->strip_n_parts = n_parts;
+    return BRT_OK;
+    });
+}
+
+int32_t brt_debug_sky_tiles(brt_ctx* ctx, uint32_t* out_bits, uint32_t n_words, uint32_t* out_cost_or_null, uint32_t* out_n_tiles) {
+    return guard(ctx ? &ctx->last_error : nullptr, [&]() -> int32_t {
+    if (!ctx) return fail(BRT_ERR_INVALID_ARGUMENT, "ctx is null");
+    if (!out_bits || !out_n_tiles) return ctx_fail(ctx, BRT_ERR_INVALID_ARGUMENT, "null pointer");
+    DeviceCtx& dc = ctx->devs[0];
+    *out_n_tiles = 0u;
+    if (!dc.sky_valid) return BRT_OK;
+    const uint32_t n_tiles = dc.sky_key[5], words = (n_tiles + 31u) / 32u;
+    if (n_words < words) return ctx_fail(ctx, BRT_ERR_INVALID_ARGUMENT, "out_bits holds fewer than ceil(tiles / 32) words");
+    HIP_TRY(ctx, hipSetDevice(dc.device));
+    HIP_TRY(ctx, hipEventSynchronize(dc.ev_last));
+    HIP_TRY(ctx, hipMemcpy(out_bits, dc.d_sky_bits, (size_t)words * 4u, hipMemcpyDeviceToHost));
+    if (out_cost_or_null) {
+        if (!dc.costs_valid || dc.tile_cost_cap < (size_t)n_tiles * 8u || dc.order_key[5] != n_tiles)
+            return ctx_fail(ctx, BRT_ERR_INVALID_ARGUMENT, "no tile costs of this view (the last measurement is gone, or was made on the host path)");
+        HIP_TRY(ctx, hipMemcpy(out_cost_or_null, dc.d_tile_cost, (size_t)n_tiles * 8u, hipMemcpyDeviceToHost));
+    }
+    *out_n_tiles = n_tiles;
     return BRT_OK;
     });
 }
diff --git a/bevyray_amd/csrc/brt_ctx.h b/bevyray_amd/csrc/brt_ctx.h
--- a/bevyray_amd/csrc/brt_ctx.h
+++ b/bevyray_amd/csrc/brt_ctx.h
@@ -13,6 +13,7 @@
 #include "brt_kernels.h"
 #include "brt_pixels.h"
 #include "brt_query.h"
+#include "brt_sky.h"
 #include "brt_upscale.h"
 
 namespace brt {
@@ -57,6 +58,11 @@
     uint32_t order_crit = 0;
     size_t tile_order_cap = 0;
     uint32_t* d_order_meta = nullptr;
+    uint32_t* d_sky_bits = nullptr;
+    size_t sky_bits_cap = 0;
+    bool sky_valid = false;
+    uint32_t sky_key[7] = {0, 0, 0, 0, 0, 0, 0};
+    SkyCamera sky_cam{};
     char* d_strip_table = nullptr;
     size_t strip_table_cap = 0;
     uint32_t strip_epoch = 0;
@@ -126,7 +132,7 @@
 enum Knob : int {
     K_BOTTOM_UP, K_REFILL_MIN, K_WALK_EXIT, K_LEAF_VOTE, K_DRAIN_DONATE, K_POOL_ADOPT, K_WGQ_BATCH, K_LPT_LANE_PERMILLE, K_TUNABLE,
     K_FORCE_GLOBAL_SCENE, K_FORCE_LDS_TOP, K_BLOCK_THREADS, K_WG_PER_CU, K_POOL_CAP, K_LPT, K_LPT_SORT, K_LPT_SKY_SLACK, K_CRIT,
-    K_ORDER_ON_HOST, K_NO_LEAN, K_PREPASS_SPP, K_NO_DIRTY_TRACKING, K_CPU_BVH, K_PLOC_ONE_BLOCK_MAX, K_BVH_QUALITY, K_POOL_FORCE, K_LPT_REFRESH_EVERY, K_LEAN_MEASURE, K_LPT_DILATE, K_SPLIT_TAIL, K_SPLIT_FORCE, K_HOT_RECORDS, K_TEST_THROW, K_QUERY_FORM, K_QUERY_STREAM_MIN, K_PIXELS_FORM, K_COUNT
+    K_ORDER_ON_HOST, K_NO_LEAN, K_PREPASS_SPP, K_NO_DIRTY_TRACKING, K_CPU_BVH, K_PLOC_ONE_BLOCK_MAX, K_BVH_QUALITY, K_POOL_FORCE, K_LPT_REFRESH_EVERY, K_LEAN_MEASURE, K_LPT_DILATE, K_SPLIT_TAIL, K_SPLIT_FORCE, K_HOT_RECORDS, K_TEST_THROW, K_QUERY_FORM, K_QUERY_STREAM_MIN, K_PIXELS_FORM, K_SKY_TILES, K_COUNT
 };
 struct KnobDef { const char* name; uint32_t dflt; };
 constexpr KnobDef kKnobs[K_COUNT] = {
@@ -137,7 +143,8 @@
     {"BRT_NO_LEAN", 0}, {"BRT_PREPASS_SPP", 4}, {"BRT_NO_DIRTY_TRACKING", 0}, {"BRT_CPU_BVH", 0},
     {"BRT_PLOC_ONE_BLOCK_MAX", kPlocOneBlockMax}, {"BRT_BVH_QUALITY", 1}, {"BRT_POOL_FORCE", 0}, {"BRT_LPT_REFRESH_EVERY", 0}, {"BRT_LEAN_MEASURE", 1}, {"BRT_LPT_DILATE", 3}, {"BRT_SPLIT_TAIL", 16}, {"BRT_SPLIT_FORCE", 0}, {"BRT_HOT_RECORDS", 1}, {"BRT_TEST_THROW", 0},
     {"BRT_QUERY_FORM", 0}, {"BRT_QUERY_STREAM_MIN", 0},
-    {"BRT_PIXELS_FORM", 0}};
+    {"BRT_PIXELS_FORM", 0},
+    {"BRT_SKY_TILES", 1}};
 struct Knobs {
     uint32_t v[K_COUNT];
     Knobs() { for (int i = 0; i < K_COUNT; i++) v[i] = kKnobs[i].dflt; }
diff --git a/bevyray_amd/csrc/brt_frame.h b/bevyray_amd/csrc/brt_frame.h
--- a/bevyray_amd/csrc/brt_frame.h
+++ b/bevyray_amd/csrc/brt_frame.h
@@ -70,6 +70,8 @@
 void view_key_of(const brt_ctx* ctx, const FrameParams& fp, uint32_t key[8]);
 int32_t attach_tile_order(brt_ctx* ctx, DeviceCtx& dc, FrameParams& fp, hipStream_t stream, bool may_measure, uint32_t flags);
 int32_t update_tile_order(brt_ctx* ctx, DeviceCtx& dc, const FrameParams& fp, hipStream_t stream);
+int32_t attach_sky_tiles(brt_ctx* ctx, DeviceCtx& dc, const FrameParams& fp, hipStream_t stream, const uint32_t** d_bits);
+SkyCamera sky_camera_of(const FrameParams& fp);
 int32_t prepass_order(brt_ctx* ctx, DeviceCtx& dc, const FrameParams& fp, const float* d_raster_rgba,
                       const float* d_raster_depth, float* d_out_tile, hipStream_t stream, uint32_t flags, bool* ran);
 uint64_t tree_shape_hash(const EncodedScene& e);
diff --git a/bevyray_amd/csrc/brt_host.cpp b/bevyray_amd/csrc/brt_host.cpp
--- a/bevyray_amd/csrc/brt_host.cpp
+++ b/bevyray_amd/csrc/brt_host.cpp
@@ -1,6 +1,7 @@
 #include "brt_host.h"
 #include "brt_ploc.h"
 #include "brt_sah.h"
+#include "brt_sky.h"
 #include "brt_srgb_table.h"
 
 #include <algorithm>
@@ -805,6 +806,47 @@
     });
 }
 
+int32_t brt_host_sky_tile(const void* models, uint32_t n_models, const void* camera80, const void* window16, uint32_t width, uint32_t height,
+                          uint32_t part, uint32_t n_parts, float margin, uint32_t* out_bits, uint32_t n_words) {
+    return guard(nullptr, [&]() -> int32_t {
+    if ((!models && n_models != 0u) || !camera80 || !window16 || !out_bits) return fail(BRT_ERR_INVALID_ARGUMENT, "null pointer");
+    if (width == 0 || height == 0 || width > 32768u || height > 32768u) return fail(BRT_ERR_INVALID_ARGUMENT, "width/height must be in [1, 32768]");
+    if (n_parts == 0u || part >= n_parts) return fail(BRT_ERR_INVALID_ARGUMENT, "part >= n_parts");
+    Camera cam;
+    Window win;
+    std::memcpy(&cam, camera80, sizeof cam);
+    std::memcpy(&win, window16, sizeof win);
+    SkyCamera sc{};
+    const float heightf = (float)win.height;
+    const float widthf = (float)win.height * cam.aspect;
+    sc.inv_width = 1.0f / widthf;
+    sc.inv_height = 1.0f / heightf;
+    sc.aspect = cam.aspect;
+    sc.tan_half_fov = tan_half_fov(cam.fov);
+    const float* a = cam.direction;
+    const float* b = cam.up;
+    const float right[3] = {a[1] * b[2] - a[2] * b[1], a[2] * b[0] - a[0] * b[2], a[0] * b[1] - a[1] * b[0]};
+    for (int k = 0; k < 3; k++) { sc.pos[k] = cam.position[k]; sc.dir[k] = a[k]; sc.up[k] = b[k]; sc.right[k] = right[k]; }
+    sc.width = width; sc.height = height;
+    const uint32_t tiles_x = (width + 7u) / 8u, strips = (height + 7u) / 8u, local_strips = (strips + n_parts - 1u) / n_parts;
+    const uint32_t n_tiles = local_strips * tiles_x;
+    if (n_words < (n_tiles + 31u) / 32u) return fail(BRT_ERR_INVALID_ARGUMENT, "out_bits holds fewer than ceil(tiles / 32) words");
+    const Model* m = static_cast<const Model*>(models);
+    std::memset(out_bits, 0, (size_t)n_words * 4u);
+    for (uint32_t tile = 0; tile < n_tiles; tile++) {
+        const uint32_t strip = tile / tiles_x, tx = tile - strip * tiles_x;
+        uint32_t px0, py0, px1, py1;
+        if (!sky_tile_rect(width, height, tx, strip * n_parts + part, &px0, &py0, &px1, &py1)) continue;
+        const SkyPyramid p = sky_pyramid(sc, px0, py0, px1, py1);
+        bool sky = p.proper;
+        for (uint32_t i = 0; i < n_models && sky; i++)
+            sky = sky_sphere_separated(p, sc, m[i].position[0], m[i].position[1], m[i].position[2], m[i].radius * m[i].radius, (double)margin);
+        if (sky) out_bits[tile >> 5] |= 1u << (tile & 31u);
+    }
+    return BRT_OK;
+    });
+}
+
 int32_t brt_host_tile_order(const uint32_t* ray_sum, const uint32_t* longest_pixel, uint32_t n_tiles, uint32_t sample_count,
                             uint64_t grid_lanes, uint32_t sorted, uint32_t lane_permille, uint32_t tiles_x, uint32_t dilate,
                             uint32_t split_tail, uint32_t* out_order, uint32_t* out_info5) {
diff --git a/bevyray_amd/csrc/brt_kernels.h b/bevyray_amd/csrc/brt_kernels.h
--- a/bevyray_amd/csrc/brt_kernels.h
+++ b/bevyray_amd/csrc/brt_kernels.h
@@ -26,6 +26,7 @@
     uint32_t grid, block;
     size_t lds_bytes;
     hipStream_t stream;
+    const uint32_t* sky_bits;
 };
 
 size_t trace_lds_bytes(const DeviceSceneView& sv, int scene_mode, uint32_t block, uint32_t pool_cap, uint32_t hist_words = 0, bool rows = false);
diff --git a/bevyray_amd/csrc/brt_sky.h b/bevyray_amd/csrc/brt_sky.h
--- /dev/null
+++ b/bevyray_amd/csrc/brt_sky.h
@@ -0,0 +1,116 @@
+#pragma once
+#include <cstdint>
+
+#include "brt_ploc.h"
+
+namespace brt {
+
+constexpr double kSkyKappa = 32.0;
+constexpr double kSkyDirSlack = 9.5367431640625e-7;
+constexpr double kSkyAwayEps2 = 2.3283064365386963e-10;
+
+struct SkyCamera {
+    float pos[3], dir[3], up[3], right[3];
+    float aspect, tan_half_fov, inv_width, inv_height;
+    uint32_t width, height;
+};
+
+struct SkyPyramid {
+    double n[5][3];
+    double nn[5];
+    double k[4][3];
+    double kk[4];
+    bool proper;
+};
+
+BRT_HD SkyPyramid sky_pyramid(const SkyCamera& cam, uint32_t px0, uint32_t py0, uint32_t px1, uint32_t py1) {
+    const double W = (double)cam.width, H = (double)cam.height;
+    const double jx = 0.5 * __builtin_fabs((double)cam.inv_width), jy = 0.5 * __builtin_fabs((double)cam.inv_height);
+    const double ax = (double)cam.aspect * (double)cam.tan_half_fov, ay = (double)cam.tan_half_fov;
+    const double wx[2] = {(2.0 * (double)px0 - W) - jx * W, (2.0 * (double)px1 - W) + jx * W};
+    const double hy[2] = {(H - 2.0 * (double)py1) - jy * H, (H - 2.0 * (double)py0) + jy * H};
+    double sx[2], sy[2];
+    for (int k = 0; k < 2; k++) { sx[k] = (wx[k] * ax) * H; sy[k] = (hy[k] * ay) * W; }
+    const double wh = W * H;
+    const double bx = ax * (1.0 + 2.0 * jx), by = ay * (1.0 + 2.0 * jy);
+    const double slack = (kSkyDirSlack * ((1.0 + bx * bx) + by * by)) * wh;
+    sx[0] -= slack; sx[1] += slack; sy[0] -= slack; sy[1] += slack;
+    const int cx[4] = {0, 1, 1, 0}, cy[4] = {0, 0, 1, 1};
+    double K[4][3], C[3] = {0.0, 0.0, 0.0};
+    for (int i = 0; i < 4; i++)
+        for (int k = 0; k < 3; k++) {
+            K[i][k] = (wh * (double)cam.dir[k] + sx[cx[i]] * (double)cam.right[k]) + sy[cy[i]] * (double)cam.up[k];
+            C[k] += K[i][k];
+        }
+    SkyPyramid p;
+    p.proper = sx[0] < sx[1] && sy[0] < sy[1];
+    for (int i = 0; i < 4; i++) {
+        const double* a = K[i];
+        const double* b = K[(i + 1) & 3];
+        double n[3] = {a[1] * b[2] - a[2] * b[1], a[2] * b[0] - a[0] * b[2], a[0] * b[1] - a[1] * b[0]};
+        const double s = (n[0] * C[0] + n[1] * C[1]) + n[2] * C[2];
+        if (!(s > 0.0)) { n[0] = -n[0]; n[1] = -n[1]; n[2] = -n[2]; }
+        for (int k = 0; k < 3; k++) p.n[i][k] = n[k];
+        p.nn[i] = (n[0] * n[0] + n[1] * n[1]) + n[2] * n[2];
+        for (int j = 2; j < 4; j++) {
+            const double* c = K[(i + j) & 3];
+            const double t = (n[0] * c[0] + n[1] * c[1]) + n[2] * c[2];
+            if (!(t > 0.0)) p.proper = false;
+        }
+        const double f = (K[i][0] * C[0] + K[i][1] * C[1]) + K[i][2] * C[2];
+        if (!(f > 0.0)) p.proper = false;
+    }
+    for (int i = 0; i < 4; i++) {
+        for (int k = 0; k < 3; k++) p.k[i][k] = K[i][k];
+        p.kk[i] = (K[i][0] * K[i][0] + K[i][1] * K[i][1]) + K[i][2] * K[i][2];
+    }
+    for (int k = 0; k < 3; k++) p.n[4][k] = C[k];
+    p.nn[4] = (C[0] * C[0] + C[1] * C[1]) + C[2] * C[2];
+    for (int i = 0; i < 5; i++)
+        if (!(p.nn[i] > 0.0) || !(p.nn[i] - p.nn[i] == 0.0)) p.proper = false;
+    return p;
+}
+
+BRT_HD bool sky_sphere_separated(const SkyPyramid& p, const SkyCamera& cam, float cx, float cy, float cz, float r2, double margin) {
+    const double oc[3] = {(double)cx - (double)cam.pos[0], (double)cy - (double)cam.pos[1], (double)cz - (double)cam.pos[2]};
+    const double l2 = (oc[0] * oc[0] + oc[1] * oc[1]) + oc[2] * oc[2];
+    const double R2 = (double)r2 + (margin * kSkyKappa * 5.9604644775390625e-8) * (l2 + (double)r2);
+    bool sep = false;
+    for (int i = 0; i < 5; i++) {
+        const double s = (p.n[i][0] * oc[0] + p.n[i][1] * oc[1]) + p.n[i][2] * oc[2];
+        if (s < 0.0 && s * s > R2 * p.nn[i]) sep = true;
+    }
+    bool away = l2 > R2;
+    for (int i = 0; i < 4; i++) {
+        const double s = (p.k[i][0] * oc[0] + p.k[i][1] * oc[1]) + p.k[i][2] * oc[2];
+        if (!(s < 0.0 && s * s > (kSkyAwayEps2 * p.kk[i]) * l2)) away = false;
+    }
+    return sep || away;
+}
+
+BRT_HD bool sky_tile_rect(uint32_t width, uint32_t height, uint32_t tile_x, uint32_t frame_strip, uint32_t* px0, uint32_t* py0,
+                          uint32_t* px1, uint32_t* py1) {
+    *px0 = tile_x * 8u; *py0 = frame_strip * 8u;
+    if (*px0 >= width || *py0 >= height || frame_strip >= 0x10000000u) return false;
+    *px1 = *px0 + 8u < width ? *px0 + 8u : width;
+    *py1 = *py0 + 8u < height ? *py0 + 8u : height;
+    return true;
+}
+
+struct SkyFrame {
+    SkyCamera cam;
+    uint32_t tiles_x, n_tiles;
+    uint32_t part, n_parts;
+    const uint32_t* strip_of;
+};
+inline uint32_t sky_bitmap_words(uint32_t n_tiles) { return ((n_tiles + 63u) / 64u) * 2u; }
+
+}
+
+#if defined(__HIPCC__)
+#include <hip/hip_runtime.h>
+
+namespace brt {
+hipError_t launch_sky_tiles(const SkyFrame& sf, const float* d_spheres, uint32_t n_spheres, uint32_t* d_bits, hipStream_t stream);
+}
+#endif
diff --git a/bevyray_amd/csrc/brt_sky.hip b/bevyray_amd/csrc/brt_sky.hip
--- /dev/null
+++ b/bevyray_amd/csrc/brt_sky.hip
@@ -0,0 +1,55 @@
+#include <hip/hip_runtime.h>
+
+#include "brt_kernels.h"
+#include "brt_sky.h"
+
+namespace brt {
+
+namespace {
+
+constexpr uint32_t SB = 256;
+
+__global__ __launch_bounds__(SB) void k_sky_tiles(SkyFrame sf, const float4* __restrict__ spheres, uint32_t n_spheres,
+                                                  uint32_t* __restrict__ bits) {
+    __shared__ float4 s_sph[SB];
+    const uint32_t tile = blockIdx.x * SB + threadIdx.x;
+    bool sky = false;
+    SkyPyramid p;
+    p.proper = false;
+    if (tile < sf.n_tiles) {
+        const uint32_t strip = tile / sf.tiles_x, tx = tile - strip * sf.tiles_x;
+        const uint32_t frame_strip = sf.strip_of ? sf.strip_of[strip] : strip * sf.n_parts + sf.part;
+        uint32_t px0, py0, px1, py1;
+        if (sky_tile_rect(sf.cam.width, sf.cam.height, tx, frame_strip, &px0, &py0, &px1, &py1)) {
+            p = sky_pyramid(sf.cam, px0, py0, px1, py1);
+            sky = p.proper;
+        }
+    }
+    for (uint32_t base = 0; base < n_spheres; base += SB) {
+        if (__syncthreads_or(sky ? 1 : 0) == 0) break;
+        const uint32_t n = n_spheres - base < SB ? n_spheres - base : SB;
+        if (threadIdx.x < n) s_sph[threadIdx.x] = spheres[base + threadIdx.x];
+        __syncthreads();
+        if (sky)
+            for (uint32_t i = 0; i < n && sky; i++) {
+                const float4 s = s_sph[i];
+                sky = sky_sphere_separated(p, sf.cam, s.x, s.y, s.z, s.w, 1.0);
+            }
+    }
+    const unsigned long long m = __ballot(sky);
+    if ((threadIdx.x & 63u) == 0u && tile < ((sf.n_tiles + 63u) & ~63u)) {
+        bits[tile >> 5] = (uint32_t)m;
+        bits[(tile >> 5) + 1u] = (uint32_t)(m >> 32);
+    }
+}
+
+}
+
+hipError_t launch_sky_tiles(const SkyFrame& sf, const float* d_spheres, uint32_t n_spheres, uint32_t* d_bits, hipStream_t stream) {
+    if (sf.n_tiles == 0u) return hipSuccess;
+    hipLaunchKernelGGL(k_sky_tiles, dim3((sf.n_tiles + SB - 1u) / SB), dim3(SB), 0, stream, sf, reinterpret_cast<const float4*>(d_spheres),
+                       n_spheres, d_bits);
+    return hipGetLastError();
+}
+
+}
diff --git a/bevyray_amd/csrc/brt_trace.h b/bevyray_amd/csrc/brt_trace.h
--- a/bevyray_amd/csrc/brt_trace.h
+++ b/bevyray_amd/csrc/brt_trace.h
@@ -349,6 +349,27 @@
         } else {
             tput = tput * att;
             bounce++;
+        }
+    }
+}
+
+BRT_DEV void sky_tile_loop(const FrameParams& fp, const PixelCoord& c, uint32_t& n_rays, float* out_tile) {
+    if (c.inside) {
+        PixelState ps;
+        pixel_begin(fp, c, ps);
+        for (uint32_t s = 0; s < fp.sample_count; s++) {
+            const f3 d = normalize3(camera_dir_raw(fp, ps.ndc0x, ps.ndc0y, ps.rng));
+            const f3 n1 = normalize3(d);
+            const float a = 0.5f * (n1.y + 1.0f);
+            const float b = 1.0f - a;
+            const f3 light = mk3(b * 1.0f + a * 0.5f, b * 1.0f + a * 0.7f, b * 1.0f + a * 1.0f);
+            ps.sum = ps.sum + sqrt3(mk3(1.0f, 1.0f, 1.0f) * light);
+        }
+        n_rays += fp.sample_count;
+        pixel_finish<true>(fp, ps, out_tile, nullptr, nullptr);
+        if (fp.tile_cost) {
+            atomicAdd(&fp.tile_cost[c.tile], fp.sample_count);
+            atomicMax(&fp.tile_cost[fp.local_strips * fp.tiles_x + c.tile], fp.sample_count);
         }
     }
 }
@@ -475,6 +496,7 @@
     const bool slices = kSlices && fp.sample_count >= 16u;
     const bool slice_b = LEAN == 0 || fp.tile_cost != nullptr;
     const uint32_t queue_size = fp.queue_size + split_tiles * 64u;
+    const uint32_t* const sky_bits = LEAN != 0 ? reinterpret_cast<const uint32_t*>(raster_depth) : nullptr;
 
     PixelState ps;
     ps.sample = 0; ps.rng = 0; ps.out_index = 0; ps.frame_index = 0; ps.tile = 0; ps.rays_begin = 0;
@@ -607,8 +629,14 @@
             uint32_t b = 0;
             if (lane == 0) b = atomicAdd(queue_counter + 1, 64u);
             b = queue_lane + (uint32_t)__shfl((int)b, 0, 64);
-            if (b < queue_size) begin_pixel(b + lane, slot_tile(fp, b >> 6));
-            else {
+            if (b < queue_size) {
+                const uint32_t tile = slot_tile(fp, b >> 6);
+                if (LEAN != 0 && sky_bits != nullptr && (b < split_lo || b >= split_hi) && b >= crit_end && fp.sample_count != 0u &&
+                    ((sky_bits[tile >> 5] >> (tile & 31u)) & 1u) != 0u)
+                    sky_tile_loop(fp, slot_to_pixel<TUNABLE>(fp, b + lane, tile), n_rays, out_tile);
+                else
+                    begin_pixel(b + lane, tile);
+            } else {
                 tiles_done = true;
                 if (COUNTERS && t_empty == 0) t_empty = wall_clock64();
             }
@@ -820,7 +848,7 @@
                                        (int)tl.lds_bytes);
     if (e != hipSuccess) return e;
     hipLaunchKernelGGL(kern, dim3(tl.grid), dim3(tl.block), tl.lds_bytes, tl.stream, tl.scene, tl.frame, tl.queue_counter,
-                       tl.out_tile, tl.raster_rgba, tl.raster_depth, tl.counters);
+                       tl.out_tile, tl.raster_rgba, LEAN != 0 ? reinterpret_cast<const float*>(tl.sky_bits) : tl.raster_depth, tl.counters);
     return hipGetLastError();
 }
 
diff --git a/include/bevyray_amd.h b/include/bevyray_amd.h
--- a/include/bevyray_amd.h
+++ b/include/bevyray_amd.h
@@ -231,6 +231,11 @@
                              uint32_t sample_count, uint64_t grid_lanes, uint32_t tiles_x, uint32_t dilate, uint32_t split_tail,
                              uint32_t* out_order, uint32_t* out_info4);
 
+int32_t brt_debug_sky_tiles(brt_ctx* ctx, uint32_t* out_bits, uint32_t n_words, uint32_t* out_cost_or_null, uint32_t* out_n_tiles);
+
+
+int32_t brt_host_sky_tile(const void* models, uint32_t n_models, const void* camera80, const void* window16, uint32_t width,
+                          uint32_t height, uint32_t part, uint32_t n_parts, float margin, uint32_t* out_bits, uint32_t n_words);
 
 int32_t brt_host_tile_order(const uint32_t* ray_sum, const uint32_t* longest_pixel, uint32_t n_tiles, uint32_t sample_count,
                             uint64_t grid_lanes, uint32_t sorted, uint32_t lane_permille, uint32_t tiles_x, uint32_t dilate,
diff --git a/integration/bevyray_amd_sys/src/lib.rs b/integration/bevyray_amd_sys/src/lib.rs
--- a/integration/bevyray_amd_sys/src/lib.rs
+++ b/integration/bevyray_amd_sys/src/lib.rs
@@ -218,6 +218,10 @@
     pub fn brt_debug_tile_order(ctx: *mut brt_ctx, ray_sum: *const u32, longest_pixel: *const u32, n_tiles: u32,
                                 sample_count: u32, grid_lanes: u64, tiles_x: u32, dilate: u32, split_tail: u32,
                                 out_order: *mut u32, out_info4: *mut u32) -> i32;
+    pub fn brt_debug_sky_tiles(ctx: *mut brt_ctx, out_bits: *mut u32, n_words: u32, out_cost_or_null: *mut u32,
+                               out_n_tiles: *mut u32) -> i32;
+    pub fn brt_host_sky_tile(models: *const c_void, n_models: u32, camera80: *const c_void, window16: *const c_void, width: u32,
+                             height: u32, part: u32, n_parts: u32, margin: f32, out_bits: *mut u32, n_words: u32) -> i32;
     pub fn brt_host_tile_order(ray_sum: *const u32, longest_pixel: *const u32, n_tiles: u32, sample_count: u32,
                                grid_lanes: u64, sorted: u32, lane_permille: u32, tiles_x: u32, dilate: u32,
                                split_tail: u32, out_order: *mut u32, out_info5: *mut u32) -> i32;
```

Result: no change. 35060, median of 6 (+0.5%).
